# sandyresearch/chipmunk

Measured on AMD Instinct MI355X. Metric: DiT denoise steps/sec at fixed sparsity, higher is better.
Workload: dtype bf16

## Files before the change

### chipmunk_amd/_native.py

```python
from __future__ import annotations

import ctypes
import os

_HERE = os.path.dirname(os.path.abspath(__file__))
LIB_PATH = os.environ.get("CHIPMUNK_HIP_LIB") or os.path.join(_HERE, "lib", "libchipmunk_hip.so")

SYMBOLS = [
    "chipmunk_last_error", "chipmunk_abi_version", "chipmunk_set_option", "chipmunk_set_random_seed",
    "chipmunk_csp_attn", "chipmunk_csp_attn_out", "chipmunk_csp_128_attn", "chipmunk_dense_attn", "chipmunk_dense_colsum_attn",
    "chipmunk_csp_mlp_mm1", "chipmunk_csp_mlp_mm1_scatter", "chipmunk_csp_mlp_mm1_fp8", "chipmunk_csp_mlp_mm2_and_scatter_add", "chipmunk_csp_scatter_add", "chipmunk_csp_mlp_mm2",
    "chipmunk_csp_mlp_mm1_ragged", "chipmunk_csp_mlp_mm1_scatter_ragged", "chipmunk_csp_mlp_mm1_fp8_ragged", "chipmunk_csp_mlp_mm2_ragged",
    "chipmunk_csp_mlp_mm2_and_scatter_add_ragged", "chipmunk_csp_scatter_add_ragged", "chipmunk_block_mean_ragged", "chipmunk_transpose16_pitched",
    "chipmunk_csp_mlp_mm1_batched", "chipmunk_csp_mlp_mm1_scatter_batched", "chipmunk_csp_mlp_mm1_fp8_batched", "chipmunk_csp_mlp_mm2_batched",
    "chipmunk_csp_mlp_mm2_and_scatter_add_batched", "chipmunk_csp_scatter_add_batched",
    "chipmunk_csp_mlp_mm1_glu", "chipmunk_csp_mlp_mm1_glu_batched", "chipmunk_csp_mlp_mm1_glu_fp8", "chipmunk_csp_mlp_mm1_glu_fp8_batched",
    "chipmunk_topk_indices", "chipmunk_topk_delta_indices", "chipmunk_topk_mask", "chipmunk_mask_to_indices", "chipmunk_mask_to_sorted_indices", "chipmunk_packed_mask_to_indices", "chipmunk_mask_row_counts", "chipmunk_mask_to_ragged_indices", "chipmunk_copy_indices",
    "chipmunk_bitpack", "chipmunk_bitunpack", "chipmunk_transpose16", "chipmunk_block_mean", "chipmunk_quantize_fp8", "chipmunk_gather_rows", "chipmunk_qkv_split_norm", "chipmunk_split_heads_rownorm", "chipmunk_dense_colsum_topk_mask", "chipmunk_dense_attn_strided", "chipmunk_csp_attn_out_ragged", "chipmunk_compact_indices", "chipmunk_residual_ln_modulate", "chipmunk_dense_colsum_attn_strided", "chipmunk_dense_colsum_topk_mask_strided", "chipmunk_release_scratch", "chipmunk_big_scratch_fallbacks",
    "chipmunk_host_alloc", "chipmunk_host_free", "chipmunk_copy_d2h_async", "chipmunk_copy_h2d_async", "chipmunk_host_bytes",
]

_lib = None


def lib() -> ctypes.CDLL:
    global _lib
    if _lib is None:
        if not os.path.exists(LIB_PATH):
            raise ImportError(
                f"{LIB_PATH} is missing: build it with `python -m chipmunk_amd.build` (hipcc --offload-arch=gfx950). "
                "chipmunk_amd has no CPU fallback.")
        _lib = ctypes.CDLL(LIB_PATH)
        _lib.chipmunk_last_error.restype = ctypes.c_char_p
        _lib.chipmunk_abi_version.restype = ctypes.c_int
        for item in filter(None, os.environ.get("CHIPMUNK_AMD_OPTIONS", "").split(",")):
            name, _, val = item.partition("=")
            if _lib.chipmunk_set_option(name.strip().encode(), int(val)) != 0:
                raise ValueError(f"CHIPMUNK_AMD_OPTIONS: {_lib.chipmunk_last_error().decode()}")
    return _lib


def last_error() -> str:
    return lib().chipmunk_last_error().decode()


def check(rc: int, what: str) -> None:
    if rc != 0:
        raise RuntimeError(f"{what}: {last_error()}")


def set_option(name: str, value: int) -> None:
    check(lib().chipmunk_set_option(name.encode(), int(value)), "chipmunk_set_option")


def manual_seed(seed: int) -> None:
    check(lib().chipmunk_set_random_seed(ctypes.c_uint64(int(seed) & 0xFFFFFFFFFFFFFFFF)), "chipmunk_set_random_seed")


class HostBuffer:

    def __init__(self, numel: int, dtype) -> None:
        import torch
        self.dtype = dtype
        self._numel = int(numel)
        self._itemsize = torch.empty(0, dtype=dtype).element_size()
        self.nbytes = self._numel * self._itemsize
        p = ctypes.c_void_p()
        check(lib().chipmunk_host_alloc(ctypes.c_size_t(max(self.nbytes, 1)), ctypes.byref(p)), "chipmunk_host_alloc")
        self.ptr = p.value

    def numel(self) -> int:
        return self._numel

    def element_size(self) -> int:
        return self._itemsize

    def is_pinned(self) -> bool:
        return True

    def free(self) -> None:
        if getattr(self, "ptr", None):
            lib().chipmunk_host_free(ctypes.c_void_p(self.ptr))
            self.ptr = None

    def __del__(self):
        try:
            self.free()
        except Exception:
            pass


def copy_d2h_async(host_ptr: int, dev_ptr: int, nbytes: int, stream: int) -> None:
    check(lib().chipmunk_copy_d2h_async(ctypes.c_void_p(host_ptr), ctypes.c_void_p(dev_ptr), ctypes.c_size_t(nbytes), ctypes.c_void_p(stream)),
          "chipmunk_copy_d2h_async")


def copy_h2d_async(dev_ptr: int, host_ptr: int, nbytes: int, stream: int) -> None:
    check(lib().chipmunk_copy_h2d_async(ctypes.c_void_p(dev_ptr), ctypes.c_void_p(host_ptr), ctypes.c_size_t(nbytes), ctypes.c_void_p(stream)),
          "chipmunk_copy_h2d_async")


def host_bytes() -> int:
    f = lib().chipmunk_host_bytes
    f.restype = ctypes.c_size_t
    return int(f())
```

### chipmunk_amd/csrc/attn.hip

```cpp
#include "common.h"
#include "attn_params.h"
#include <type_traits>

namespace {

constexpr int QG = 192;
constexpr int QW = 48;
constexpr int KVT = 32;
constexpr int NST = 4;
constexpr int KRING = 8;
constexpr int HD = 128;
constexpr int TILE_BYTES = KVT * HD * 2;
constexpr float SCALE_LOG2E = 0.08838834764f * 1.44269504089f;
constexpr int NSTV = NST + 1;
constexpr int KEY_RING_OFF = (NST + NSTV) * TILE_BYTES;
constexpr int CS_OFF = KEY_RING_OFF + KRING * 256;
constexpr int ATTN_LDS_BYTES = CS_OFF + 2 * 2 * 4 * KVT * 4;

__device__ __forceinline__ f32x4 mfma16(bf16x8 a, bf16x8 b, f32x4 c) {
    return __builtin_amdgcn_mfma_f32_16x16x32_bf16(a, b, c, 0, 0, 0);
}

#ifdef ATTN_PROF
__device__ unsigned long long g_attn_prof[8 * 8];
// ... 1062 lines not shown
    p.q = (const uint16_t *)q, p.k = (const uint16_t *)k, p.v = (const uint16_t *)v, p.o = (uint16_t *)o_out;
    p.o_in = (const uint16_t *)o_in;
    for (int i = 0; i < 3; ++i) p.qs[i] = q_strides[i], p.ks[i] = k_strides[i], p.vs[i] = v_strides[i], p.os[i] = o_strides[i];
    p.indices = indices, p.counts = counts;
    p.B = B, p.H = H, p.Nq = Nq, p.Nk = Nk, p.G = (Nq + QG - 1) / QG, p.idx_stride = idx_stride;
    p.o_scale = (float)o_scale;
    return launch_attn<true, true, false>(p, (hipStream_t)stream);
}

extern "C" int chipmunk_csp_attn_out_ragged(const void *q, const void *k, const void *v, const void *o_in, void *o_out,
                                            const int64_t q_strides[3], const int64_t k_strides[3], const int64_t v_strides[3],
                                            const int64_t o_strides[3], const int32_t *indices, const int64_t *idx_offsets,
                                            const int32_t *counts, int B, int H, int Nq, int Nk, int o_scale, void *stream) {
    if (int e = check_common(q, k, v, o_out, B, H, Nq, Nk)) return e;
    CM_CHECK(o_in != nullptr && ((uintptr_t)o_in & 15) == 0, "csp_attn_out_ragged: o_in missing or not 16-byte aligned");
    CM_CHECK(o_scale == 1 || o_scale == -1, "o_scale must be 1 or -1");
    CM_CHECK(indices && counts && idx_offsets, "csp_attn_out_ragged: indices / offsets / counts missing");
    CM_CHECK(((uintptr_t)indices & 15) == 0, "csp_attn_out_ragged: indices must be 16-byte aligned");
    if (int e = check_strides(q_strides, "q")) return e;
    if (int e = check_strides(k_strides, "k")) return e;
    if (int e = check_strides(v_strides, "v")) return e;
    if (int e = check_strides(o_strides, "o")) return e;
    AttnParams p = {};
    p.q = (const uint16_t *)q, p.k = (const uint16_t *)k, p.v = (const uint16_t *)v, p.o = (uint16_t *)o_out;
    p.o_in = (const uint16_t *)o_in;
    for (int i = 0; i < 3; ++i) p.qs[i] = q_strides[i], p.ks[i] = k_strides[i], p.vs[i] = v_strides[i], p.os[i] = o_strides[i];
    p.indices = indices, p.counts = counts, p.idx_off = idx_offsets;
    p.B = B, p.H = H, p.Nq = Nq, p.Nk = Nk, p.G = (Nq + QG - 1) / QG, p.idx_stride = 0;
    p.o_scale = (float)o_scale;
    return launch_attn<true, true, false>(p, (hipStream_t)stream);
}

extern "C" int chipmunk_csp_128_attn(const void *q, const void *k, const void *v, void *o, const int32_t *indices,
                                     const int32_t *counts, int B, int H, int Nq, int Nk, int idx_stride,
                                     void *stream) {
    if (int e = check_common(q, k, v, o, B, H, Nq, Nk)) return e;
    CM_CHECK(indices && counts, "csp_128_attn: indices / counts missing");
    AttnParams p = {};
    p.q = (const uint16_t *)q, p.k = (const uint16_t *)k, p.v = (const uint16_t *)v, p.o = (uint16_t *)o;
    contiguous_strides(p.qs, H, Nq), contiguous_strides(p.os, H, Nq);
    contiguous_strides(p.ks, H, Nk), contiguous_strides(p.vs, H, Nk);
    p.indices = indices, p.counts = counts;
    p.B = B, p.H = H, p.Nq = Nq, p.Nk = Nk, p.G = (Nq + QG - 1) / QG, p.idx_stride = idx_stride;
    p.o_scale = 1.f;
    return launch_attn<true, false, false>(p, (hipStream_t)stream);
}

static int output_strides(int64_t os[3], const int64_t *o_strides, int H, int Nq) {
    if (!o_strides) {
        contiguous_strides(os, H, Nq);
        return CHIPMUNK_OK;
    }
    for (int i = 0; i < 3; ++i) os[i] = o_strides[i];
    return check_strides(o_strides, "o");
}

extern "C" int chipmunk_dense_attn_strided(const void *q, const void *k, const void *v, const int64_t q_strides[3],
                                           const int64_t k_strides[3], const int64_t v_strides[3], void *o,
                                           const int64_t *o_strides, float *l, int B, int H, int Nq, int Nk, void *stream) {
    if (int e = check_common(q, k, v, o, B, H, Nq, Nk)) return e;
    CM_CHECK(l != nullptr, "dense_attn: l output missing");
    if (int e = check_strides(q_strides, "q")) return e;
    if (int e = check_strides(k_strides, "k")) return e;
    if (int e = check_strides(v_strides, "v")) return e;
    AttnParams p = {};
    p.q = (const uint16_t *)q, p.k = (const uint16_t *)k, p.v = (const uint16_t *)v, p.o = (uint16_t *)o;
    for (int i = 0; i < 3; ++i) p.qs[i] = q_strides[i], p.ks[i] = k_strides[i], p.vs[i] = v_strides[i];
    if (int e = output_strides(p.os, o_strides, H, Nq)) return e;
    p.l_out = l;
    p.B = B, p.H = H, p.Nq = Nq, p.Nk = Nk, p.G = (Nq + QG - 1) / QG;
    p.o_scale = 1.f;
    if (use_dense64(B, H, Nq, Nk)) {
        CM_CHECK((int64_t)Nk * p.ks[2] * 2 < (1ll << 32) && (int64_t)Nk * p.vs[2] * 2 < (1ll << 32),
                 "attention: one head's K or V spans more than 4 GiB (32-bit DMA offsets)");
        return chipmunk_dense64_launch(q, k, v, o, l, p.qs, p.ks, p.vs, p.os, B, H, Nq, Nk, (hipStream_t)stream);
    }
    return launch_attn<false, false, true>(p, (hipStream_t)stream);
}

extern "C" int chipmunk_dense_attn(const void *q, const void *k, const void *v, const int64_t q_strides[3],
                                   const int64_t k_strides[3], const int64_t v_strides[3], void *o, float *l, int B,
                                   int H, int Nq, int Nk, void *stream) {
    return chipmunk_dense_attn_strided(q, k, v, q_strides, k_strides, v_strides, o, nullptr, l, B, H, Nq, Nk, stream);
}

extern "C" int chipmunk_dense_colsum_attn_strided(const void *q, const void *k, const void *v, const int64_t q_strides[3],
                                                  const int64_t k_strides[3], const int64_t v_strides[3], const float *pin,
                                                  void *o, const int64_t *o_strides, void *cs, float *l, int B, int H, int Nq,
                                                  int Nk, int cs_stride, void *stream) {
    if (int e = check_common(q, k, v, o, B, H, Nq, Nk)) return e;
    CM_CHECK(l && cs && pin, "dense_colsum_attn: p / cs / l missing");
    CM_CHECK(cs_stride >= Nk, "dense_colsum_attn: cs row stride %d < Nk %d", cs_stride, Nk);
    if (int e = check_strides(q_strides, "q")) return e;
    if (int e = check_strides(k_strides, "k")) return e;
    if (int e = check_strides(v_strides, "v")) return e;
    AttnParams p = {};
    p.q = (const uint16_t *)q, p.k = (const uint16_t *)k, p.v = (const uint16_t *)v, p.o = (uint16_t *)o;
    for (int i = 0; i < 3; ++i) p.qs[i] = q_strides[i], p.ks[i] = k_strides[i], p.vs[i] = v_strides[i];
    if (int e = output_strides(p.os, o_strides, H, Nq)) return e;
    p.l_out = l, p.p_in = pin, p.cs = (uint16_t *)cs, p.cs_stride = cs_stride;
    p.B = B, p.H = H, p.Nq = Nq, p.Nk = Nk, p.G = (Nq + QG - 1) / QG;
    p.o_scale = 1.f;
    hipStream_t st = (hipStream_t)stream;
    int rc;
    if (chipmunk_get_option("attn_fused_colsum") == 5) {
        if (use_colsum64(B, H, Nq, Nk)) return chipmunk_colsum64_launch(p, st);
        return launch_attn<false, false, false, true>(p, st);
    }
    if (use_dense64(B, H, Nq, Nk)) {
        CM_CHECK((int64_t)Nk * p.ks[2] * 2 < (1ll << 32) && (int64_t)Nk * p.vs[2] * 2 < (1ll << 32),
                 "attention: one head's K or V spans more than 4 GiB (32-bit DMA offsets)");
        if (chipmunk_get_option("attn_fused_colsum") != 2) {
            int hc = H;
            uint16_t *part = nullptr;
            const int hc_min = chipmunk_get_option("attn_fused_colsum") == 4 ? 1 : 0;
            if (hc_min) hc = 1;
            for (; hc >= 1; hc /= 2) {
                part = (uint16_t *)chipmunk_big_scratch(st, chipmunk_colsum_part_bytes(hc == H ? B : 1, hc, Nq, Nk));
                if (part) break;
            }
            if (part && hc == H) return chipmunk_dense64_colsum_launch(p, part, st);
            if (part) {
                for (int b = 0; b < B; ++b)
                    for (int h0 = 0; h0 < H; h0 += hc) {
                        AttnParams c = p;
                        const int hn = H - h0 < hc ? H - h0 : hc;
                        const int64_t bh0 = (int64_t)b * H + h0;
                        c.q += b * p.qs[0] + h0 * p.qs[1], c.k += b * p.ks[0] + h0 * p.ks[1], c.v += b * p.vs[0] + h0 * p.vs[1];
                        c.o += b * p.os[0] + h0 * p.os[1];
                        c.l_out += bh0 * Nq, c.p_in += bh0 * Nq, c.cs += bh0 * p.G * (int64_t)cs_stride;
                        c.B = 1, c.H = hn;
                        if (int e = chipmunk_dense64_colsum_launch(c, part, st)) return e;
                    }
                return CHIPMUNK_OK;
            }
        }
        rc = chipmunk_dense64_launch(q, k, v, o, l, p.qs, p.ks, p.vs, p.os, B, H, Nq, Nk, st);
    } else {
        rc = launch_attn<false, false, true>(p, st);
    }
    if (rc != CHIPMUNK_OK) return rc;
    if (use_colsum64(B, H, Nq, Nk)) return chipmunk_colsum64_launch(p, st);
    return launch_attn<false, false, false, true>(p, st);
}

extern "C" int chipmunk_dense_colsum_attn(const void *q, const void *k, const void *v, const int64_t q_strides[3],
                                          const int64_t k_strides[3], const int64_t v_strides[3], const float *pin,
                                          void *o, void *cs, float *l, int B, int H, int Nq, int Nk, int cs_stride,
                                          void *stream) {
    return chipmunk_dense_colsum_attn_strided(q, k, v, q_strides, k_strides, v_strides, pin, o, nullptr, cs, l, B, H, Nq, Nk,
                                              cs_stride, stream);
}

extern "C" int chipmunk_dense_colsum_topk_mask_strided(const void *q, const void *k, const void *v, const int64_t q_strides[3],
                                               const int64_t k_strides[3], const int64_t v_strides[3], const float *pin, void *o,
                                               const int64_t *o_strides, float *l, int B, int H, int Nq, int Nk, const void *static_mask,
                                               int64_t static_stride, int static_rows, const void *group_flags, void *mask,
                                               int topk, double random_amount, void *stream) {
    if (int e = check_common(q, k, v, o, B, H, Nq, Nk)) return e;
    CM_CHECK(l && pin && mask, "dense_colsum_topk_mask: p / l / mask missing");
    if (int e = check_strides(q_strides, "q")) return e;
    if (int e = check_strides(k_strides, "k")) return e;
    if (int e = check_strides(v_strides, "v")) return e;
    hipStream_t st = (hipStream_t)stream;
    if (!use_dense64(B, H, Nq, Nk) || chipmunk_get_option("attn_fused_colsum") == 2 || (Nk & 3) || Nk > CHIPMUNK_TOPK_MASK_MAX_N)
        return CHIPMUNK_ERR_UNSUPPORTED;
    AttnParams p = {};
    p.q = (const uint16_t *)q, p.k = (const uint16_t *)k, p.v = (const uint16_t *)v, p.o = (uint16_t *)o;
    for (int i = 0; i < 3; ++i) p.qs[i] = q_strides[i], p.ks[i] = k_strides[i], p.vs[i] = v_strides[i];
    CM_CHECK((int64_t)Nk * p.ks[2] * 2 < (1ll << 32) && (int64_t)Nk * p.vs[2] * 2 < (1ll << 32),
             "attention: one head's K or V spans more than 4 GiB (32-bit DMA offsets)");
    if (int e = output_strides(p.os, o_strides, H, Nq)) return e;
    p.l_out = l, p.p_in = pin, p.cs = nullptr, p.cs_stride = 0;
    p.B = B, p.H = H, p.Nq = Nq, p.Nk = Nk, p.G = (Nq + QG - 1) / QG;
    p.o_scale = 1.f;
    uint16_t *part = (uint16_t *)chipmunk_big_scratch(st, chipmunk_colsum_part_bytes(B, H, Nq, Nk));
    if (!part) return CHIPMUNK_ERR_UNSUPPORTED;
    if (int e = chipmunk_dense64_colsum_launch(p, part, st)) return e;
    const int nrb = ((Nq + 255) / 256) * 2;
    return chipmunk_topk_mask_parts(part, chipmunk_colsum_part_stride(Nk), nrb, p.G, Nq, static_mask, static_stride, static_rows, group_flags, mask, B * H * p.G, Nk,
                                    topk, random_amount, st);
}

extern "C" int chipmunk_dense_colsum_topk_mask(const void *q, const void *k, const void *v, const int64_t q_strides[3],
                                               const int64_t k_strides[3], const int64_t v_strides[3], const float *pin, void *o,
                                               float *l, int B, int H, int Nq, int Nk, const void *static_mask,
                                               int64_t static_stride, int static_rows, const void *group_flags, void *mask,
                                               int topk, double random_amount, void *stream) {
    return chipmunk_dense_colsum_topk_mask_strided(q, k, v, q_strides, k_strides, v_strides, pin, o, nullptr, l, B, H, Nq, Nk,
                                                   static_mask, static_stride, static_rows, group_flags, mask, topk, random_amount,
                                                   stream);
}
```

### chipmunk_amd/csrc/attn_params.h

```cpp
#pragma once
#include <stdint.h>
#include <hip/hip_runtime.h>

struct AttnParams {
    const uint16_t *q, *k, *v;
    uint16_t *o;
    const uint16_t *o_in;
    int64_t qs[3], ks[3], vs[3], os[3];
    const int32_t *indices, *counts;
    const int64_t *idx_off;
    float *l_out;
    const float *p_in;
    uint16_t *cs;
    int cs_stride;
    int B, H, Nq, Nk, G, idx_stride;
    float o_scale;
    int split_full, nsplit;
    float *ws;
    int32_t *tickets;
    const int32_t *plan;
    int xcd_chunks;
    const float *kmax;
    uint16_t *cs_part;
    int cs_pstride;
    int probe;
};


int chipmunk_csp64_launch(const AttnParams &p, int inplace, int grid, hipStream_t stream);
int chipmunk_dense64_colsum_launch(const AttnParams &p, uint16_t *part, hipStream_t stream);
int chipmunk_topk_mask_parts(const uint16_t *part, int part_stride, int nrb, int groups_per_bh, int Nq, const void *static_mask, int64_t static_stride,
                             int static_rows, const void *group_flags, void *mask, int rows, int n, int k, double random_amount,
                             hipStream_t stream);
size_t chipmunk_colsum_part_bytes(int B, int H, int Nq, int Nk);
int chipmunk_colsum_part_stride(int Nk);
int chipmunk_colsum64_launch(const AttnParams &p, hipStream_t stream);
int chipmunk_csp96_launch(const AttnParams &p, int inplace, int grid, hipStream_t stream);
const float *chipmunk_knorm_max(const uint16_t *k, const int64_t ks[3], int B, int H, int Nk, hipStream_t stream);

__host__ __device__ inline int colsum_part_rows(int j, int nwg, int &r0, int &r1) {
    const int a = (3 * j) >> 2, w0 = 3 * j - 4 * a;
    r0 = 2 * a + (w0 ? 1 : 0);
    r1 = 2 * (a + 1);
    return (w0 >= 2 && a + 1 < nwg) ? 2 : 1;
}

struct IndexRow {
    const int32_t *ptr;
    int width;
};
__device__ __forceinline__ IndexRow index_row(const AttnParams &p, int64_t item) {
    if (p.idx_off) {
        const int64_t o = p.idx_off[item];
        return {p.indices + o, (int)(p.idx_off[item + 1] - o)};
    }
    return {p.indices + item * p.idx_stride, p.idx_stride};
}
```

### chipmunk_amd/csrc/indexed_io.hip

```cpp
#include "common.h"
#include "attn_params.h"

namespace {

__device__ __forceinline__ uint32_t wave_incl_scan(uint32_t x) {
    x += (uint32_t)__builtin_amdgcn_update_dpp(0, (int)x, 0x111, 0xf, 0xf, true);
    x += (uint32_t)__builtin_amdgcn_update_dpp(0, (int)x, 0x112, 0xf, 0xf, true);
    x += (uint32_t)__builtin_amdgcn_update_dpp(0, (int)x, 0x114, 0xf, 0xf, true);
    x += (uint32_t)__builtin_amdgcn_update_dpp(0, (int)x, 0x118, 0xf, 0xf, true);
    x += (uint32_t)__builtin_amdgcn_update_dpp(0, (int)x, 0x142, 0xa, 0xf, false);
    x += (uint32_t)__builtin_amdgcn_update_dpp(0, (int)x, 0x143, 0xc, 0xf, false);
    return x;
}
struct M2IParams {
    const uint8_t *mask;
    int32_t *indices;
    int32_t *counts;
    int n, pad_n, multiple_of;
    const int64_t *offsets;
};

template <bool PACKED, bool SORTED = false, bool RAGGED = false>
__global__ __launch_bounds__(256) void mask_to_indices_kernel(const M2IParams p) {
    extern __shared__ __attribute__((aligned(16))) unsigned char smem[];
// ... 70 lines not shown
    }
    __syncthreads();

    if constexpr (SORTED) {
        uint32_t *blktot = (uint32_t *)T;
        for (int blk = w; blk < NB; blk += 4) {
            const uint32_t c = wave_incl_scan(__popc(bits[blk * 64 + lane]));
            if (lane == 63) blktot[blk] = c;
        }
        __syncthreads();
        if (w == 0) {
            uint32_t run = 0;
            for (int b0 = 0; b0 < NB; b0 += 64) {
                const uint32_t v = b0 + lane < NB ? blktot[b0 + lane] : 0u;
                const uint32_t incl = wave_incl_scan(v);
                if (b0 + lane < NB) blktot[b0 + lane] = run + incl - v;
                run += (uint32_t)__builtin_amdgcn_readlane((int)incl, 63);
            }
            if (lane == 0) blktot[NB] = run;
        }
        __syncthreads();
        const int total = (int)blktot[NB];
        for (int blk = w; blk < NB; blk += 4) {
            uint32_t v = bits[blk * 64 + lane];
            const uint32_t c = __popc(v);
            const uint32_t incl = wave_incl_scan(c);
            int pos = (int)(blktot[blk] + incl - c);
            const int col0 = (blk * 64 + lane) * 32;
            while (v) {
                const int bit = __builtin_ctz(v);
                v &= v - 1;
                put(pos++, col0 + bit);
            }
        }
        if constexpr (RAGGED) zero_rest(total);
        if (tid == 0) {
            const int padded = ((total + p.multiple_of - 1) / p.multiple_of) * p.multiple_of;
            int pp = total;
            for (int i = 0; i < NI && pp < padded; ++i) {
                uint32_t z = ~bits[i];
                const int rem = n - i * 32;
                if (rem < 32) z &= (1u << rem) - 1u;
                while (z && pp < padded) {
                    const int bit = __builtin_ctz(z);
                    z &= z - 1;
                    put(pp++, i * 32 + bit);
                }
            }
            if constexpr (!RAGGED) p.counts[row] = padded;
        }
        return;
    }
    for (int blk = w; blk < NB; blk += 4) {
        const uint32_t word = bits[blk * 64 + lane];
        unsigned long long mine = 0;
#pragma unroll
        for (int t = 0; t < 32; ++t) {
            const unsigned long long bal = __ballot((word >> t) & 1u);
            if (lane == t) mine = bal;
        }
        if (lane < 32) T[lane * NB + blk] = mine;
    }
    __syncthreads();

    if (tid < 32) {
        uint32_t run = 0;
        for (int blk = 0; blk < NB; ++blk) {
            pre[tid * NB + blk] = run;
            run += __popcll(T[tid * NB + blk]);
        }
        cls[tid + 1] = run;
    }
    __syncthreads();
    if (tid == 0) {
        uint32_t run = 0;
        for (int t = 0; t < 32; ++t) {
            const uint32_t c = cls[t + 1];
            cls[t] = run;
            run += c;
            if (t == 31) cls[32] = run;
        }
    }
    __syncthreads();
    const int total = (int)cls[32];

    for (int cell = tid; cell < 32 * NB; cell += 256) {
        const int t = cell / NB, blk = cell - t * NB;
        unsigned long long v = T[cell];
        int pos = (int)(cls[t] + pre[cell]);
        while (v) {
            const int bit = __builtin_ctzll(v);
            v &= v - 1;
            put(pos++, ((blk * 64 + bit) << 5) + t);
        }
    }
    if constexpr (RAGGED) zero_rest(total);

    if (tid == 0) {
        const int padded = ((total + p.multiple_of - 1) / p.multiple_of) * p.multiple_of;
        int pos = total;
        for (int i = 0; i < NI && pos < padded; ++i) {
            uint32_t z = ~bits[i];
            const int rem = n - i * 32;
            if (rem < 32) z &= (1u << rem) - 1u;
            while (z && pos < padded) {
                const int bit = __builtin_ctz(z);
                z &= z - 1;
                put(pos++, i * 32 + bit);
            }
        }
        if constexpr (!RAGGED) p.counts[row] = padded;
    }
}

struct RowCountParams {
    const uint8_t *mask;
    int32_t *counts;
    int64_t *lengths;
    int64_t rows;
    int n, pad_n, multiple_of;
};

template <bool PACKED>
__global__ __launch_bounds__(256) void mask_row_counts_kernel(const RowCountParams p) {
    const int lane = threadIdx.x & 63;
    const int64_t row = (int64_t)blockIdx.x * 4 + (threadIdx.x >> 6);
    if (row >= p.rows) return;
    const int nbytes = PACKED ? p.n >> 3 : p.n;
    const uint8_t *src = p.mask + (PACKED ? (row * p.n) >> 3 : row * p.n);
    auto set_in_byte = [](uint32_t b) { return PACKED ? (uint32_t)__popc(b) : (uint32_t)(b != 0); };
    auto set_in_word = [](uint32_t x) {
        if constexpr (!PACKED) x = (x | (x >> 1) | (x >> 2) | (x >> 3) | (x >> 4) | (x >> 5) | (x >> 6) | (x >> 7)) & 0x01010101u;
        return (uint32_t)__popc(x);
    };
    const int head = min(nbytes, (int)((16 - ((uintptr_t)src & 15)) & 15));
    uint32_t cnt = lane < head ? set_in_byte(src[lane]) : 0u;
    const int nvec = (nbytes - head) >> 4;
    const u32x4 *vec = (const u32x4 *)(src + head);
#pragma unroll 4
    for (int i = lane; i < nvec; i += 64) {
        const u32x4 x = vec[i];
        cnt += set_in_word(x[0]) + set_in_word(x[1]) + set_in_word(x[2]) + set_in_word(x[3]);
    }
    const int tail = head + (nvec << 4) + lane;
    if (tail < nbytes) cnt += set_in_byte(src[tail]);
    const int64_t kept = (uint32_t)__builtin_amdgcn_readlane((int)wave_incl_scan(cnt), 63);
    if (lane == 0) {
        const int64_t padded = ((kept + p.multiple_of - 1) / p.multiple_of) * p.multiple_of;
        p.counts[row] = (int32_t)padded;
        p.lengths[row] = (min(padded, (int64_t)p.pad_n) + 31) / 32 * 32;
    }
}

struct TopkParams {
    const void *act;
    void *cache;
    int32_t *indices;
    int32_t *counts;
    int rows, cols, multiple_of;
    float quantile, random_amount;
    uint32_t salt;
};

template <typename T>
__device__ __forceinline__ float load_as_float(const T *p, int i);
template <>
__device__ __forceinline__ float load_as_float<uint16_t>(const uint16_t *p, int i) { return bf16_bits_to_f32(p[i]); }
template <>
__device__ __forceinline__ float load_as_float<_Float16>(const _Float16 *p, int i) { return (float)p[i]; }
template <>
__device__ __forceinline__ float load_as_float<float>(const float *p, int i) { return p[i]; }

template <typename T>
__device__ __forceinline__ float round_to(float x);
template <>
__device__ __forceinline__ float round_to<uint16_t>(float x) { return round_bf16(x); }
template <>
__device__ __forceinline__ float round_to<_Float16>(float x) { return (float)(_Float16)x; }
template <>
__device__ __forceinline__ float round_to<float>(float x) { return x; }

__device__ __forceinline__ float hash_uniform(uint32_t row, uint32_t col, uint32_t salt) {
    uint32_t x = (row * 0x9E3779B9u ^ (col + 0x7F4A7C15u) * 0x85EBCA6Bu) + salt * 0xC2B2AE35u;
    x ^= x >> 16, x *= 0x7feb352du, x ^= x >> 15, x *= 0x846ca68bu, x ^= x >> 16;
    return (float)(x >> 8) * (1.0f / 16777216.0f);
}

__device__ __forceinline__ int compact_slot(bool keep, int lane, int w, uint32_t *wave_tot, int &base) {
    const unsigned long long bal = __ballot(keep);
    const int before = __popcll(bal & ((1ull << lane) - 1ull));
    if (lane == 0) wave_tot[w] = __popcll(bal);
    __syncthreads();
    int off = base, tot = 0;
#pragma unroll
    for (int i = 0; i < 16; ++i) {
        const int c = wave_tot[i];
        off += i < w ? c : 0;
        tot += c;
    }
    __syncthreads();
    base += tot;
    return keep ? off + before : -1;
}

template <typename T, bool DELTA>
__global__ __launch_bounds__(1024) void topk_indices_kernel(const TopkParams p) {
    __shared__ uint32_t wave_tot[16];
    __shared__ float thr_s;
    const int tid = threadIdx.x, lane = tid & 63, w = tid >> 6;
    const int row = blockIdx.x;
    const T *x = (const T *)p.act + (int64_t)row * p.cols;
    T *xc = DELTA ? (T *)p.cache + (int64_t)row * p.cols : nullptr;
    int32_t *out = p.indices + (int64_t)row * p.cols;
    const int cols = p.cols;
    auto value = [&](int c) {
        const float b = load_as_float<T>(x, c);
        if constexpr (DELTA) return fabsf(round_to<T>(b - load_as_float<T>(xc, c)));
        else return b;
    };

    const uint32_t salt = p.salt ^ (__float_as_uint(value(0)) * 0x27D4EB2Fu);
    if (p.quantile == 0.f) {
        if constexpr (DELTA)
            for (int c = tid; c < cols; c += 1024) xc[c] = x[c];
        for (int c = tid; c < cols; c += 1024) out[c] = c;
        if (tid == 0) p.counts[row] = cols;
        return;
    }
    if (p.quantile == 1.f) {
        for (int c = tid; c < cols; c += 1024) out[c] = -1;
        if (tid == 0) p.counts[row] = 0;
        return;
    }
    __shared__ float sample[1024];
    float v_first[16];
#pragma unroll
    for (int j = 0; j < 16; ++j) {
        const int c = j * 1024 + tid;
        v_first[j] = c < cols ? value(c) : 0.f;
    }
    sample[tid] = v_first[0];
    __syncthreads();
    if (w == 0) {
        uint32_t key[16];
#pragma unroll
        for (int j = 0; j < 16; ++j) {
            const uint32_t u = __float_as_uint(sample[lane + 64 * j]);
            key[j] = (u & 0x80000000u) ? ~u : (u | 0x80000000u);
        }
        const int k = (int)(1024 * p.quantile);
        uint32_t res = 0;
        constexpr int LOWZ = !DELTA ? 0 : std::is_same<T, uint16_t>::value ? 16 : std::is_same<T, _Float16>::value ? 13 : 0;
        constexpr int LAST = LOWZ ? LOWZ - 1 : 0;
        for (int bit = 31; bit >= LAST; --bit) {
            const uint32_t cand = res | (LOWZ && bit == LAST ? (1u << LOWZ) - 1u : (1u << bit));
            int cnt = 0;
#pragma unroll
            for (int j = 0; j < 16; ++j) cnt += key[j] < cand ? 1 : 0;
            const int tot = (int)sum_across_rows(row16_sum((float)cnt));
            if (tot <= k) res = cand;
        }
        const uint32_t u = (res & 0x80000000u) ? (res & 0x7fffffffu) : ~res;
        if (lane == 0) thr_s = __uint_as_float(u);
    }
    __syncthreads();
    const float thr = thr_s;

    __shared__ uint32_t tot[16 * 16 + 1];
    int base = 0;
    int my_last_invalid = -1;
    for (int pass0 = 0; pass0 < cols; pass0 += 16 * 1024) {
        float v[16];
#pragma unroll
        for (int j = 0; j < 16; ++j) {
            const int c = pass0 + j * 1024 + tid;
            v[j] = pass0 == 0 ? v_first[j] : (c < cols ? value(c) : 0.f);
        }
        uint32_t keepbits = 0;
        int before[16];
#pragma unroll
        for (int j = 0; j < 16; ++j) {
            const int c = pass0 + j * 1024 + tid;
            bool keep = false;
            if (c < cols) {
                keep = v[j] >= thr;
                if (!keep && p.random_amount > 0.f) keep = hash_uniform(row, c, salt) < p.random_amount;
                if (!keep) my_last_invalid = c;
            }
            const unsigned long long bal = __ballot(keep);
            before[j] = __popcll(bal & ((1ull << lane) - 1ull));
            if (lane == 0) tot[j * 16 + w] = __popcll(bal);
            keepbits |= keep ? (1u << j) : 0u;
        }
        __syncthreads();
        if (tid < 64) {
            uint32_t a0 = tot[tid * 4], a1 = tot[tid * 4 + 1], a2 = tot[tid * 4 + 2], a3 = tot[tid * 4 + 3];
            uint32_t sum = a0 + a1 + a2 + a3, incl = sum;
#pragma unroll
            for (int d = 1; d < 64; d <<= 1) {
                const uint32_t o = __shfl_up(incl, d);
                if (lane >= d) incl += o;
            }
            const uint32_t excl = incl - sum;
            tot[tid * 4] = excl, tot[tid * 4 + 1] = excl + a0, tot[tid * 4 + 2] = excl + a0 + a1;
            tot[tid * 4 + 3] = excl + a0 + a1 + a2;
            if (tid == 63) tot[256] = incl;
// ... 9 lines not shown
        base += tot[256];
        __syncthreads();
    }
    const int kept = base;
    const int mod = kept % p.multiple_of;
    const int pad = mod == 0 ? 0 : p.multiple_of - mod;
    if (tid == 0) p.counts[row] = kept + pad;
    if (pad > 0) {
        int pbase = 0;
        const int slot = compact_slot(my_last_invalid != -1, lane, w, wave_tot, pbase);
        if (slot >= 0 && slot < pad) {
            out[kept + slot] = my_last_invalid;
            if constexpr (DELTA) xc[my_last_invalid] = x[my_last_invalid];
        }
    }
}

template <typename T>
__global__ __launch_bounds__(256) void copy_indices_kernel(const T *src, T *dst, const int32_t *inds,
                                                           const int32_t *counts, int M, int R, int F) {
    const int64_t grow = blockIdx.x;
    const int64_t b = grow / ((int64_t)M * R);
    const int base_m = (int)((grow % ((int64_t)M * R)) / R);
    const int cnt = counts[b * M + base_m];
    const int32_t *ii = inds + (b * M + base_m) * (int64_t)F;
    for (int c = threadIdx.x; c < cnt; c += 256) {
        const int col = ii[c];
        dst[grow * F + col] = src[grow * F + col];
    }
}

__global__ __launch_bounds__(256) void bitpack_kernel(const uint8_t *mask, uint8_t *packed, int64_t n) {
    const int64_t nb = (n + 7) >> 3;
    for (int64_t i = (int64_t)blockIdx.x * 256 + threadIdx.x; i < nb; i += (int64_t)gridDim.x * 256) {
        uint8_t byte = 0;
        if (i * 8 + 8 <= n && ((((uintptr_t)mask) & 7) == 0)) {
            unsigned long long v = *(const unsigned long long *)(mask + i * 8);
#pragma unroll
            for (int j = 0; j < 8; ++j) byte |= (uint8_t)((((v >> (8 * j)) & 0xffull) != 0) << j);
        } else {
            for (int j = 0; j < 8 && i * 8 + j < n; ++j) byte |= (uint8_t)((mask[i * 8 + j] != 0) << j);
        }
        packed[i] = byte;
    }
}
__global__ __launch_bounds__(256) void bitunpack_kernel(const uint8_t *packed, uint8_t *mask, int64_t n) {
    const int64_t nb = (n + 7) >> 3;
    for (int64_t i = (int64_t)blockIdx.x * 256 + threadIdx.x; i < nb; i += (int64_t)gridDim.x * 256) {
        const uint8_t byte = packed[i];
        if (i * 8 + 8 <= n && ((((uintptr_t)mask) & 7) == 0)) {
            unsigned long long v = 0;
#pragma unroll
            for (int j = 0; j < 8; ++j) v |= (unsigned long long)((byte >> j) & 1u) << (8 * j);
            *(unsigned long long *)(mask + i * 8) = v;
        } else {
            for (int j = 0; j < 8 && i * 8 + j < n; ++j) mask[i * 8 + j] = (byte >> j) & 1u;
        }
    }
}

__global__ __launch_bounds__(256) void transpose16_kernel(const uint16_t *src, uint16_t *dst, int R, int C, int ld) {
    __shared__ __attribute__((aligned(16))) uint16_t tile[64][72];
    const int64_t boff = (int64_t)blockIdx.z * R * C;
    const int r0 = blockIdx.y * 64, c0 = blockIdx.x * 64;
    const int tid = threadIdx.x;
#pragma unroll
    for (int i = 0; i < 2; ++i) {
        const int item = i * 256 + tid, r = item >> 3, ch = item & 7;
        u32x4 v = {0u, 0u, 0u, 0u};
        if (r0 + r < R && c0 + ch * 8 + 8 <= C) v = *(const u32x4 *)(src + boff + (int64_t)(r0 + r) * C + c0 + ch * 8);
        else if (r0 + r < R)
            for (int e = 0; e < 8; ++e)
                if (c0 + ch * 8 + e < C) {
                    const uint32_t x = src[boff + (int64_t)(r0 + r) * C + c0 + ch * 8 + e];
                    v[e >> 1] |= x << (16 * (e & 1));
                }
#pragma unroll
        for (int e = 0; e < 4; ++e) {
            tile[ch * 8 + 2 * e][r] = (uint16_t)(v[e] & 0xffffu);
            tile[ch * 8 + 2 * e + 1][r] = (uint16_t)(v[e] >> 16);
        }
    }
    __syncthreads();
#pragma unroll
    for (int i = 0; i < 2; ++i) {
        const int item = i * 256 + tid, c = item >> 3, ch = item & 7;
        if (c0 + c >= C) continue;
        uint16_t *d = dst + (int64_t)blockIdx.z * C * ld + (int64_t)(c0 + c) * ld + r0 + ch * 8;
        if (r0 + ch * 8 + 8 <= ld && ((ld & 7) == 0)) *(u32x4 *)d = *(const u32x4 *)&tile[c][ch * 8];
        else
            for (int e = 0; e < 8; ++e)
                if (r0 + ch * 8 + e < ld) d[e] = tile[c][ch * 8 + e];
    }
}

__global__ __launch_bounds__(256) void compact_indices_kernel(const int32_t *indices, int64_t idx_stride, const int32_t *counts,
                                                             const int64_t *offsets, int32_t *flat) {
    const int64_t r = blockIdx.x;
    const int32_t *src = indices + r * idx_stride;
    const int64_t o = offsets[r];
    int32_t *dst = flat + o;
    const int width = (int)(offsets[r + 1] - o);
    int c = counts[r];
    c = c < 0 ? 0 : (c < width ? c : width);
    c = c < idx_stride ? c : (int)idx_stride;
    if ((((uintptr_t)src | (uintptr_t)dst) & 15) == 0) {
        const int c4 = c >> 2;
        for (int i = threadIdx.x; i < c4; i += 256) ((u32x4 *)dst)[i] = ((const u32x4 *)src)[i];
        for (int i = (c4 << 2) + threadIdx.x; i < c; i += 256) dst[i] = src[i];
    } else {
        for (int i = threadIdx.x; i < c; i += 256) dst[i] = src[i];
    }
    for (int i = c + threadIdx.x; i < width; i += 256) dst[i] = 0;
}

size_t m2i_lds_bytes(int n, bool sorted) {
    const int NI = (n + 31) >> 5, NB = (NI + 63) >> 6;
    if (sorted) return (size_t)NB * 64 * 4 + (size_t)(NB + 1) * 4 + 16;
    return (size_t)NB * 64 * 4 + (size_t)32 * NB * 8 + (size_t)32 * NB * 4 + 33 * 4 + 16;
}

template <bool PACKED, bool SORTED = false, bool RAGGED = false>
int launch_m2i(const void *mask, int32_t *indices, int32_t *counts, int64_t rows, int n, int pad_n, int multiple_of,
               void *stream, const int64_t *offsets = nullptr) {
    CM_CHECK(mask && indices && (RAGGED ? (const void *)offsets : (const void *)counts), "mask_to_indices: null pointer");
    CM_CHECK(rows >= 0 && n > 0 && pad_n >= n && multiple_of > 0, "mask_to_indices: bad sizes rows=%lld n=%d pad_n=%d multiple_of=%d",
             (long long)rows, n, pad_n, multiple_of);
    CM_CHECK(rows < (1ll << 31), "mask_to_indices: too many rows");
    if (PACKED) CM_CHECK(n % 8 == 0, "packed_mask_to_indices: n must be a multiple of 8 (got %d)", n);
    const size_t lds = m2i_lds_bytes(n, SORTED);
    CM_CHECK(lds <= 160 * 1024, "mask_to_indices: row length %d needs %zu B of LDS (> 160 KiB)", n, lds);
    if (rows == 0) return CHIPMUNK_OK;
    auto kern = mask_to_indices_kernel<PACKED, SORTED, RAGGED>;
    if (lds > 64 * 1024) (void)hipFuncSetAttribute((const void *)kern, hipFuncAttributeMaxDynamicSharedMemorySize, (int)lds);
    M2IParams p = {(const uint8_t *)mask, indices, counts, n, pad_n, multiple_of, offsets};
    hipLaunchKernelGGL(kern, dim3((unsigned)rows), dim3(256), lds, (hipStream_t)stream, p);
    CM_LAUNCH_CHECK();
    return CHIPMUNK_OK;
}


struct TopkMaskParams {
    const uint16_t *cs;
    const uint8_t *stat;
    const uint8_t *groups;
    uint8_t *mask;
    int64_t cs_stride, stat_stride;
    int rows, n, k, stat_rows;
    float random_amount;
    uint32_t salt;
    const uint16_t *parts;
    int64_t pstride;
    int nrb, ngroups, nq;
};

__device__ __forceinline__ uint32_t bf16_key(uint32_t u) {
    return (u & 0x8000u) ? (~u & 0xffffu) : (u | 0x8000u);
}

template <int KPT, bool ALIGNED, bool PARTS = false>
__global__ __launch_bounds__(1024) void topk_mask_kernel(const TopkMaskParams p) {
    constexpr int NV = KPT / 4;
    __shared__ int wave_cnt[16];
    const int tid = threadIdx.x, lane = tid & 63, w = tid >> 6;
    const int row = blockIdx.x;
    const int n = p.n;
    const uint16_t *x = nullptr;
    int prow = 1;
    int64_t row1 = 0;
    if constexpr (PARTS) {
        const int bh = row / p.ngroups, g = row - bh * p.ngroups;
        int r0, r1;
        prow = colsum_part_rows(g, p.nrb / 2, r0, r1);
        x = p.parts + ((int64_t)bh * p.nrb + r0) * p.pstride;
        row1 = (int64_t)(r1 - r0) * p.pstride;
    } else {
        x = p.cs + (int64_t)row * p.cs_stride;
    }
    const uint32_t lane_off8 = 8u * (uint32_t)tid;
    const uint32_t lane_off4 = 4u * (uint32_t)tid;
    uint32_t key[NV][2];
    constexpr int LB = NV % 10 == 0 ? 10 : (NV % 8 == 0 ? 8 : (NV % 6 == 0 ? 6 : 4));
    static_assert(NV % LB == 0, "NV must split into whole load batches");
#pragma unroll
    for (int j0 = 0; j0 < NV; j0 += LB) {
        uint32_t raw[LB][2];
#pragma unroll
        for (int jj = 0; jj < LB; ++jj) {
            const int c = 4 * tid + 4096 * (j0 + jj);
            uint32_t v0 = 0xffffffffu, v1 = 0xffffffffu;
            if constexpr (ALIGNED) {
                if (c < n) {
                    const u32x2 v = *(const u32x2 *)((const unsigned char *)(x + 4096 * (j0 + jj)) + lane_off8);
                    v0 = v[0], v1 = v[1];
                    if constexpr (PARTS) {
                        if (prow == 2) {
                            float a0 = __uint_as_float(v0 << 16), a1 = __uint_as_float(v0 & 0xffff0000u);
                            float a2 = __uint_as_float(v1 << 16), a3 = __uint_as_float(v1 & 0xffff0000u);
                            const u32x2 y = *(const u32x2 *)((const unsigned char *)(x + row1 + 4096 * (j0 + jj)) + lane_off8);
                            a0 += __uint_as_float(y[0] << 16), a1 += __uint_as_float(y[0] & 0xffff0000u);
                            a2 += __uint_as_float(y[1] << 16), a3 += __uint_as_float(y[1] & 0xffff0000u);
                            v0 = pack_bf16x2(a0, a1), v1 = pack_bf16x2(a2, a3);
                        }
                    }
                }
            } else if (c < n) {
                v0 = v1 = 0;
#pragma unroll
                for (int e = 0; e < 4; ++e) {
                    const uint32_t u = c + e < n ? x[c + e] : 0xffffu;
                    if (e < 2) v0 |= u << (16 * e);
                    else v1 |= u << (16 * (e - 2));
                }
            }
            raw[jj][0] = v0, raw[jj][1] = v1;
        }
#pragma unroll
        for (int jj = 0; jj < LB; ++jj) {
            key[j0 + jj][0] = bf16_key(raw[jj][0] & 0xffffu) | (bf16_key(raw[jj][0] >> 16) << 16);
            key[j0 + jj][1] = bf16_key(raw[jj][1] & 0xffffu) | (bf16_key(raw[jj][1] >> 16) << 16);
        }
        __builtin_amdgcn_sched_barrier(0);
    }
    auto block_count = [&](int mine) {
#pragma unroll
        for (int d = 32; d > 0; d >>= 1) mine += __shfl_xor(mine, d);
        if (lane == 0) wave_cnt[w] = mine;
        __syncthreads();
        int t = 0;
#pragma unroll
        for (int i = 0; i < 16; ++i) t += wave_cnt[i];
        __syncthreads();
        return t;
    };
    const bool active = p.groups == nullptr || p.groups[row] != 0;
    const int k = p.k < n ? p.k : n;
    uint32_t thr = 0x10000u;
    int ties_to_take = 0;
    if (active && k > 0) {
        uint32_t res = 0;
        for (int bit = 15; bit >= 0; --bit) {
            const uint32_t cand = res | (1u << bit);
            const uint32_t cm1 = (cand - 1u) | ((cand - 1u) << 16);
            const uint32_t one2 = 0x00010001u;
            uint32_t cnt2 = 0;
#pragma unroll
            for (int j = 0; j < NV; ++j)
#pragma unroll
                for (int h = 0; h < 2; ++h) {
                    uint32_t d;
                    asm volatile("v_pk_sub_u16 %0, %1, %2 clamp\n\tv_pk_min_u16 %0, %0, %3" : "=&v"(d) : "v"(key[j][h]), "v"(cm1), "v"(one2));
                    asm volatile("v_pk_add_u16 %0, %0, %1" : "+v"(cnt2) : "v"(d));
                }
            const int mine = (int)(cnt2 & 0xffffu) + (int)(cnt2 >> 16);
            if (block_count(mine) >= k) res = cand;
        }
        thr = res;
        int gt = 0;
#pragma unroll
        for (int j = 0; j < NV; ++j)
#pragma unroll
            for (int h = 0; h < 2; ++h) {
                uint32_t kw = key[j][h];
                asm volatile("" : "+v"(kw));
                gt += ((kw & 0xffffu) > thr ? 1 : 0) + ((kw >> 16) > thr ? 1 : 0);
            }
        ties_to_take = k - block_count(gt);
    }
    int my_ties = 0;
    if (ties_to_take > 0) {
#pragma unroll
        for (int j = 0; j < NV; ++j)
#pragma unroll
            for (int h = 0; h < 2; ++h) {
                uint32_t kw = key[j][h];
                asm volatile("" : "+v"(kw));
                my_ties += ((kw & 0xffffu) == thr ? 1 : 0) + ((kw >> 16) == thr ? 1 : 0);
            }
    }
    int tie_budget = 0;
    {
        int incl = my_ties;
#pragma unroll
        for (int d = 1; d < 64; d <<= 1) {
            const int o = __shfl_up(incl, d);
            if (lane >= d) incl += o;
        }
        if (lane == 63) wave_cnt[w] = incl;
        __syncthreads();
        int before = incl - my_ties;
#pragma unroll
        for (int i = 0; i < 16; ++i) before += i < w ? wave_cnt[i] : 0;
        __syncthreads();
        tie_budget = ties_to_take - before;
    }
    uint8_t *out = p.mask + (int64_t)row * n;
    const uint8_t *st = p.stat ? p.stat + (int64_t)(row % p.stat_rows) * p.stat_stride : nullptr;
    const bool rnd = active && p.random_amount > 0.f;
    auto combined4 = [&](int c0, uint32_t &v0, uint32_t &v1) {
        const u32x2 v = *(const u32x2 *)(x + c0);
        v0 = v[0], v1 = v[1];
        if constexpr (PARTS) {
            float a0 = __uint_as_float(v0 << 16), a1 = __uint_as_float(v0 & 0xffff0000u);
            float a2 = __uint_as_float(v1 << 16), a3 = __uint_as_float(v1 & 0xffff0000u);
            if (prow == 2) {
                const u32x2 y = *(const u32x2 *)(x + row1 + c0);
                a0 += __uint_as_float(y[0] << 16), a1 += __uint_as_float(y[0] & 0xffff0000u);
                a2 += __uint_as_float(y[1] << 16), a3 += __uint_as_float(y[1] & 0xffff0000u);
            }
            v0 = pack_bf16x2(a0, a1), v1 = pack_bf16x2(a2, a3);
        }
    };
    uint32_t first = x[0];
    if constexpr (PARTS) {
        uint32_t f0, f1;
        combined4(0, f0, f1);
        first = f0 & 0xffffu;
    }
    const uint32_t salt = p.salt ^ (first * 0x27D4EB2Fu);
    const int nsteps = (n + 4095) / 4096;
    auto emit = [&](auto keyed, int c, uint32_t v0, uint32_t v1, uint32_t sb) {
        uint32_t bytes = 0;
        if constexpr (decltype(keyed)::value) asm volatile("" : "+v"(v0), "+v"(v1));
#pragma unroll
        for (int e = 0; e < 4; ++e) {
            const uint32_t half = ((e < 2 ? v0 : v1) >> (16 * (e & 1))) & 0xffffu;
            const uint32_t kv = decltype(keyed)::value ? half : bf16_key(half);
            bool keep = kv > thr;
            const bool tie = kv == thr && tie_budget > 0 && c + e < n;
            tie_budget -= tie ? 1 : 0;
            keep = keep || tie;
            if (rnd && !keep) keep = hash_uniform(row, c + e, salt) < p.random_amount;
            keep = keep || ((sb >> (8 * e)) & 0xffu) != 0;
            bytes |= (keep ? 1u : 0u) << (8 * e);
        }
        if constexpr (ALIGNED) {
            *(uint32_t *)(out + c) = bytes;
        } else {
#pragma unroll
            for (int e = 0; e < 4; ++e)
                if (c + e < n) out[c + e] = (uint8_t)(bytes >> (8 * e));
        }
    };
    if constexpr (ALIGNED) {
        constexpr int OB = 5;
#pragma unroll
        for (int j0 = 0; j0 < NV; j0 += OB) {
            uint32_t sbv[OB];
#pragma unroll
            for (int jj = 0; jj < OB; ++jj) {
                const int c = 4 * tid + 4096 * (j0 + jj);
                sbv[jj] = (j0 + jj < NV && st && c < n) ? *(const uint32_t *)(st + c) : 0u;
            }
            __builtin_amdgcn_sched_barrier(0);
#pragma unroll
            for (int jj = 0; jj < OB; ++jj) {
                if constexpr (true) {
                    const int c = 4 * tid + 4096 * (j0 + jj);
                    if (j0 + jj < NV && c < n) emit(std::integral_constant<int, 1>{}, c, key[(j0 + jj) < NV ? (j0 + jj) : 0][0], key[(j0 + jj) < NV ? (j0 + jj) : 0][1], sbv[jj]);
                    asm volatile("" ::: "memory");
                }
            }
            __builtin_amdgcn_sched_barrier(0);
        }
    } else {
        for (int j = 0; j < nsteps; ++j) {
            const int c = 4 * tid + 4096 * j;
            if (c >= n) break;
            uint32_t v0 = 0, v1 = 0, sb = 0;
#pragma unroll
            for (int e = 0; e < 4; ++e) {
                const uint32_t u = c + e < n ? x[c + e] : 0xffffu;
                if (e < 2) v0 |= u << (16 * e);
                else v1 |= u << (16 * (e - 2));
                if (st && c + e < n) sb |= (uint32_t)st[c + e] << (8 * e);
            }
            emit(std::integral_constant<int, 0>{}, c, v0, v1, sb);
        }
    }
}

__device__ __forceinline__ uint32_t bf16_key2(uint32_t u) {
    uint32_t s;
    const uint32_t fifteen2 = 0x000f000fu;
    asm("v_pk_ashrrev_i16 %0, %1, %2" : "=v"(s) : "v"(fifteen2), "v"(u));
    return u ^ (s | 0x80008000u);
}

template <bool ALIGNED, bool PARTS>
__global__ __launch_bounds__(1024) void topk_mask_stream_kernel(const TopkMaskParams p) {
    __shared__ int wave_cnt[16];
    const int tid = threadIdx.x, lane = tid & 63, w = tid >> 6;
    const int row = blockIdx.x;
    const int n = p.n;
    const uint16_t *x = nullptr;
    int prow = 1;
    int64_t row1 = 0;
    if constexpr (PARTS) {
        const int bh = row / p.ngroups, g = row - bh * p.ngroups;
        int r0, r1;
        prow = colsum_part_rows(g, p.nrb / 2, r0, r1);
        x = p.parts + ((int64_t)bh * p.nrb + r0) * p.pstride;
        row1 = (int64_t)(r1 - r0) * p.pstride;
    } else {
        x = p.cs + (int64_t)row * p.cs_stride;
    }
    const uint32_t lane_off8 = 8u * (uint32_t)tid;
    const int nsteps = (n + 4095) / 4096;
    const bool active = p.groups == nullptr || p.groups[row] != 0;
    const int k = p.k < n ? p.k : n;
    const bool select = active && k > 0;
    const bool rnd = active && p.random_amount > 0.f;

    auto combined4 = [&](int c0, uint32_t &v0, uint32_t &v1) {
        const u32x2 v = *(const u32x2 *)(x + c0);
        v0 = v[0], v1 = v[1];
        if constexpr (PARTS) {
            if (prow == 2) {
                float a0 = __uint_as_float(v0 << 16), a1 = __uint_as_float(v0 & 0xffff0000u);
                float a2 = __uint_as_float(v1 << 16), a3 = __uint_as_float(v1 & 0xffff0000u);
                const u32x2 y = *(const u32x2 *)(x + row1 + c0);
                a0 += __uint_as_float(y[0] << 16), a1 += __uint_as_float(y[0] & 0xffff0000u);
                a2 += __uint_as_float(y[1] << 16), a3 += __uint_as_float(y[1] & 0xffff0000u);
                v0 = pack_bf16x2(a0, a1), v1 = pack_bf16x2(a2, a3);
            }
        }
    };
    uint32_t first = 0;
    if (rnd) {
        first = x[0];
        if constexpr (PARTS) {
            uint32_t f0, f1;
            combined4(0, f0, f1);
            first = f0 & 0xffffu;
        }
    }
    const uint32_t salt = p.salt ^ (first * 0x27D4EB2Fu);
    if constexpr (PARTS) {
        __syncthreads();
        if (select) {
            uint16_t *xk = const_cast<uint16_t *>(x);
            for (int j = 0; j < nsteps; ++j) {
                const int c = 4 * tid + 4096 * j;
                if (c < n) {
                    uint32_t v0, v1;
                    combined4(c, v0, v1);
                    u32x2 kk = {bf16_key2(v0), bf16_key2(v1)};
                    *(u32x2 *)(xk + c) = kk;
                }
            }
        }
        __syncthreads();
    }
    auto load_raw = [&](int j, uint32_t &v0, uint32_t &v1) {
        const int c = 4 * tid + 4096 * j;
        if constexpr (ALIGNED) {
            v0 = v1 = PARTS ? 0u : 0xffffffffu;
            if (c < n) {
                const u32x2 v = *(const u32x2 *)((const unsigned char *)(x + 4096 * j) + lane_off8);
                v0 = v[0], v1 = v[1];
            }
        } else {
            v0 = v1 = 0xffffffffu;
            if (c < n) {
                v0 = v1 = 0;
#pragma unroll
                for (int e = 0; e < 4; ++e) {
                    const uint32_t u = c + e < n ? x[c + e] : 0xffffu;
                    if (e < 2) v0 |= u << (16 * e);
                    else v1 |= u << (16 * (e - 2));
                }
            }
        }
    };
    auto to_keys = [&](uint32_t &v0, uint32_t &v1) {
        if constexpr (!PARTS) v0 = bf16_key2(v0), v1 = bf16_key2(v1);
    };
    auto block_count = [&](int mine) {
#pragma unroll
        for (int d = 32; d > 0; d >>= 1) mine += __shfl_xor(mine, d);
        if (lane == 0) wave_cnt[w] = mine;
        __syncthreads();
        int t = 0;
#pragma unroll
        for (int i = 0; i < 16; ++i) t += wave_cnt[i];
        __syncthreads();
        return t;
    };
    constexpr int U = ALIGNED ? 8 : 2;
    uint32_t thr = 0x10000u;
    int ties_to_take = 0, my_ties = 0;
    if (select) {
        uint32_t res = 0;
        for (int bit = 15; bit >= 0; --bit) {
            const uint32_t cand = res | (1u << bit);
            const uint32_t cm1 = (cand - 1u) | ((cand - 1u) << 16);
            const uint32_t one2 = 0x00010001u;
// ... 5 lines not shown
#pragma unroll
                for (int jj = 0; jj < U; ++jj) {
                    to_keys(kw[jj][0], kw[jj][1]);
#pragma unroll
                    for (int h = 0; h < 2; ++h) {
                        uint32_t d;
                        asm volatile("v_pk_sub_u16 %0, %1, %2 clamp\n\tv_pk_min_u16 %0, %0, %3" : "=&v"(d) : "v"(kw[jj][h]), "v"(cm1), "v"(one2));
                        asm volatile("v_pk_add_u16 %0, %0, %1" : "+v"(cnt2) : "v"(d));
                    }
                }
            }
            const int mine = (int)(cnt2 & 0xffffu) + (int)(cnt2 >> 16);
            if (block_count(mine) >= k) res = cand;
        }
        thr = res;
        int gt = 0;
        for (int j0 = 0; j0 < nsteps; j0 += U) {
            uint32_t kw[U][2];
#pragma unroll
            for (int jj = 0; jj < U; ++jj) load_raw(j0 + jj, kw[jj][0], kw[jj][1]);
#pragma unroll
            for (int jj = 0; jj < U; ++jj) {
                to_keys(kw[jj][0], kw[jj][1]);
#pragma unroll
                for (int h = 0; h < 2; ++h) {
                    const uint32_t lo = kw[jj][h] & 0xffffu, hi = kw[jj][h] >> 16;
                    gt += (lo > thr ? 1 : 0) + (hi > thr ? 1 : 0);
                    my_ties += (lo == thr ? 1 : 0) + (hi == thr ? 1 : 0);
                }
            }
        }
        ties_to_take = k - block_count(gt);
    }
    int tie_budget = 0;
    {
        int incl = my_ties;
#pragma unroll
        for (int d = 1; d < 64; d <<= 1) {
            const int o = __shfl_up(incl, d);
            if (lane >= d) incl += o;
        }
        if (lane == 63) wave_cnt[w] = incl;
        __syncthreads();
        int before = incl - my_ties;
#pragma unroll
        for (int i = 0; i < 16; ++i) before += i < w ? wave_cnt[i] : 0;
        __syncthreads();
        tie_budget = ties_to_take - before;
    }
    uint8_t *out = p.mask + (int64_t)row * n;
    const uint8_t *st = p.stat ? p.stat + (int64_t)(row % p.stat_rows) * p.stat_stride : nullptr;
    for (int j0 = 0; j0 < nsteps; j0 += U) {
        uint32_t kw[U][2], sbv[U];
#pragma unroll
        for (int jj = 0; jj < U; ++jj) {
            const int c = 4 * tid + 4096 * (j0 + jj);
            kw[jj][0] = kw[jj][1] = 0;
            if (select) load_raw(j0 + jj, kw[jj][0], kw[jj][1]);
            sbv[jj] = 0;
            if constexpr (ALIGNED) {
                if (st && c < n) sbv[jj] = *(const uint32_t *)(st + c);
            } else if (st) {
#pragma unroll
                for (int e = 0; e < 4; ++e)
                    if (c + e < n) sbv[jj] |= (uint32_t)st[c + e] << (8 * e);
            }
        }
#pragma unroll
        for (int jj = 0; jj < U; ++jj) {
            const int c = 4 * tid + 4096 * (j0 + jj);
            if (c >= n) continue;
            if (select) to_keys(kw[jj][0], kw[jj][1]);
            uint32_t bytes = 0;
#pragma unroll
            for (int e = 0; e < 4; ++e) {
                const uint32_t kv = (kw[jj][e >> 1] >> (16 * (e & 1))) & 0xffffu;
                bool keep = kv > thr;
                const bool tie = kv == thr && tie_budget > 0 && c + e < n;
                tie_budget -= tie ? 1 : 0;
                keep = keep || tie;
                if (rnd && !keep) keep = hash_uniform(row, c + e, salt) < p.random_amount;
                keep = keep || ((sbv[jj] >> (8 * e)) & 0xffu) != 0;
                bytes |= (keep ? 1u : 0u) << (8 * e);
            }
            if constexpr (ALIGNED) {
                *(uint32_t *)(out + c) = bytes;
            } else {
#pragma unroll
                for (int e = 0; e < 4; ++e)
                    if (c + e < n) out[c + e] = (uint8_t)(bytes >> (8 * e));
            }
        }
    }
}

}

extern "C" int chipmunk_mask_to_indices(const void *mask, int32_t *indices, int32_t *counts, int64_t rows, int n,
                                        int pad_n, int multiple_of, void *stream) {
    return launch_m2i<false>(mask, indices, counts, rows, n, pad_n, multiple_of, stream);
}

extern "C" int chipmunk_packed_mask_to_indices(const void *packed, int32_t *indices, int32_t *counts, int64_t rows,
                                               int n, int pad_n, int multiple_of, void *stream) {
    return launch_m2i<true>(packed, indices, counts, rows, n, pad_n, multiple_of, stream);
}

static int launch_topk(const void *activation, void *cache, int dtype, int32_t *indices, int32_t *counts, int rows,
                       int cols, double sparsity_amount, int multiple_of, double random_amount, void *stream) {
    CM_CHECK(activation && indices && counts, "topk_indices: null pointer");
    CM_CHECK(rows >= 0 && cols >= 1024, "topk_indices: rows >= 0 and cols >= 1024 required (the quantile is taken over the first 1024 columns); got rows=%d cols=%d", rows, cols);
    CM_CHECK(multiple_of > 0, "topk_indices: multiple_of must be positive");
    CM_CHECK(sparsity_amount >= 0.0 && sparsity_amount <= 1.0, "topk_indices: sparsity_amount must be in [0,1]");
    if (rows == 0) return CHIPMUNK_OK;
    TopkParams p = {activation, cache, indices, counts, rows, cols, multiple_of, (float)sparsity_amount, (float)random_amount,
                    random_amount > 0.0 ? chipmunk_next_random_salt() : 0u};
    hipStream_t s = (hipStream_t)stream;
#define LAUNCH_TOPK(T)                                                                                           \
    do {                                                                                                         \
        if (cache) hipLaunchKernelGGL((topk_indices_kernel<T, true>), dim3(rows), dim3(1024), 0, s, p);          \
        else hipLaunchKernelGGL((topk_indices_kernel<T, false>), dim3(rows), dim3(1024), 0, s, p);               \
    } while (0)
    switch (dtype) {
        case CHIPMUNK_DTYPE_BF16: LAUNCH_TOPK(uint16_t); break;
        case CHIPMUNK_DTYPE_FP16: LAUNCH_TOPK(_Float16); break;
        case CHIPMUNK_DTYPE_FP32: LAUNCH_TOPK(float); break;
        default: CM_CHECK(false, "topk_indices: unsupported dtype code %d", dtype);
    }
#undef LAUNCH_TOPK
    CM_LAUNCH_CHECK();
    return CHIPMUNK_OK;
}

extern "C" int chipmunk_mask_to_sorted_indices(const void *mask, int packed, int32_t *indices, int32_t *counts,
                                               int64_t rows, int n, int pad_n, int multiple_of, void *stream) {
    return packed ? launch_m2i<true, true>(mask, indices, counts, rows, n, pad_n, multiple_of, stream)
                  : launch_m2i<false, true>(mask, indices, counts, rows, n, pad_n, multiple_of, stream);
}

extern "C" int chipmunk_mask_row_counts(const void *mask, int packed, int32_t *counts, int64_t *lengths, int64_t rows, int n,
                                        int pad_n, int multiple_of, void *stream) {
    CM_CHECK(mask && counts && lengths, "mask_row_counts: null pointer");
    CM_CHECK(rows >= 0 && n > 0 && pad_n >= n && multiple_of > 0, "mask_row_counts: bad sizes rows=%lld n=%d pad_n=%d multiple_of=%d",
             (long long)rows, n, pad_n, multiple_of);
    CM_CHECK(rows < (1ll << 31), "mask_row_counts: too many rows");
    CM_CHECK(!packed || n % 8 == 0, "mask_row_counts: n must be a multiple of 8 for a packed mask (got %d)", n);
    const size_t lds = m2i_lds_bytes(n, true);
    CM_CHECK(lds <= 160 * 1024, "mask_to_indices: row length %d needs %zu B of LDS (> 160 KiB)", n, lds);
    if (rows == 0) return CHIPMUNK_OK;
    RowCountParams p = {(const uint8_t *)mask, counts, lengths, rows, n, pad_n, multiple_of};
    const dim3 grid((unsigned)((rows + 3) / 4));
    if (packed) hipLaunchKernelGGL(mask_row_counts_kernel<true>, grid, dim3(256), 0, (hipStream_t)stream, p);
    else hipLaunchKernelGGL(mask_row_counts_kernel<false>, grid, dim3(256), 0, (hipStream_t)stream, p);
    CM_LAUNCH_CHECK();
    return CHIPMUNK_OK;
}

extern "C" int chipmunk_mask_to_ragged_indices(const void *mask, int packed, int sorted, const int64_t *offsets, int32_t *flat,
                                               int64_t rows, int n, int multiple_of, void *stream) {
    if (packed) return sorted ? launch_m2i<true, true, true>(mask, flat, nullptr, rows, n, n, multiple_of, stream, offsets)
                              : launch_m2i<true, false, true>(mask, flat, nullptr, rows, n, n, multiple_of, stream, offsets);
    return sorted ? launch_m2i<false, true, true>(mask, flat, nullptr, rows, n, n, multiple_of, stream, offsets)
                  : launch_m2i<false, false, true>(mask, flat, nullptr, rows, n, n, multiple_of, stream, offsets);
}

extern "C" int chipmunk_topk_indices(const void *activation, int dtype, int32_t *indices, int32_t *counts, int rows,
                                     int cols, double sparsity_amount, int multiple_of, double random_amount,
                                     void *stream) {
    return launch_topk(activation, nullptr, dtype, indices, counts, rows, cols, sparsity_amount, multiple_of,
                       random_amount, stream);
}

extern "C" int chipmunk_topk_delta_indices(const void *activation, void *cache, int dtype, int32_t *indices,
                                           int32_t *counts, int rows, int cols, double sparsity_amount,
                                           int multiple_of, double random_amount, void *stream) {
    CM_CHECK(cache != nullptr, "topk_delta_indices: cache missing");
    return launch_topk(activation, cache, dtype, indices, counts, rows, cols, sparsity_amount, multiple_of,
                       random_amount, stream);
}

extern "C" int chipmunk_copy_indices(const void *src, void *dst, const int32_t *inds, const int32_t *counts, int B,
                                     int M, int R, int F, int elem_size, void *stream) {
    CM_CHECK(src && dst && inds && counts, "copy_indices: null pointer");
    CM_CHECK(B >= 0 && M > 0 && R > 0 && F > 0, "copy_indices: bad sizes");
    CM_CHECK(elem_size == 2 || elem_size == 4, "copy_indices: element size must be 2 or 4 bytes (got %d)", elem_size);
    const int64_t rows = (int64_t)B * M * R;
    if (rows == 0) return CHIPMUNK_OK;
    CM_CHECK(rows < (1ll << 31), "copy_indices: too many rows");
    hipStream_t s = (hipStream_t)stream;
    if (elem_size == 2)
        hipLaunchKernelGGL(copy_indices_kernel<uint16_t>, dim3((unsigned)rows), dim3(256), 0, s, (const uint16_t *)src,
                           (uint16_t *)dst, inds, counts, M, R, F);
    else
        hipLaunchKernelGGL(copy_indices_kernel<uint32_t>, dim3((unsigned)rows), dim3(256), 0, s, (const uint32_t *)src,
                           (uint32_t *)dst, inds, counts, M, R, F);
    CM_LAUNCH_CHECK();
    return CHIPMUNK_OK;
}

extern "C" int chipmunk_bitpack(const void *mask, void *packed, int64_t n, void *stream) {
    CM_CHECK(mask && packed && n >= 0, "bitpack: bad arguments");
    if (n == 0) return CHIPMUNK_OK;
    const int64_t nb = (n + 7) >> 3;
    const unsigned grid = (unsigned)((nb + 255) / 256 < 8192 ? (nb + 255) / 256 : 8192);
    hipLaunchKernelGGL(bitpack_kernel, dim3(grid), dim3(256), 0, (hipStream_t)stream, (const uint8_t *)mask,
                       (uint8_t *)packed, n);
    CM_LAUNCH_CHECK();
    return CHIPMUNK_OK;
}

extern "C" int chipmunk_bitunpack(const void *packed, void *mask, int64_t n, void *stream) {
    CM_CHECK(mask && packed && n >= 0, "bitunpack: bad arguments");
    if (n == 0) return CHIPMUNK_OK;
    const int64_t nb = (n + 7) >> 3;
    const unsigned grid = (unsigned)((nb + 255) / 256 < 8192 ? (nb + 255) / 256 : 8192);
    hipLaunchKernelGGL(bitunpack_kernel, dim3(grid), dim3(256), 0, (hipStream_t)stream, (const uint8_t *)packed,
                       (uint8_t *)mask, n);
    CM_LAUNCH_CHECK();
    return CHIPMUNK_OK;
}

extern "C" int chipmunk_transpose16(const void *src, void *dst, int B, int R, int C, void *stream) {
    CM_CHECK(src && dst && B > 0 && R > 0 && C > 0, "transpose16: bad arguments");
    CM_CHECK((C & 7) == 0 || true, "unreachable");
    hipLaunchKernelGGL(transpose16_kernel, dim3((C + 63) / 64, (R + 63) / 64, B), dim3(256), 0, (hipStream_t)stream,
                       (const uint16_t *)src, (uint16_t *)dst, R, C, R);
    CM_LAUNCH_CHECK();
    return CHIPMUNK_OK;
}

extern "C" int chipmunk_transpose16_pitched(const void *src, void *dst, int B, int R, int C, int ld, void *stream) {
    CM_CHECK(src && dst && B > 0 && R > 0 && C > 0, "transpose16: bad arguments");
    CM_CHECK(ld >= R, "transpose16: the output pitch ld (%d) must be at least R (%d)", ld, R);
    hipLaunchKernelGGL(transpose16_kernel, dim3((C + 63) / 64, (ld + 63) / 64, B), dim3(256), 0, (hipStream_t)stream,
                       (const uint16_t *)src, (uint16_t *)dst, R, C, ld);
    CM_LAUNCH_CHECK();
    return CHIPMUNK_OK;
}

template <typename V>
__global__ __launch_bounds__(256) void gather_rows_kernel(const V *src, V *dst, const int32_t *map, int64_t n_out,
                                                          int64_t n_src, int64_t cpr, int64_t total) {
    for (int64_t idx = (int64_t)blockIdx.x * 256 + threadIdx.x; idx < total; idx += (int64_t)gridDim.x * 256) {
        const int64_t row = idx / cpr, c = idx - row * cpr;
        const int64_t o = row / n_out, r = row - o * n_out;
        dst[idx] = src[(o * n_src + map[r]) * cpr + c];
    }
}

extern "C" int chipmunk_gather_rows(const void *src, void *dst, const int32_t *map, int64_t outer, int64_t n_src,
                                    int64_t n_out, int64_t row_bytes, void *stream) {
    CM_CHECK(src && dst && map, "gather_rows: null pointer");
    CM_CHECK(outer >= 0 && n_src > 0 && n_out >= 0 && row_bytes > 0, "gather_rows: bad sizes");
    if (outer == 0 || n_out == 0) return CHIPMUNK_OK;
    hipStream_t s = (hipStream_t)stream;
    const uintptr_t align = (uintptr_t)src | (uintptr_t)dst | (uintptr_t)row_bytes;
#define LAUNCH_GATHER(V)                                                                                              \
    do {                                                                                                              \
        const int64_t cpr = row_bytes / (int64_t)sizeof(V), total = outer * n_out * cpr;                               \
        const int64_t blocks = (total + 255) / 256;                                                                    \
        hipLaunchKernelGGL((gather_rows_kernel<V>), dim3((unsigned)(blocks > 65536 * 16 ? 65536 * 16 : blocks)),       \
                           dim3(256), 0, s, (const V *)src, (V *)dst, map, n_out, n_src, cpr, total);                  \
    } while (0)
    if ((align & 15) == 0) LAUNCH_GATHER(u32x4);
    else if ((align & 3) == 0) LAUNCH_GATHER(uint32_t);
    else if ((align & 1) == 0) LAUNCH_GATHER(uint16_t);
    else LAUNCH_GATHER(uint8_t);
#undef LAUNCH_GATHER
    CM_LAUNCH_CHECK();
    return CHIPMUNK_OK;
}

int chipmunk_topk_mask_parts(const uint16_t *part, int part_stride, int nrb, int groups_per_bh, int Nq, const void *static_mask, int64_t static_stride,
                             int static_rows, const void *group_flags, void *mask, int rows, int n, int k, double random_amount,
                             hipStream_t s) {
    CM_CHECK(part && mask && rows >= 0 && n > 0 && (n & 3) == 0 && n <= CHIPMUNK_TOPK_MASK_MAX_N && k >= 0 && part_stride >= n && (part_stride & 3) == 0, "topk_mask_parts: bad arguments");
    CM_CHECK(!static_mask || (static_rows > 0 && static_stride >= n && (static_stride & 3) == 0 && ((uintptr_t)static_mask & 3) == 0),
             "topk_mask_parts: bad static mask geometry");
    CM_CHECK(((uintptr_t)mask & 3) == 0 && ((uintptr_t)part & 7) == 0, "topk_mask_parts: unaligned buffers");
    if (rows == 0) return CHIPMUNK_OK;
    TopkMaskParams p = {nullptr, (const uint8_t *)static_mask, (const uint8_t *)group_flags, (uint8_t *)mask, 0, static_stride,
                        rows, n, k, static_mask ? static_rows : 1, (float)random_amount,
                        random_amount > 0.0 ? chipmunk_next_random_salt() : 0u};
    p.parts = part, p.pstride = part_stride, p.nrb = nrb, p.ngroups = groups_per_bh, p.nq = Nq;
    if (n > 1024 * 120 || chipmunk_get_option("topk_mask_stream") == 1) hipLaunchKernelGGL((topk_mask_stream_kernel<true, true>), dim3(rows), dim3(1024), 0, s, p);
    else if (n <= 1024 * 16) hipLaunchKernelGGL((topk_mask_kernel<16, true, true>), dim3(rows), dim3(1024), 0, s, p);
    else if (n <= 1024 * 48) hipLaunchKernelGGL((topk_mask_kernel<48, true, true>), dim3(rows), dim3(1024), 0, s, p);
    else hipLaunchKernelGGL((topk_mask_kernel<120, true, true>), dim3(rows), dim3(1024), 0, s, p);
    CM_LAUNCH_CHECK();
    return CHIPMUNK_OK;
}

__global__ __launch_bounds__(256) void qkv_split_norm_kernel(const uint16_t *qkv, int64_t row_stride, const uint16_t *qw,
                                                             const uint16_t *kw, uint16_t *q, uint16_t *k, uint16_t *v, int64_t n,
                                                             int H, float eps, int64_t segments, const float *fcos, const float *fsin,
                                                             int64_t rope_rows) {
    const int l15 = threadIdx.x & 15;
    u32x4 wq = {0x3f803f80u, 0x3f803f80u, 0x3f803f80u, 0x3f803f80u}, wk = wq;
    if (qw) wq = *(const u32x4 *)(qw + l15 * 8);
    if (kw) wk = *(const u32x4 *)(kw + l15 * 8);
    for (int64_t seg = ((int64_t)blockIdx.x * 256 + threadIdx.x) >> 4; seg < segments; seg += ((int64_t)gridDim.x * 256) >> 4) {
        const int64_t tok = seg / (3 * H);
        const int rem = (int)(seg - tok * 3 * H), which = rem / H, h = rem - which * H;
        u32x4 x = *(const u32x4 *)(qkv + tok * row_stride + (int64_t)rem * 128 + l15 * 8);
        uint16_t *dst = (which == 0 ? q : which == 1 ? k : v) + ((int64_t)h * n + tok) * 128 + l15 * 8;
        if (which < 2) {
            float f[8], ss = 0.f;
#pragma unroll
            for (int e = 0; e < 4; ++e) {
                f[2 * e] = __uint_as_float(x[e] << 16), f[2 * e + 1] = __uint_as_float(x[e] & 0xffff0000u);
                ss = __builtin_fmaf(f[2 * e], f[2 * e], ss);
                ss = __builtin_fmaf(f[2 * e + 1], f[2 * e + 1], ss);
            }
            ss = row16_sum(ss);
            const float r = 1.0f / __builtin_sqrtf(ss * (1.0f / 128.0f) + eps);
            const u32x4 w = which == 0 ? wq : wk;
#pragma unroll
            for (int e = 0; e < 4; ++e) {
                float a = f[2 * e] * r, b = f[2 * e + 1] * r;
                round_bf16_pair(a, b);
                x[e] = pack_bf16x2(a * __uint_as_float(w[e] << 16), b * __uint_as_float(w[e] & 0xffff0000u));
            }
            if (fcos && tok < rope_rows) {
                const f32x4 c0 = *(const f32x4 *)(fcos + tok * 128 + l15 * 8), c1 = *(const f32x4 *)(fcos + tok * 128 + l15 * 8 + 4);
                const f32x4 s0 = *(const f32x4 *)(fsin + tok * 128 + l15 * 8), s1 = *(const f32x4 *)(fsin + tok * 128 + l15 * 8 + 4);
#pragma unroll
                for (int e = 0; e < 4; ++e) {
                    const float re = __uint_as_float(x[e] << 16), im = __uint_as_float(x[e] & 0xffff0000u);
                    const float cr = e < 2 ? c0[2 * e] : c1[2 * e - 4], ci = e < 2 ? c0[2 * e + 1] : c1[2 * e - 3];
                    const float sr = e < 2 ? s0[2 * e] : s1[2 * e - 4], si = e < 2 ? s0[2 * e + 1] : s1[2 * e - 3];
                    x[e] = pack_bf16x2(re * cr + (-im) * sr, im * ci + re * si);
                }
            }
        }
        *(u32x4 *)dst = x;
    }
}

extern "C" int chipmunk_qkv_split_norm(const void *qkv, int64_t row_stride, const void *q_weight, const void *k_weight, void *q,
                                       void *k, void *v, int64_t n, int heads, float eps, const float *freqs_cos,
                                       const float *freqs_sin, int64_t rope_rows, void *stream) {
    CM_CHECK(qkv && q && k && v, "qkv_split_norm: null pointer");
    CM_CHECK(n >= 0 && heads > 0 && row_stride >= (int64_t)3 * heads * 128, "qkv_split_norm: bad sizes");
    CM_CHECK((((uintptr_t)qkv | (uintptr_t)q | (uintptr_t)k | (uintptr_t)v | (uintptr_t)q_weight | (uintptr_t)k_weight) & 15) == 0 &&
                 (row_stride & 7) == 0 && (((uintptr_t)freqs_cos | (uintptr_t)freqs_sin) & 15) == 0,
             "qkv_split_norm: pointers and the row stride must be 16-byte aligned");
    CM_CHECK((freqs_cos == nullptr) == (freqs_sin == nullptr) && rope_rows >= 0 && rope_rows <= n, "qkv_split_norm: bad rotary arguments");
    if (n == 0) return CHIPMUNK_OK;
    const int64_t segments = n * 3 * heads, blocks = (segments + 15) / 16;
    hipLaunchKernelGGL(qkv_split_norm_kernel, dim3((unsigned)(blocks > 256 * 64 ? 256 * 64 : blocks)), dim3(256), 0, (hipStream_t)stream,
                       (const uint16_t *)qkv, row_stride, (const uint16_t *)q_weight, (const uint16_t *)k_weight, (uint16_t *)q,
                       (uint16_t *)k, (uint16_t *)v, n, heads, eps, segments, freqs_cos, freqs_sin, freqs_cos ? rope_rows : 0);
    CM_LAUNCH_CHECK();
    return CHIPMUNK_OK;
}

extern "C" int chipmunk_topk_mask(const void *cs, int64_t cs_stride, const void *static_mask, int64_t static_stride,
                                  int static_rows, const void *group_flags, void *mask, int rows, int n, int k,
                                  double random_amount, void *stream) {
    CM_CHECK(cs && mask, "topk_mask: null pointer");
    CM_CHECK(rows >= 0 && n > 0 && k >= 0, "topk_mask: bad sizes (rows=%d n=%d k=%d)", rows, n, k);
    CM_CHECK(cs_stride >= n, "topk_mask: cs row stride %lld < n %d", (long long)cs_stride, n);
    CM_CHECK(n <= CHIPMUNK_TOPK_MASK_MAX_N, "topk_mask: rows of more than %d columns are not supported (got %d)", CHIPMUNK_TOPK_MASK_MAX_N, n);
    CM_CHECK(!static_mask || (static_rows > 0 && static_stride >= n), "topk_mask: bad static mask geometry");
    CM_CHECK(random_amount >= 0.0 && random_amount <= 1.0, "topk_mask: random_amount must be in [0,1]");
    if (rows == 0) return CHIPMUNK_OK;
    TopkMaskParams p = {(const uint16_t *)cs, (const uint8_t *)static_mask, (const uint8_t *)group_flags, (uint8_t *)mask,
                        cs_stride, static_stride, rows, n, k, static_mask ? static_rows : 1, (float)random_amount,
                        random_amount > 0.0 ? chipmunk_next_random_salt() : 0u};
    hipStream_t s = (hipStream_t)stream;
    const bool aligned = n % 4 == 0 && (((uintptr_t)cs) & 7) == 0 && (cs_stride * 2) % 8 == 0 && (((uintptr_t)mask) & 3) == 0 &&
                         (!static_mask || ((((uintptr_t)static_mask) & 3) == 0 && static_stride % 4 == 0));
#define LAUNCH_TM(KPT)                                                                                       \
    do {                                                                                                     \
        if (aligned) hipLaunchKernelGGL((topk_mask_kernel<KPT, true>), dim3(rows), dim3(1024), 0, s, p);     \
        else hipLaunchKernelGGL((topk_mask_kernel<KPT, false>), dim3(rows), dim3(1024), 0, s, p);            \
    } while (0)
    if (n > 1024 * 120 || chipmunk_get_option("topk_mask_stream") == 1) {
        if (aligned) hipLaunchKernelGGL((topk_mask_stream_kernel<true, false>), dim3(rows), dim3(1024), 0, s, p);
        else hipLaunchKernelGGL((topk_mask_stream_kernel<false, false>), dim3(rows), dim3(1024), 0, s, p);
    } else if (n <= 1024 * 16) LAUNCH_TM(16);
    else if (n <= 1024 * 48) LAUNCH_TM(48);
    else LAUNCH_TM(120);
#undef LAUNCH_TM
    CM_LAUNCH_CHECK();
    return CHIPMUNK_OK;
}

extern "C" int chipmunk_compact_indices(const int32_t *indices, int64_t idx_stride, const int32_t *counts, const int64_t *offsets,
                                        int32_t *flat, int64_t rows, void *stream) {
    CM_CHECK(indices && counts && offsets && flat, "compact_indices: null pointer");
    CM_CHECK(rows >= 0 && rows < (1ll << 31) && idx_stride > 0, "compact_indices: bad sizes rows=%lld idx_stride=%lld", (long long)rows,
             (long long)idx_stride);
    if (rows == 0) return CHIPMUNK_OK;
    hipLaunchKernelGGL(compact_indices_kernel, dim3((unsigned)rows), dim3(256), 0, (hipStream_t)stream, indices, idx_stride, counts,
                       offsets, flat);
    CM_LAUNCH_CHECK();
    return CHIPMUNK_OK;
}
```

### chipmunk_amd/csrc/torch_registry.cpp

```cpp
#include <ATen/ATen.h>
#include <ATen/hip/impl/HIPStreamMasqueradingAsCUDA.h>
#include <Python.h>
#include <c10/core/DeviceGuard.h>
#include <torch/library.h>

#include <vector>

#include "../../include/chipmunk_hip.h"

extern "C" {
PyObject *PyInit_cuda(void) {
    static struct PyModuleDef module_def = {PyModuleDef_HEAD_INIT, "cuda", NULL, -1, NULL};
    return PyModule_Create(&module_def);
}
}

namespace chipmunk {
namespace {

void *cur_stream(const at::Tensor &t) {
    return (void *)c10::hip::getCurrentHIPStreamMasqueradingAsCUDA(t.device().index()).stream();
}
void check(int rc, const char *op) { TORCH_CHECK(rc == 0, "chipmunk::", op, ": ", chipmunk_last_error()); }

// ... 589 lines not shown
    TORCH_CHECK(counts.numel() == activation.size(0) * activation.size(1), "counts must be [batch, rows]");
    int dtype;
    switch (activation.scalar_type()) {
        case at::kBFloat16: dtype = CHIPMUNK_DTYPE_BF16; break;
        case at::kHalf: dtype = CHIPMUNK_DTYPE_FP16; break;
        case at::kFloat: dtype = CHIPMUNK_DTYPE_FP32; break;
        default: TORCH_CHECK(false, "Unsupported dtype for topk_indices");
    }
    c10::DeviceGuard guard(activation.device());
    check(chipmunk_topk_indices(activation.data_ptr(), dtype, indices.data_ptr<int>(), counts.data_ptr<int>(),
                                (int)(activation.size(0) * activation.size(1)), (int)activation.size(2),
                                sparsity_amount, (int)multiple_of, random_amount, cur_stream(activation)),
          "topk_indices");
}

void topk_delta_indices(at::Tensor activation, at::Tensor cache, at::Tensor indices, at::Tensor counts,
                        double sparsity_amount, int64_t multiple_of, double random_amount) {
    CHECK_DEV(activation); CHECK_DEV(cache); CHECK_DEV(indices); CHECK_DEV(counts);
    CHECK_CONTIG(activation); CHECK_CONTIG(cache); CHECK_CONTIG(indices); CHECK_CONTIG(counts);
    TORCH_CHECK(activation.dim() == 3 && cache.sizes() == activation.sizes(), "activation and cache must be [batch, rows, cols]");
    TORCH_CHECK(cache.scalar_type() == activation.scalar_type(), "activation and cache must have the same dtype");
    CHECK_I32(indices); CHECK_I32(counts);
    TORCH_CHECK(indices.sizes() == activation.sizes(), "indices must have the shape of activation");
    TORCH_CHECK(counts.numel() == activation.size(0) * activation.size(1), "counts must be [batch, rows]");
    int dtype;
    switch (activation.scalar_type()) {
        case at::kBFloat16: dtype = CHIPMUNK_DTYPE_BF16; break;
        case at::kHalf: dtype = CHIPMUNK_DTYPE_FP16; break;
        case at::kFloat: dtype = CHIPMUNK_DTYPE_FP32; break;
        default: TORCH_CHECK(false, "Unsupported dtype for topk_delta_indices");
    }
    c10::DeviceGuard guard(activation.device());
    check(chipmunk_topk_delta_indices(activation.data_ptr(), cache.data_ptr(), dtype, indices.data_ptr<int>(),
                                      counts.data_ptr<int>(), (int)(activation.size(0) * activation.size(1)),
                                      (int)activation.size(2), sparsity_amount, (int)multiple_of, random_amount,
                                      cur_stream(activation)),
          "topk_delta_indices");
}

std::vector<at::Tensor> mask_to_indices(at::Tensor mask, int64_t multiple_of, int64_t pad_to_multiple_of) {
    TORCH_CHECK(mask.dim() == 4, "mask must be 4-dimensional [b, h, m, n]");
    TORCH_CHECK(mask.scalar_type() == at::kBool, "mask must be bool type");
    CHECK_DEV(mask);
    TORCH_CHECK(multiple_of > 0 && pad_to_multiple_of > 0, "multiple_of and pad_to_multiple_of must be positive");
    mask = mask.contiguous();
    const int64_t b = mask.size(0), h = mask.size(1), m = mask.size(2), n = mask.size(3);
    const int64_t pad_n = ((n + pad_to_multiple_of - 1) / pad_to_multiple_of) * pad_to_multiple_of;
    c10::DeviceGuard guard(mask.device());
    at::Tensor indices = at::empty({b, h, m, pad_n}, mask.options().dtype(at::kInt));
    at::Tensor counts = at::empty({b, h, m}, mask.options().dtype(at::kInt));
    check(chipmunk_mask_to_indices(mask.data_ptr(), indices.data_ptr<int>(), counts.data_ptr<int>(), b * h * m, (int)n,
                                   (int)pad_n, (int)multiple_of, cur_stream(mask)),
          "mask_to_indices");
    return {indices, counts};
}

std::vector<at::Tensor> packed_mask_to_indices(at::Tensor packed, at::IntArrayRef shape, int64_t multiple_of,
                                               int64_t pad_to_multiple_of) {
    TORCH_CHECK(packed.scalar_type() == at::kByte && packed.is_contiguous(), "packed must be a contiguous uint8 tensor");
    CHECK_DEV(packed);
    TORCH_CHECK(shape.size() == 4, "shape must be [b, h, m, n]");
    const int64_t b = shape[0], h = shape[1], m = shape[2], n = shape[3];
    TORCH_CHECK(n % 8 == 0, "n must be a multiple of 8");
    TORCH_CHECK(packed.numel() * 8 >= b * h * m * n, "packed is too short for the given shape");
    const int64_t pad_n = ((n + pad_to_multiple_of - 1) / pad_to_multiple_of) * pad_to_multiple_of;
    c10::DeviceGuard guard(packed.device());
    at::Tensor indices = at::empty({b, h, m, pad_n}, packed.options().dtype(at::kInt));
    at::Tensor counts = at::empty({b, h, m}, packed.options().dtype(at::kInt));
    check(chipmunk_packed_mask_to_indices(packed.data_ptr(), indices.data_ptr<int>(), counts.data_ptr<int>(),
                                          b * h * m, (int)n, (int)pad_n, (int)multiple_of, cur_stream(packed)),
          "packed_mask_to_indices");
    return {indices, counts};
}

at::Tensor transpose_last2(at::Tensor x) {
    CHECK_DEV(x);
    TORCH_CHECK(x.dim() >= 2 && x.element_size() == 2, "transpose_last2: need a >=2-D tensor of a 16-bit dtype");
    x = x.contiguous();
    const int64_t R = x.size(-2), C = x.size(-1), B = x.numel() / (R * C);
    auto sizes = x.sizes().vec();
    std::swap(sizes[sizes.size() - 1], sizes[sizes.size() - 2]);
    c10::DeviceGuard guard(x.device());
    at::Tensor out = at::empty(sizes, x.options());
    check(chipmunk_transpose16(x.data_ptr(), out.data_ptr(), (int)B, (int)R, (int)C, cur_stream(x)), "transpose_last2");
    return out;
}

at::Tensor transpose_last2_pitched(at::Tensor x, int64_t ld) {
    CHECK_DEV(x);
    TORCH_CHECK(x.dim() >= 2 && x.element_size() == 2, "transpose_last2_pitched: need a >=2-D tensor of a 16-bit dtype");
    x = x.contiguous();
    const int64_t R = x.size(-2), C = x.size(-1), B = x.numel() / (R * C);
    TORCH_CHECK(ld >= R, "transpose_last2_pitched: ld must be at least the row count");
    auto sizes = x.sizes().vec();
    sizes[sizes.size() - 2] = C;
    sizes[sizes.size() - 1] = ld;
    c10::DeviceGuard guard(x.device());
    at::Tensor out = at::empty(sizes, x.options());
    check(chipmunk_transpose16_pitched(x.data_ptr(), out.data_ptr(), (int)B, (int)R, (int)C, (int)ld, cur_stream(x)), "transpose_last2_pitched");
    return out;
}

at::Tensor block_mean(at::Tensor x, int64_t mbm) {
    CHECK_DEV(x);
    TORCH_CHECK(x.dim() == 3 && x.scalar_type() == at::kBFloat16, "block_mean: need a [b, n, c] bfloat16 tensor");
    TORCH_CHECK(mbm > 0 && x.size(1) > 0, "block_mean: mbm and n must be positive");
    x = x.contiguous();
    c10::DeviceGuard guard(x.device());
    const int64_t n = x.size(1), blocks = (n + mbm - 1) / mbm;
    at::Tensor out = at::empty({x.size(0), blocks, x.size(2)}, x.options());
    if (n % mbm == 0) {
        check(chipmunk_block_mean(x.data_ptr(), out.data_ptr(), x.size(0) * n, (int)x.size(2), (int)mbm, cur_stream(x)), "block_mean");
    } else {
        for (int64_t b = 0; b < x.size(0); ++b)
            check(chipmunk_block_mean_ragged(x[b].data_ptr(), out[b].data_ptr(), n, (int)x.size(2), (int)mbm, cur_stream(x)), "block_mean");
    }
    return out;
}

at::Tensor quantize_fp8(at::Tensor x, at::Tensor scale, double max_value) {
    CHECK_DEV(x); CHECK_DEV(scale);
    TORCH_CHECK(x.scalar_type() == at::kBFloat16, "quantize_fp8: x must be bfloat16");
    TORCH_CHECK(scale.scalar_type() == at::kFloat && scale.numel() == 1, "quantize_fp8: scale must be a one-element float32 tensor");
    TORCH_CHECK(x.numel() % 8 == 0, "quantize_fp8: the element count must be a multiple of 8");
    x = x.contiguous();
    c10::DeviceGuard guard(x.device());
    at::Tensor out = at::empty(x.sizes(), x.options().dtype(at::kFloat8_e4m3fn));
    check(chipmunk_quantize_fp8(x.data_ptr(), scale.data_ptr<float>(), out.data_ptr(), x.numel(), (float)max_value, cur_stream(x)), "quantize_fp8");
    return out;
}

std::vector<at::Tensor> mask_to_sorted_indices(at::Tensor mask, at::IntArrayRef shape, int64_t multiple_of,
                                               int64_t pad_to_multiple_of) {
    CHECK_DEV(mask);
    const bool packed = mask.scalar_type() == at::kByte;
    TORCH_CHECK(packed || mask.scalar_type() == at::kBool, "mask must be bool, or uint8 bit-packed with a shape");
    mask = mask.contiguous();
    std::vector<int64_t> shp = packed ? shape.vec() : mask.sizes().vec();
    TORCH_CHECK(shp.size() == 4, "shape must be [b, h, m, n]");
    const int64_t b = shp[0], h = shp[1], m = shp[2], n = shp[3];
    if (packed) TORCH_CHECK(n % 8 == 0 && mask.numel() * 8 >= b * h * m * n, "bad packed mask");
    const int64_t pad_n = ((n + pad_to_multiple_of - 1) / pad_to_multiple_of) * pad_to_multiple_of;
    c10::DeviceGuard guard(mask.device());
    at::Tensor indices = at::empty({b, h, m, pad_n}, mask.options().dtype(at::kInt));
    at::Tensor counts = at::empty({b, h, m}, mask.options().dtype(at::kInt));
    check(chipmunk_mask_to_sorted_indices(mask.data_ptr(), packed ? 1 : 0, indices.data_ptr<int>(),
                                          counts.data_ptr<int>(), b * h * m, (int)n, (int)pad_n, (int)multiple_of,
                                          cur_stream(mask)),
          "mask_to_sorted_indices");
    return {indices, counts};
}

std::vector<at::Tensor> mask_to_ragged_indices(at::Tensor mask, at::IntArrayRef shape, int64_t multiple_of, int64_t pad_to_multiple_of,
                                               bool sorted) {
    CHECK_DEV(mask);
    const bool packed = mask.scalar_type() == at::kByte;
    TORCH_CHECK(packed || mask.scalar_type() == at::kBool, "mask must be bool, or uint8 bit-packed with a shape");
    TORCH_CHECK(multiple_of > 0 && pad_to_multiple_of > 0, "multiple_of and pad_to_multiple_of must be positive");
    mask = mask.contiguous();
    std::vector<int64_t> shp = packed ? shape.vec() : mask.sizes().vec();
    TORCH_CHECK(shp.size() == 4, "shape must be [b, h, m, n]");
    const int64_t b = shp[0], h = shp[1], m = shp[2], n = shp[3], rows = b * h * m;
    if (packed) TORCH_CHECK(n % 8 == 0 && mask.numel() * 8 >= rows * n, "bad packed mask");
    const int64_t pad_n = ((n + pad_to_multiple_of - 1) / pad_to_multiple_of) * pad_to_multiple_of;
    TORCH_CHECK(n > 0 && pad_n <= INT_MAX, "rows must have between 1 and 2^31 - 1 columns");
    c10::DeviceGuard guard(mask.device());
    at::Tensor counts = at::empty({b, h, m}, mask.options().dtype(at::kInt));
    at::Tensor len = at::empty({rows}, mask.options().dtype(at::kLong));
    check(chipmunk_mask_row_counts(mask.data_ptr(), packed ? 1 : 0, counts.data_ptr<int>(), len.data_ptr<int64_t>(), rows, (int)n,
                                   (int)pad_n, (int)multiple_of, cur_stream(mask)),
          "mask_to_ragged_indices");
    at::Tensor offsets = at::zeros({rows + 1}, len.options());
    if (rows) offsets.narrow(0, 1, rows).copy_(len.cumsum(0));
    const int64_t total = rows ? offsets[rows].item<int64_t>() : 0;
    at::Tensor flat = at::empty({total + 64}, counts.options());
    flat.narrow(0, total, 64).zero_();
    check(chipmunk_mask_to_ragged_indices(mask.data_ptr(), packed ? 1 : 0, sorted ? 1 : 0, offsets.data_ptr<int64_t>(), flat.data_ptr<int>(),
                                          rows, (int)n, (int)multiple_of, cur_stream(mask)),
          "mask_to_ragged_indices");
    return {flat, offsets, counts};
}

std::vector<at::Tensor> dense_colsum_attn_layout(at::Tensor q, at::Tensor k, at::Tensor v, at::Tensor p, bool token_major_o);
at::Tensor topk_mask(at::Tensor cs, int64_t k, double random_amount, const c10::optional<at::Tensor> &groups,
                     const c10::optional<at::Tensor> &static_mask);
std::vector<at::Tensor> dense_colsum_topk_mask(at::Tensor q, at::Tensor k, at::Tensor v, at::Tensor p, int64_t k_top, double random_amount,
                                               const c10::optional<at::Tensor> &groups, const c10::optional<at::Tensor> &static_mask,
                                               bool token_major_o) {
    CHECK_DEV(q); CHECK_DEV(k); CHECK_DEV(v); CHECK_DEV(p);
    CHECK_BF16(q); CHECK_BF16(k); CHECK_BF16(v);
    const bool shapes_ok = q.dim() == 4 && k.dim() == 4 && v.dim() == 4 && q.size(3) == 128 && q.stride(3) == 1 && k.stride(3) == 1 &&
                           v.stride(3) == 1 && p.scalar_type() == at::kFloat && p.is_contiguous();
    if (shapes_ok) {
        const int64_t B = q.size(0), H = q.size(1), Nq = q.size(2), Nk = k.size(2), G = (Nq + 191) / 192;
        const void *st = nullptr, *gf = nullptr;
        int64_t st_stride = 0, st_rows = 1;
        at::Tensor stc, gfc;
        bool ok = p.numel() == B * H * Nq;
        if (ok && static_mask.has_value() && static_mask->defined()) {
            stc = *static_mask;
            ok = stc.is_cuda() && stc.scalar_type() == at::kBool && stc.dim() == 4 && stc.size(3) == Nk && stc.size(2) == G && stc.size(1) == H &&
                 (stc.size(0) == 1 || stc.size(0) == B) && stc.stride(3) == 1 && stc.stride(1) == G * stc.stride(2) &&
                 (stc.size(0) == 1 || stc.stride(0) == H * stc.stride(1));
            if (ok) st = stc.data_ptr(), st_stride = stc.stride(2), st_rows = stc.size(0) * H * G;
        }
        if (ok && groups.has_value() && groups->defined()) {
            gfc = *groups;
            ok = gfc.is_cuda() && gfc.scalar_type() == at::kBool && gfc.dim() == 4 && gfc.size(3) == 1 && gfc.size(2) == G && gfc.size(1) == H &&
                 (gfc.size(0) == 1 || gfc.size(0) == B);
            if (ok) {
                gfc = gfc.expand({B, H, G, 1}).contiguous();
                gf = gfc.data_ptr();
            }
        }
        if (ok) {
            c10::DeviceGuard guard(q.device());
            at::Tensor o = alloc_o(q, q, token_major_o);
            const int64_t os[3] = {o.stride(0), o.stride(1), o.stride(2)};
            at::Tensor l = at::empty({B, H, Nq, 1}, q.options().dtype(at::kFloat));
            at::Tensor mask = at::empty({B, H, G, Nk}, q.options().dtype(at::kBool));
            const int64_t qs[3] = {q.stride(0), q.stride(1), q.stride(2)}, ks[3] = {k.stride(0), k.stride(1), k.stride(2)},
                          vs[3] = {v.stride(0), v.stride(1), v.stride(2)};
            const int rc = chipmunk_dense_colsum_topk_mask_strided(q.data_ptr(), k.data_ptr(), v.data_ptr(), qs, ks, vs, p.data_ptr<float>(), o.data_ptr(),
                                                           os, l.data_ptr<float>(), (int)B, (int)H, (int)Nq, (int)Nk, st, st_stride, (int)st_rows, gf,
                                                           mask.data_ptr(), (int)k_top, random_amount, cur_stream(q));
            if (rc == CHIPMUNK_OK) return {o, mask, l};
            if (rc != CHIPMUNK_ERR_UNSUPPORTED) check(rc, "dense_colsum_topk_mask");
        }
    }
    auto ocl = dense_colsum_attn_layout(q, k, v, p, token_major_o);
    at::Tensor cs = ocl[1];
    const int64_t Nk = k.size(2), G = (q.size(2) + 191) / 192;
    if (cs.size(-1) != Nk || cs.size(-2) != G) cs = cs.slice(-2, 0, G).slice(-1, 0, Nk);
    return {ocl[0], topk_mask(cs, k_top, random_amount, groups, static_mask), ocl[2]};
}

at::Tensor topk_mask(at::Tensor cs, int64_t k, double random_amount, const c10::optional<at::Tensor> &groups,
                     const c10::optional<at::Tensor> &static_mask) {
    CHECK_DEV(cs); CHECK_BF16(cs);
    TORCH_CHECK(cs.dim() == 4 && cs.stride(3) == 1, "cs must be [B, H, G, N] with a contiguous last dim");
    const int64_t B = cs.size(0), H = cs.size(1), G = cs.size(2), N = cs.size(3);
    if (!(cs.stride(1) == G * cs.stride(2) && (B == 1 || cs.stride(0) == H * cs.stride(1)))) cs = cs.contiguous();
    const int64_t rows = B * H * G;
    c10::DeviceGuard guard(cs.device());
    at::Tensor mask = at::empty({B, H, G, N}, cs.options().dtype(at::kBool));
    const void *st = nullptr, *gf = nullptr;
    int64_t st_stride = 0, st_rows = 1;
    at::Tensor stc, gfc;
    if (static_mask.has_value() && static_mask->defined()) {
        stc = *static_mask;
        CHECK_DEV(stc);
        TORCH_CHECK(stc.scalar_type() == at::kBool && stc.dim() == 4 && stc.size(3) == N && stc.size(2) == G &&
                    stc.size(1) == H && (stc.size(0) == 1 || stc.size(0) == B), "static_mask must be bool [1|B, H, G, N]");
        if (!(stc.stride(3) == 1 && stc.stride(1) == G * stc.stride(2) && (stc.size(0) == 1 || stc.stride(0) == H * stc.stride(1))))
            stc = stc.contiguous();
        st = stc.data_ptr(), st_stride = stc.stride(2), st_rows = stc.size(0) * H * G;
    }
    if (groups.has_value() && groups->defined()) {
        gfc = *groups;
        CHECK_DEV(gfc);
        TORCH_CHECK(gfc.scalar_type() == at::kBool && gfc.dim() == 4 && gfc.size(3) == 1 && gfc.size(2) == G &&
                    gfc.size(1) == H && (gfc.size(0) == 1 || gfc.size(0) == B), "groups must be bool [1|B, H, G, 1]");
        gfc = gfc.expand({B, H, G, 1}).contiguous();
        gf = gfc.data_ptr();
    }
    check(chipmunk_topk_mask(cs.data_ptr(), cs.stride(2), st, st_stride, (int)st_rows, gf, mask.data_ptr(), (int)rows, (int)N,
                             (int)k, random_amount, cur_stream(cs)),
          "topk_mask");
    return mask;
}

at::Tensor bitpack(at::Tensor mask) {
    TORCH_CHECK(mask.scalar_type() == at::kBool, "mask must be bool type");
    CHECK_DEV(mask);
    mask = mask.contiguous();
    c10::DeviceGuard guard(mask.device());
    at::Tensor packed = at::empty({(mask.numel() + 7) / 8}, mask.options().dtype(at::kByte));
    check(chipmunk_bitpack(mask.data_ptr(), packed.data_ptr(), mask.numel(), cur_stream(mask)), "bitpack");
    return packed;
}
at::Tensor bitunpack(at::Tensor packed, at::IntArrayRef shape) {
    TORCH_CHECK(packed.scalar_type() == at::kByte && packed.is_contiguous(), "packed must be a contiguous uint8 tensor");
    CHECK_DEV(packed);
    int64_t n = 1;
    for (auto d : shape) n *= d;
    TORCH_CHECK(packed.numel() * 8 >= n, "packed is too short for the given shape");
    c10::DeviceGuard guard(packed.device());
    at::Tensor mask = at::empty(shape, packed.options().dtype(at::kBool));
    check(chipmunk_bitunpack(packed.data_ptr(), mask.data_ptr(), n, cur_stream(packed)), "bitunpack");
    return mask;
}

std::vector<at::Tensor> qkv_split_norm(at::Tensor qkv, const c10::optional<at::Tensor> &q_weight, const c10::optional<at::Tensor> &k_weight,
                                       int64_t heads, double eps, const c10::optional<at::Tensor> &freqs_cos,
                                       const c10::optional<at::Tensor> &freqs_sin) {
    CHECK_DEV(qkv); CHECK_BF16(qkv);
    TORCH_CHECK(qkv.dim() == 2 && qkv.stride(1) == 1 && qkv.size(1) >= 3 * heads * 128, "qkv_split_norm: qkv must be [n, >= 3*heads*128] with a contiguous last dim");
    const void *qw = nullptr, *kw = nullptr;
    at::Tensor qwc, kwc;
    if (q_weight.has_value() && q_weight->defined()) { qwc = q_weight->contiguous(); CHECK_DEV(qwc); CHECK_BF16(qwc); TORCH_CHECK(qwc.numel() == 128); qw = qwc.data_ptr(); }
    if (k_weight.has_value() && k_weight->defined()) { kwc = k_weight->contiguous(); CHECK_DEV(kwc); CHECK_BF16(kwc); TORCH_CHECK(kwc.numel() == 128); kw = kwc.data_ptr(); }
    const int64_t n = qkv.size(0);
    const float *fc = nullptr, *fs = nullptr;
    int64_t rope_rows = 0;
    at::Tensor fcc, fsc;
    if (freqs_cos.has_value() && freqs_cos->defined()) {
        TORCH_CHECK(freqs_sin.has_value() && freqs_sin->defined(), "qkv_split_norm: freqs_cos without freqs_sin");
        fcc = freqs_cos->contiguous(), fsc = freqs_sin->contiguous();
        CHECK_DEV(fcc); CHECK_DEV(fsc);
        TORCH_CHECK(fcc.scalar_type() == at::kFloat && fsc.scalar_type() == at::kFloat && fcc.dim() == 2 && fcc.size(1) == 128 &&
                    fsc.sizes() == fcc.sizes() && fcc.size(0) <= n, "qkv_split_norm: freqs must be float32 [rows <= n, 128]");
        fc = fcc.data_ptr<float>(), fs = fsc.data_ptr<float>(), rope_rows = fcc.size(0);
    }
    c10::DeviceGuard guard(qkv.device());
    at::Tensor out = at::empty({3, 1, heads, n, 128}, qkv.options());
    check(chipmunk_qkv_split_norm(qkv.data_ptr(), qkv.stride(0), qw, kw, out[0].data_ptr(), out[1].data_ptr(), out[2].data_ptr(), n,
                                  (int)heads, (float)eps, fc, fs, rope_rows, cur_stream(qkv)),
          "qkv_split_norm");
    return {out[0], out[1], out[2]};
}

std::vector<at::Tensor> split_heads_rownorm(at::Tensor x, int64_t heads, int64_t parts, const c10::optional<at::Tensor> &w0,
                                            const c10::optional<at::Tensor> &w1, const c10::optional<at::Tensor> &w2, int64_t norm_mask,
                                            int64_t rope_mask, double eps, const c10::optional<at::Tensor> &freqs_cos,
                                            const c10::optional<at::Tensor> &freqs_sin) {
    CHECK_DEV(x); CHECK_BF16(x);
    TORCH_CHECK(parts >= 1 && parts <= 3 && heads >= 1 && heads <= 64, "split_heads_rownorm: parts must be in 1 .. 3 and heads in 1 .. 64");
    TORCH_CHECK((x.dim() == 2 || x.dim() == 3) && x.stride(-1) == 1 && x.size(-1) >= parts * heads * 128,
                "split_heads_rownorm: x must be [B, n, >= parts*heads*128] or [n, >= parts*heads*128] with a contiguous last dim");
    TORCH_CHECK(norm_mask >= 0 && rope_mask >= 0 && (norm_mask >> parts) == 0 && (rope_mask >> parts) == 0, "split_heads_rownorm: a mask names a part past parts");
    const int64_t B = x.dim() == 3 ? x.size(0) : 1, n = x.size(-2), C = heads * 128;
    TORCH_CHECK(B >= 1, "split_heads_rownorm: empty batch");
    const c10::optional<at::Tensor> *ws[3] = {&w0, &w1, &w2};
    at::Tensor wc[3];
    const void *wp[3] = {nullptr, nullptr, nullptr};
    int wd[3] = {0, 0, 0};
    for (int p = 0; p < 3; ++p) {
        if (!(ws[p]->has_value() && (*ws[p])->defined())) continue;
        TORCH_CHECK(p < parts && (norm_mask >> p & 1), "split_heads_rownorm: weight ", p, " belongs to a part that is not normalised");
        wc[p] = (*ws[p])->contiguous();
        CHECK_DEV(wc[p]);
        TORCH_CHECK((wc[p].scalar_type() == at::kBFloat16 || wc[p].scalar_type() == at::kFloat) && wc[p].numel() == C,
                    "split_heads_rownorm: a weight must be bfloat16 or float32 with heads*128 entries");
        wp[p] = wc[p].data_ptr(), wd[p] = wc[p].scalar_type() == at::kFloat ? 2 : 1;
    }
    const float *fc = nullptr, *fs = nullptr;
    int64_t rope_rows = 0;
    at::Tensor fcc, fsc;
    const bool has_cos = freqs_cos.has_value() && freqs_cos->defined(), has_sin = freqs_sin.has_value() && freqs_sin->defined();
    TORCH_CHECK(has_cos == has_sin, "split_heads_rownorm: freqs_cos and freqs_sin come together");
    TORCH_CHECK(rope_mask == 0 || has_cos, "split_heads_rownorm: a rotated part needs freqs_cos / freqs_sin");
    if (has_cos) {
        fcc = freqs_cos->contiguous(), fsc = freqs_sin->contiguous();
        CHECK_DEV(fcc); CHECK_DEV(fsc);
        TORCH_CHECK(fcc.scalar_type() == at::kFloat && fsc.scalar_type() == at::kFloat && fcc.dim() == 2 && fcc.size(1) == 128 &&
                    fsc.sizes() == fcc.sizes() && fcc.size(0) <= n, "split_heads_rownorm: freqs must be float32 [rows <= n, 128]");
        fc = fcc.data_ptr<float>(), fs = fsc.data_ptr<float>(), rope_rows = fcc.size(0);
    }
    c10::DeviceGuard guard(x.device());
    at::Tensor out = at::empty({parts, B, heads, n, 128}, x.options());
    void *op[3] = {nullptr, nullptr, nullptr};
    std::vector<at::Tensor> res;
    for (int p = 0; p < parts; ++p) res.push_back(out[p]), op[p] = res.back().data_ptr();
    if (n == 0) return res;
    check(chipmunk_split_heads_rownorm(x.data_ptr(), x.dim() == 3 ? x.stride(0) : 0, x.stride(-2), (int)parts, wp[0], wd[0], wp[1], wd[1], wp[2],
                                       wd[2], op[0], op[1], op[2], (unsigned)norm_mask, (unsigned)rope_mask, B, n, (int)heads, (float)eps, fc,
                                       fs, rope_rows, cur_stream(x)),
          "split_heads_rownorm");
    return res;
}

at::Tensor gather_rows(at::Tensor src, at::Tensor map) {
    CHECK_DEV(src);
    CHECK_DEV(map);
    TORCH_CHECK(src.dim() >= 2, "gather_rows: src must be [..., n, d]");
    TORCH_CHECK(map.scalar_type() == at::kInt && map.dim() == 1 && map.is_contiguous(), "gather_rows: map must be a contiguous int32 vector");
    src = src.contiguous();
    const int64_t n_src = src.size(-2), d = src.size(-1), n_out = map.numel();
    const int64_t outer = n_src * d == 0 ? 0 : src.numel() / (n_src * d);
    auto sizes = src.sizes().vec();
    sizes[sizes.size() - 2] = n_out;
    c10::DeviceGuard guard(src.device());
    at::Tensor dst = at::empty(sizes, src.options());
    if (dst.numel() == 0) return dst;
    check(chipmunk_gather_rows(src.data_ptr(), dst.data_ptr(), map.data_ptr<int>(), outer, n_src, n_out,
                               d * (int64_t)src.element_size(), cur_stream(src)),
          "gather_rows");
    return dst;
}

}

TORCH_LIBRARY(chipmunk, m) {
    m.def("csp_mlp_mm1(Tensor a, Tensor b_colmajor, Tensor(c!) c, Tensor bias, Tensor pa_cache_colmajor, Tensor indices, Tensor indices_counts) -> ()");
    m.def("csp_mlp_mm2_and_scatter_add(Tensor packed, Tensor(unpacked_colmajor!) unpacked_colmajor, Tensor sp_inds, Tensor sp_counts, Tensor mma_a, Tensor mma_b, Tensor mma_c, int num_sms_scatter_add, int matmul_kernel) -> ()");

    m.def("csp_attn(Tensor q, Tensor k, Tensor v, Tensor o, Tensor indices, Tensor indices_counts, int o_scale) -> ()");
    m.def("csp_128_attn(Tensor q, Tensor k, Tensor v, Tensor indices, Tensor indices_counts) -> Tensor");
    m.def("dense_attn(Tensor q, Tensor k, Tensor v) -> Tensor[]");
    m.def("dense_colsum_attn(Tensor q, Tensor k, Tensor v, Tensor p) -> Tensor[]");

    m.def("copy_indices(Tensor bmfc1, Tensor(bm_mid_cache!) bm_mid_cache, Tensor sp_inds, Tensor sp_counts) -> ()");
    m.def("topk_indices(Tensor activation, Tensor(indices!) indices, Tensor counts, float sparsity_amount, int multiple_of, float random_amount) -> ()");
    m.def("csp_scatter_add(Tensor packed, Tensor(unpacked_colmajor!) unpacked_colmajor, Tensor sp_inds, Tensor sp_counts, int num_sms) -> ()");
    m.def("mask_to_indices(Tensor mask, int multiple_of, int pad_to_multiple_of) -> Tensor[]");

    m.def("csp_attn_out(Tensor q, Tensor k, Tensor v, Tensor o_in, Tensor indices, Tensor indices_counts, int o_scale) -> Tensor");
    m.def("csp_mlp_mm1_scatter(Tensor a, Tensor b_colmajor, Tensor(c!) c, Tensor bias, Tensor(pa_cache_colmajor!) pa_cache_colmajor, Tensor indices, Tensor indices_counts) -> ()");
    m.def("csp_mlp_mm2(Tensor mma_a, Tensor mma_b, Tensor indices, Tensor counts, Tensor(mma_c!) mma_c) -> ()");
    m.def("csp_mlp_mm1_fp8(Tensor a, Tensor b, Tensor(c!) c, Tensor bias, Tensor(pa_cache_colmajor!) pa_cache_colmajor, Tensor indices, Tensor indices_counts, Tensor scale_a, Tensor scale_b, bool update_cache) -> ()");
    m.def("csp_mlp_mm1_fp8_scatter(Tensor a, Tensor b, Tensor(c!) c, Tensor bias, Tensor(pa_cache_colmajor!) pa_cache_colmajor, Tensor indices, Tensor indices_counts, Tensor scale_a, Tensor scale_b) -> ()");
    m.def("csp_mlp_mm1_glu(Tensor a, Tensor b_gate, Tensor b_up, Tensor(c!) c, Tensor? bias_gate, Tensor? bias_up, Tensor(pa_cache_colmajor!) pa_cache_colmajor, Tensor indices, Tensor indices_counts, str act, bool update_cache) -> ()");
    m.def("csp_mlp_mm1_glu_fp8(Tensor a, Tensor b_gate, Tensor b_up, Tensor(c!) c, Tensor? bias_gate, Tensor? bias_up, Tensor(pa_cache_colmajor!) pa_cache_colmajor, Tensor indices, Tensor indices_counts, Tensor scale_a, Tensor scale_b_gate, Tensor scale_b_up, str act, bool update_cache) -> ()");
    m.def("topk_delta_indices(Tensor activation, Tensor(cache!) cache, Tensor(indices!) indices, Tensor(counts!) counts, float sparsity_amount, int multiple_of, float random_amount) -> ()");
    m.def("packed_mask_to_indices(Tensor packed, int[] shape, int multiple_of, int pad_to_multiple_of) -> Tensor[]");
    m.def("mask_to_sorted_indices(Tensor mask, int[] shape, int multiple_of, int pad_to_multiple_of) -> Tensor[]");
    m.def("topk_mask(Tensor cs, int k, float random_amount, Tensor? groups, Tensor? static_mask) -> Tensor");
    m.def("dense_colsum_topk_mask(Tensor q, Tensor k, Tensor v, Tensor p, int k_top, float random_amount, Tensor? groups, Tensor? static_mask, bool token_major_o=False) -> Tensor[]");
    m.def("dense_attn_layout(Tensor q, Tensor k, Tensor v, bool token_major_o) -> Tensor[]");
    m.def("dense_colsum_attn_layout(Tensor q, Tensor k, Tensor v, Tensor p, bool token_major_o) -> Tensor[]");
    m.def("compact_indices(Tensor indices, Tensor counts) -> Tensor[]");
    m.def("mask_to_ragged_indices(Tensor mask, int[] shape, int multiple_of, int pad_to_multiple_of, bool sorted) -> Tensor[]");
    m.def("csp_attn_out_ragged(Tensor q, Tensor k, Tensor v, Tensor o_in, Tensor indices, Tensor offsets, Tensor indices_counts, int o_scale) -> Tensor");
    m.def("residual_ln_modulate(Tensor x, Tensor? y, Tensor? gate, Tensor shift, Tensor scale, float eps) -> Tensor[]");
    m.def("transpose_last2(Tensor x) -> Tensor");
    m.def("transpose_last2_pitched(Tensor x, int ld) -> Tensor");
    m.def("block_mean(Tensor x, int mbm) -> Tensor");
    m.def("quantize_fp8(Tensor x, Tensor scale, float max_value) -> Tensor");
    m.def("bitpack(Tensor mask) -> Tensor");
    m.def("bitunpack(Tensor packed, int[] shape) -> Tensor");
    m.def("gather_rows(Tensor src, Tensor map) -> Tensor");
    m.def("qkv_split_norm(Tensor qkv, Tensor? q_weight, Tensor? k_weight, int heads, float eps, Tensor? freqs_cos=None, Tensor? freqs_sin=None) -> Tensor[]");
    m.def("split_heads_rownorm(Tensor x, int heads, int parts, Tensor? w0, Tensor? w1, Tensor? w2, int norm_mask, int rope_mask, float eps, Tensor? freqs_cos=None, Tensor? freqs_sin=None) -> Tensor[]");
}

TORCH_LIBRARY_IMPL(chipmunk, CUDA, m) {
    m.impl("qkv_split_norm", &qkv_split_norm);
    m.impl("split_heads_rownorm", &split_heads_rownorm);
    m.impl("csp_mlp_mm1_fp8_scatter", &csp_mlp_mm1_fp8_scatter);
    m.impl("dense_colsum_topk_mask", &dense_colsum_topk_mask);
    m.impl("csp_mlp_mm1", &csp_mlp_mm1);
    m.impl("csp_mlp_mm2_and_scatter_add", &csp_mlp_mm2_and_scatter_add);
    m.impl("copy_indices", &copy_indices);
    m.impl("topk_indices", &topk_indices);
    m.impl("csp_scatter_add", &csp_scatter_add);
    m.impl("mask_to_indices", &mask_to_indices);
    m.impl("csp_attn", &csp_attn);
    m.impl("csp_128_attn", &csp_128_attn);
    m.impl("dense_attn", &dense_attn);
    m.impl("dense_colsum_attn", &dense_colsum_attn);
    m.impl("compact_indices", &compact_indices);
    m.impl("residual_ln_modulate", &residual_ln_modulate);
    m.impl("csp_attn_out_ragged", &csp_attn_out_ragged);
    m.impl("dense_attn_layout", &dense_attn_layout);
    m.impl("dense_colsum_attn_layout", &dense_colsum_attn_layout);
    m.impl("csp_attn_out", &csp_attn_out);
    m.impl("csp_mlp_mm1_scatter", &csp_mlp_mm1_scatter);
    m.impl("csp_mlp_mm2", &csp_mlp_mm2);
    m.impl("csp_mlp_mm1_fp8", &csp_mlp_mm1_fp8);
    m.impl("csp_mlp_mm1_glu", &csp_mlp_mm1_glu);
    m.impl("csp_mlp_mm1_glu_fp8", &csp_mlp_mm1_glu_fp8);
    m.impl("topk_delta_indices", &topk_delta_indices);
    m.impl("packed_mask_to_indices", &packed_mask_to_indices);
    m.impl("mask_to_sorted_indices", &mask_to_sorted_indices);
    m.impl("mask_to_ragged_indices", &mask_to_ragged_indices);
    m.impl("topk_mask", &topk_mask);
    m.impl("transpose_last2", &transpose_last2);
    m.impl("transpose_last2_pitched", &transpose_last2_pitched);
    m.impl("block_mean", &block_mean);
    m.impl("quantize_fp8", &quantize_fp8);
    m.impl("bitpack", &bitpack);
    m.impl("bitunpack", &bitunpack);
    m.impl("gather_rows", &gather_rows);
}

}
```

### chipmunk_amd/modules/attn.py

```python
from __future__ import annotations

from typing import Optional, Tuple

import torch
import torch.nn.functional as F
from torch import Tensor, nn

from .. import ops
from ..ops.voxel import get_local_indices_with_text
from ..util.config import GLOBAL_CONFIG, amd_key
from ..util.layer_counter import LayerCounter
from ..util.storage import AttnStorage
from ..util.storage.offloaded_tensor import release_kept_offloaded, release_resident, reserve_kept_offloaded, reserve_resident

singleton_static_mask: Optional[Tensor] = None
singleton_video_query_groups: Optional[Tensor] = None


def _cdiv(a: int, b: int) -> int:
    return (a + b - 1) // b


def _dense_attn_raw(q: Tensor, k: Tensor, v: Tensor, token_major_o: bool):
    return torch.ops.chipmunk.dense_attn_layout(q, k, v, True) if token_major_o else torch.ops.chipmunk.dense_attn(q, k, v)


class SparseDiffAttn(nn.Module):
    def __init__(self, layer_num: int, layer_counter: LayerCounter, storage_slot: int = 0, query_group_offset: int = 0):
        super().__init__()
        self.layer_num = layer_num
        self.layer_counter = layer_counter
        self.query_group_offset = query_group_offset
        self.storage = AttnStorage(layer_num, init_names=["indices", "out_cache"], slot=storage_slot)
        self.mask_shape = [None] * GLOBAL_CONFIG["num_model_invocations_per_inference_step"]
        self._unpacked = [None] * GLOBAL_CONFIG["num_model_invocations_per_inference_step"]

    def initialize_static_mask(self, seq_shape: Tuple, txt_len: int, local_heads_num: int, device: torch.device):
        if len(seq_shape) == 2:
            raise NotImplementedError("Not yet implemented for 2D sequences")
        tt, th, tw = seq_shape
        cfg = GLOBAL_CONFIG["attn"]
        n_video = tt * th * tw
        topk = int(cfg["top_keys"] * n_video)
        lv = cfg["local_voxels"]
        mask, _, _ = get_local_indices_with_text(vid_shape=(tt, th, tw), txt_len=txt_len, voxel_shape=(4, 6, 8),
                                                 local_shape=(lv, lv, lv), rk=cfg["random_keys"], device=device)
        if cfg["local_1d_window"] > 0:
            window = int(cfg["local_1d_window"] * n_video)
            for qg in range(n_video // 192):
                centre = qg * 192 + 96
                mask[qg, max(0, centre - window // 2):min(n_video, centre + window // 2)] = True
        mask = mask[None, None, :, :].expand(1, local_heads_num, -1, -1).contiguous()
        sparse_groups = (mask.sum(dim=-1, keepdim=True) + topk) < (n_video + txt_len)
        global singleton_static_mask, singleton_video_query_groups
        singleton_static_mask = mask
        singleton_video_query_groups = sparse_groups

    def _static(self, heads: int, qg: int, n: int):
        g0 = self.query_group_offset
        assert heads <= singleton_static_mask.shape[1] or singleton_static_mask.shape[1] == 1, (
            f"this module serves {heads} heads but initialize_static_mask() built {singleton_static_mask.shape[1]} head planes "
            "(local_heads_num): build the static mask for the largest head chunk")
        h = min(heads, singleton_static_mask.shape[1])
        return (singleton_static_mask[:, :h, g0:g0 + qg, :n], singleton_video_query_groups[:, :h, g0:g0 + qg, :])

    def random_and_topk(self, cs: Tensor, topk: int) -> Tensor:
        cfg = GLOBAL_CONFIG["attn"]
        qg, n = cs.shape[-2], cs.shape[-1]
        static, groups = self._static(cs.shape[1], qg, n)
        if cs.is_cuda and amd_key("attn", "fused_topk_mask") and cs.dtype == torch.bfloat16 and n <= ops.TOPK_MASK_MAX_N:
            return ops.topk_mask(cs, topk, 0.01, groups, static)
        mask = torch.randint(0, 100, cs.shape, device=cs.device, dtype=torch.uint8) == 0
        mask.scatter_(-1, cs.topk(k=topk, dim=-1).indices, True)
        mask.logical_and_(groups)
        mask.logical_or_(static)
        return mask

    def release_kept_indices(self) -> None:
        for inv, old in enumerate(self._unpacked):
            if old is not None:
                self._release_kept(old)
                self._unpacked[inv] = None

    @staticmethod
    def _release_kept(kept) -> None:
        release_resident(kept[3])
        if kept[4]:
            release_kept_offloaded(kept[3])

    def __del__(self):
        try:
            self.release_kept_indices()
        except Exception:
            pass

    @torch.compiler.disable
    def _remember_indices(self, inds: Optional[Tensor], counts: Tensor, ragged=None) -> None:
        inv = self.layer_counter.cur_model_invocation_per_step
        old, self._unpacked[inv] = self._unpacked[inv], None
        if old is not None:
            self._release_kept(old)
        self.storage.indices.suppress_current(False)
        if not (counts.is_cuda and amd_key("attn", "keep_unpacked_indices") and amd_key("attn", "fused_residual")
                and (self.storage.indices.is_resident() or amd_key("attn", "keep_unpacked_indices_offloaded"))):
            return
        if not reserve_resident(0):
            return
        flat, offsets = ragged if ragged is not None else ops.compact_indices(inds, counts)
        nbytes = 4 * flat.numel() + 8 * offsets.numel() + 4 * counts.numel()
        off_mode = not self.storage.indices.is_resident()
        if off_mode and not reserve_kept_offloaded(nbytes):
            return
        if not reserve_resident(nbytes):
            if off_mode:
                release_kept_offloaded(nbytes)
            return
        self._unpacked[inv] = (flat, offsets, counts, nbytes, off_mode)
        self.storage.indices.suppress_current(off_mode and bool(GLOBAL_CONFIG["attn"]["recompute_mask"]))

    def _kept_indices(self):
        kept = self._unpacked[self.layer_counter.cur_model_invocation_per_step]
        if kept is not None and GLOBAL_CONFIG["attn"]["should_compress_indices"] and (
                self.storage.indices.is_resident() or amd_key("attn", "keep_unpacked_indices_offloaded")):
            return kept[:3]
        return None

    def _stored_mask(self):
        if self.storage.indices.is_suppressed():
            self.storage.indices.suppress_current(False)
            self.storage.indices.load_async()
            self.storage.indices.load_async_wait()
        return self.storage.get_indices(), self.mask_shape[self.layer_counter.cur_model_invocation_per_step]

    @staticmethod
    def _ragged_enabled(x: Tensor) -> bool:
        return bool(x.is_cuda and GLOBAL_CONFIG["attn"]["should_compress_indices"] and amd_key("attn", "fused_residual")
                    and amd_key("attn", "fused_packed_mask_to_indices") and amd_key("attn", "ragged_mask_to_indices"))

    @torch.compiler.disable
    def _ragged_indices(self, packed: Tensor, shape, multiple_of: int, bm: int, mask: Optional[Tensor] = None):
        if shape[-1] % 8 != 0:
            packed = mask if mask is not None else ops.bitunpack(packed, shape)
        return ops.mask_to_ragged_indices(packed, shape, multiple_of, bm, bool(amd_key("attn", "sorted_indices")))

    def _stored_indices(self, multiple_of: int, bm: int):
        cfg = GLOBAL_CONFIG["attn"]
        if cfg["should_compress_indices"]:
            packed, shape = self._stored_mask()
            if amd_key("attn", "fused_packed_mask_to_indices") and packed.is_cuda and shape[-1] % 8 == 0:
                if amd_key("attn", "sorted_indices"):
                    return ops.mask_to_sorted_indices(packed, shape, multiple_of, bm)
                return ops.packed_mask_to_indices(packed, shape, multiple_of, bm)
            return ops.mask_to_indices(ops.bitunpack(packed, shape), multiple_of, bm)
        return self.storage.get_indices(), self.storage.get_counts()

    def _fast_attention(self, q: Tensor, k: Tensor, v: Tensor, inference_step: int, do_full_step: bool) -> Tensor:
        cfg = GLOBAL_CONFIG["attn"]
        bm = cfg["mbm"]
        assert bm == 192, "The kernel was written for BM=192. You may need to change the kernel."
        do_padding = cfg["pad_qkv_before_kernel"]
        multiple_of = 128 if do_padding else cfg["counts_multiple_of"]

        tm = bool(q.is_cuda and amd_key("attn", "token_major_output"))
        use_ragged = self._ragged_enabled(q)
        if self.layer_num < cfg["first_n_dense_layers"]:
            o, _ = ops.dense_attn(q, k, v, tm)
            return o

        if do_full_step:
            if inference_step == 0:
                o, lse = ops.dense_attn(q, k, v, tm) if do_padding else _dense_attn_raw(q, k, v, tm)
                lse[..., k.shape[-2]:, :] = 0
                self.storage.set_lse_constants(lse)
                return o

            ragged = None
            if inference_step == 1 or cfg["recompute_mask"]:
                prev_lse = self.storage.get_lse_constants()
                tk = int(multiple_of * round((cfg["top_keys"] * k.shape[-2]) / multiple_of))
                mask = bs = None
                if (q.is_cuda and cfg["should_compress_indices"] and tk > 0 and amd_key("attn", "fused_colsum_topk")
                        and amd_key("attn", "fused_topk_mask") and k.shape[-2] <= ops.TOPK_MASK_MAX_N):
                    static, groups = self._static(q.shape[1], _cdiv(q.shape[-2], bm), k.shape[-2])
                    o, mask, lse = ops.dense_colsum_topk_mask(q, k, v, prev_lse, tk, 0.01, groups, static, tm)
                elif do_padding:
                    o, bs, lse = ops.dense_colsum_attn(q, k, v, prev_lse, tm)
                else:
                    o, bs, lse = (torch.ops.chipmunk.dense_colsum_attn_layout(q, k, v, prev_lse, True) if tm else
                                  torch.ops.chipmunk.dense_colsum_attn(q, k, v, prev_lse))
                lse[..., k.shape[-2]:, :] = 0
                self.storage.set_lse_constants(lse)
                if cfg["should_compress_indices"]:
                    if mask is not None:
                        pass
                    elif tk > 0:
                        mask = self.random_and_topk(bs, tk)
                    else:
                        mask = self._static(bs.shape[1], bs.shape[-2], bs.shape[-1])[0]
                    packed, mask_shape = ops.bitpack(mask)
                    self.mask_shape[self.layer_counter.cur_model_invocation_per_step] = mask_shape
                    self.storage.set_indices(packed)
                    if use_ragged:
                        ragged = self._ragged_indices(packed, mask_shape, multiple_of, bm, mask)
                        self._remember_indices(None, ragged[2], ragged[:2])
                    else:
                        if mask.is_cuda and amd_key("attn", "fused_packed_mask_to_indices") and amd_key("attn", "sorted_indices"):
                            inds, counts = ops.mask_to_sorted_indices(mask, mask.shape, multiple_of, bm)
                        else:
                            inds, counts = ops.mask_to_indices(mask, multiple_of, bm)
                        self._remember_indices(inds, counts)
                else:
                    kseq = k.shape[-2]
                    bs = bs[..., :_cdiv(kseq, bm), :kseq]
                    inds = torch.topk(bs, k=tk, dim=-1).indices
                    counts = torch.full((q.shape[0], q.shape[1], _cdiv(q.shape[-2], bm)), tk, device=q.device,
                                        dtype=torch.int32)
                    pad = torch.empty((*counts.shape, q.shape[-2] - tk), device=q.device, dtype=torch.int32)
                    inds = torch.cat([inds, pad], dim=-1).to(torch.int32)
                    self.storage.set_indices(inds)
                    self.storage.set_counts(counts)
            else:
                o, _ = ops.dense_attn(q, k, v, tm)

            if use_ragged:
                if ragged is None:
                    ragged = self._ragged_indices(*self._stored_mask(), multiple_of, bm)
            elif not (inference_step == 1 or cfg["recompute_mask"]):
                inds, counts = self._stored_indices(multiple_of, bm)

            if ragged is not None:
                o_cache = ops.csp_attn_out_ragged(q, k, v, o, ragged[0], ragged[1], ragged[2], -1)
            elif o.is_cuda and amd_key("attn", "fused_residual"):
                o_cache = ops.csp_attn_out(q, k, v, o, inds, counts, -1)
            elif do_padding:
                o_cache = o - ops.csp_attn(q, k, v, inds, counts)
            else:
                o_cache = o.clone()
                ops.csp_attn_inplace(q, k, v, o_cache, inds, counts, -1)
            self.storage.set_out_cache(o_cache)
            return o

        o = self.storage.get_out_cache()
        kept = self._kept_indices() if (o.is_cuda and amd_key("attn", "fused_residual")) else None
        if kept is not None:
            return ops.csp_attn_out_ragged(q, k, v, o, kept[0], kept[1], kept[2], 1)
        if use_ragged:
            flat, offsets, counts = self._ragged_indices(*self._stored_mask(), multiple_of, bm)
            return ops.csp_attn_out_ragged(q, k, v, o, flat, offsets, counts, 1)
        inds, counts = self._stored_indices(multiple_of, bm)
        if do_padding:
            if o.is_cuda and amd_key("attn", "fused_residual"):
                return ops.csp_attn_out(q, k, v, o, inds, counts, 1)
            return o + ops.csp_attn(q, k, v, inds, counts)
        persistent = self.storage.out_cache.is_resident()
        if o.is_cuda and amd_key("attn", "fused_residual") and persistent:
            return ops.csp_attn_out(q, k, v, o, inds, counts, 1)
        if persistent:
            o = o.clone()
        ops.csp_attn_inplace(q, k, v, o, inds, counts, 1)
        return o

    def forward(self, q: Tensor, k: Tensor, v: Tensor) -> Tensor:
        if not GLOBAL_CONFIG["attn"]["is_enabled"]:
            return F.scaled_dot_product_attention(q, k, v)
        do_full_step = self.layer_counter.should_do_full_attn_step()
        out = self._fast_attention(q, k, v, self.layer_counter.cur_inference_step, do_full_step)
        self.layer_counter.increment()
        return out

    def __call__(self, *args, **kwargs):
        return self.forward(*args, **kwargs)
```

### chipmunk_amd/ops/__init__.py

```python
from .mlp import run_e2e as mlp
from .mlp import run_e2e_glu as mlp_glu, run_e2e_glu, mm1_glu
from .mlp import run_e2e_glu_fp8 as mlp_glu_fp8, run_e2e_glu_fp8, mm1_glu_fp8
from .indexed_io import (copy_indices, topk_indices, mask_to_indices, scatter_add, packed_mask_to_indices,
                         mask_to_sorted_indices, mask_to_ragged_indices, topk_mask, manual_seed, TOPK_MASK_MAX_N)
from .attn import compact_indices, csp_attn, csp_attn_inplace, csp_attn_out, csp_attn_out_ragged, dense_attn, dense_colsum_attn, dense_colsum_topk_mask
from .patch import patchify, unpatchify, patchify_rope
from .bitpack import bitpack, bitunpack
from . import voxel
from .qkv import qkv_split_norm, residual_ln_modulate, split_heads_rownorm, wan_rope_table

__all__ = ["mlp", "copy_indices", "topk_indices", "mask_to_indices", "scatter_add", "csp_attn", "dense_attn",
           "dense_colsum_attn", "patchify", "unpatchify", "patchify_rope", "bitpack", "bitunpack",
           "packed_mask_to_indices", "mask_to_sorted_indices", "csp_attn_inplace", "csp_attn_out", "topk_mask", "TOPK_MASK_MAX_N", "voxel", "manual_seed", "qkv_split_norm", "dense_colsum_topk_mask", "compact_indices", "csp_attn_out_ragged", "residual_ln_modulate",
           "split_heads_rownorm", "wan_rope_table", "mask_to_ragged_indices", "mlp_glu", "run_e2e_glu", "mm1_glu",
           "mlp_glu_fp8", "run_e2e_glu_fp8", "mm1_glu_fp8"]

from . import _fake
```

### chipmunk_amd/ops/_fake.py

```python
import torch


def _o_like(q, token_major):
    B, H, N, D = q.shape
    return q.new_empty((B, N, H, D)).permute(0, 2, 1, 3) if token_major else q.new_empty((B, H, N, D))


def _register():
    lib = torch.library

    @lib.register_fake("chipmunk::csp_128_attn")
    def _(q, k, v, indices, indices_counts):
        return torch.empty_like(q)

    @lib.register_fake("chipmunk::csp_attn_out")
    def _(q, k, v, o_in, indices, indices_counts, o_scale):
        return torch.empty_like(o_in)

    @lib.register_fake("chipmunk::residual_ln_modulate")
    def _(x, y, gate, shift, scale, eps):
        return [torch.empty_like(x), torch.empty_like(x)] if y is not None else [torch.empty_like(x)]

    @lib.register_fake("chipmunk::csp_attn_out_ragged")
    def _(q, k, v, o_in, indices, offsets, indices_counts, o_scale):
        return torch.empty_like(o_in)

    @lib.register_fake("chipmunk::dense_attn")
    def _(q, k, v):
        return [_o_like(q, False), q.new_empty((q.shape[0], q.shape[1], q.shape[2], 1), dtype=torch.float32)]

    @lib.register_fake("chipmunk::dense_attn_layout")
    def _(q, k, v, token_major_o):
        return [_o_like(q, token_major_o), q.new_empty((q.shape[0], q.shape[1], q.shape[2], 1), dtype=torch.float32)]

    @lib.register_fake("chipmunk::dense_colsum_attn_layout")
    def _(q, k, v, p, token_major_o):
        groups = (q.shape[2] + 191) // 192
        return [_o_like(q, token_major_o),
                q.new_empty((q.shape[0], q.shape[1], groups, max(q.shape[2], k.shape[2]))),
                q.new_empty((q.shape[0], q.shape[1], q.shape[2], 1), dtype=torch.float32)]

    @lib.register_fake("chipmunk::dense_colsum_attn")
    def _(q, k, v, p):
        groups = (q.shape[2] + 191) // 192
        return [_o_like(q, False),
                q.new_empty((q.shape[0], q.shape[1], groups, max(q.shape[2], k.shape[2]))),
                q.new_empty((q.shape[0], q.shape[1], q.shape[2], 1), dtype=torch.float32)]

    @lib.register_fake("chipmunk::mask_to_indices")
    def _(mask, multiple_of, pad_to_multiple_of):
        b, h, m, n = mask.shape
        pad_n = (n + pad_to_multiple_of - 1) // pad_to_multiple_of * pad_to_multiple_of
        return [mask.new_empty((b, h, m, pad_n), dtype=torch.int32), mask.new_empty((b, h, m), dtype=torch.int32)]

    @lib.register_fake("chipmunk::packed_mask_to_indices")
    def _(packed, shape, multiple_of, pad_to_multiple_of):
        b, h, m, n = shape
        pad_n = (n + pad_to_multiple_of - 1) // pad_to_multiple_of * pad_to_multiple_of
        return [packed.new_empty((b, h, m, pad_n), dtype=torch.int32), packed.new_empty((b, h, m), dtype=torch.int32)]

    @lib.register_fake("chipmunk::topk_mask")
    def _(cs, k, random_amount, groups, static_mask):
        return cs.new_empty(cs.shape, dtype=torch.bool)

    @lib.register_fake("chipmunk::block_mean")
    def _(x, mbm):
        return x.new_empty((x.shape[0], (x.shape[1] + mbm - 1) // mbm, x.shape[2]))

    @lib.register_fake("chipmunk::transpose_last2")
    def _(x):
        return x.new_empty(x.shape[:-2] + (x.shape[-1], x.shape[-2]))

    @lib.register_fake("chipmunk::transpose_last2_pitched")
    def _(x, ld):
        return x.new_empty(x.shape[:-2] + (x.shape[-1], ld))

    @lib.register_fake("chipmunk::quantize_fp8")
    def _(x, scale, max_value):
        return x.new_empty(x.shape, dtype=torch.float8_e4m3fn)

    @lib.register_fake("chipmunk::bitpack")
    def _(mask):
        return mask.new_empty(((mask.numel() + 7) // 8,), dtype=torch.uint8)

    @lib.register_fake("chipmunk::bitunpack")
    def _(packed, shape):
        return packed.new_empty(tuple(shape), dtype=torch.bool)

    @lib.register_fake("chipmunk::gather_rows")
    def _(src, map):
        shape = list(src.shape)
        shape[-2] = map.shape[0]
        return src.new_empty(shape)

    @lib.register_fake("chipmunk::dense_colsum_topk_mask")
    def _(q, k, v, p, k_top, random_amount, groups, static_mask, token_major_o=False):
        B, H, Nq, D = q.shape
        G = (Nq + 191) // 192
        return [_o_like(q, token_major_o), q.new_empty((B, H, G, k.shape[2]), dtype=torch.bool),
                q.new_empty((B, H, Nq, 1), dtype=torch.float32)]

    @lib.register_fake("chipmunk::qkv_split_norm")
    def _(qkv, q_weight, k_weight, heads, eps, freqs_cos=None, freqs_sin=None):
        out = qkv.new_empty((3, 1, heads, qkv.shape[0], 128))
        return [out[0], out[1], out[2]]

    @lib.register_fake("chipmunk::split_heads_rownorm")
    def _(x, heads, parts, w0, w1, w2, norm_mask, rope_mask, eps, freqs_cos=None, freqs_sin=None):
        out = x.new_empty((parts, x.shape[0] if x.dim() == 3 else 1, heads, x.shape[-2], 128))
        return [out[p] for p in range(parts)]

    @lib.register_fake("chipmunk::csp_mlp_mm1_glu")
    def _(a, b_gate, b_up, c, bias_gate, bias_up, pa_cache_colmajor, indices, indices_counts, act, update_cache):
        torch._check(a.shape[-1] == b_gate.shape[1] and b_gate.shape == b_up.shape, lambda: "a, b_gate and b_up must share K; b_up the shape of b_gate")
        torch._check(c.shape == a.shape[:-1] + (b_gate.shape[0],), lambda: "c must be [M, F] ([B, M, F] with the batch size of a)")
        torch._check(act in ("gelu_tanh", "silu", "gelu"), lambda: f"csp_mlp_mm1_glu: unknown activation '{act}'")
        return None

    @lib.register_fake("chipmunk::csp_mlp_mm1_glu_fp8")
    def _(a, b_gate, b_up, c, bias_gate, bias_up, pa_cache_colmajor, indices, indices_counts, scale_a, scale_b_gate, scale_b_up, act,
          update_cache):
        f8 = torch.float8_e4m3fn
        torch._check(a.dtype == f8 and b_gate.dtype == f8 and b_up.dtype == f8, lambda: "a, b_gate and b_up must be float8_e4m3fn")
        torch._check(c.dtype == torch.bfloat16 and pa_cache_colmajor.dtype == torch.bfloat16, lambda: "c and pa_cache_colmajor must be bfloat16")
        torch._check(a.shape[-1] == b_gate.shape[1] and b_gate.shape == b_up.shape, lambda: "a, b_gate and b_up must share K; b_up the shape of b_gate")
        torch._check(c.shape == a.shape[:-1] + (b_gate.shape[0],), lambda: "c must be [M, F] ([B, M, F] with the batch size of a)")
        for s in (scale_a, scale_b_gate, scale_b_up):
            torch._check(s.dtype == torch.float32 and s.numel() == 1, lambda: "scale_a, scale_b_gate and scale_b_up must be one-element float32 tensors")
        torch._check(act in ("gelu_tanh", "silu", "gelu"), lambda: f"csp_mlp_mm1_glu_fp8: unknown activation '{act}'")
        return None


_register()
```

### chipmunk_amd/ops/attn.py

```python
from __future__ import annotations

from typing import Tuple

import torch
import torch.nn.functional as F

PM = 192


def _pad_len(n: int) -> int:
    return ((n + PM - 1) // PM) * PM


def _last_dim_contiguous(t: torch.Tensor) -> torch.Tensor:
    return t if t.stride(-1) == 1 else t.contiguous()


def dense_attn(q: torch.Tensor, k: torch.Tensor, v: torch.Tensor, token_major_o: bool = False) -> Tuple[torch.Tensor, torch.Tensor]:
    n = q.shape[-2]
    q, k, v = _last_dim_contiguous(q), _last_dim_contiguous(k), _last_dim_contiguous(v)
    o, l = torch.ops.chipmunk.dense_attn_layout(q, k, v, True) if token_major_o else torch.ops.chipmunk.dense_attn(q, k, v)
    padded = _pad_len(n)
    if padded != n:
        l = F.pad(l, (0, 0, 0, padded - n))
    return o, l


def dense_colsum_attn(q: torch.Tensor, k: torch.Tensor, v: torch.Tensor, p: torch.Tensor, token_major_o: bool = False
                      ) -> Tuple[torch.Tensor, torch.Tensor, torch.Tensor]:
    n = q.shape[-2]
    padded = _pad_len(n)
    assert p.shape[-2] in (n, padded), "p must be the l vector of the previous full step"
    p_rows = p[..., :n, :].contiguous()
    q, k, v = _last_dim_contiguous(q), _last_dim_contiguous(k), _last_dim_contiguous(v)
    if token_major_o:
        o, cs, l = torch.ops.chipmunk.dense_colsum_attn_layout(q, k, v, p_rows, True)
    else:
        o, cs, l = torch.ops.chipmunk.dense_colsum_attn(q, k, v, p_rows)
    if padded != n:
        l = F.pad(l, (0, 0, 0, padded - n))
    kseq = k.shape[-2]
    kgroups = (kseq + PM - 1) // PM
    if cs.shape[-2] != kgroups or cs.shape[-1] != kseq:
        cs = cs[..., :kgroups, :kseq]
    return o, cs, l


def dense_colsum_topk_mask(q: torch.Tensor, k: torch.Tensor, v: torch.Tensor, p: torch.Tensor, k_top: int, random_amount: float,
                           groups, static_mask, token_major_o: bool = False) -> Tuple[torch.Tensor, torch.Tensor, torch.Tensor]:
    n = q.shape[-2]
    padded = _pad_len(n)
    assert p.shape[-2] in (n, padded), "p must be the l vector of the previous full step"
    o, mask, l = torch.ops.chipmunk.dense_colsum_topk_mask(_last_dim_contiguous(q), _last_dim_contiguous(k), _last_dim_contiguous(v),
                                                           p[..., :n, :].contiguous(), k_top, random_amount, groups, static_mask,
                                                           token_major_o)
    if padded != n:
        l = F.pad(l, (0, 0, 0, padded - n))
    return o, mask, l


def csp_attn(q: torch.Tensor, k: torch.Tensor, v: torch.Tensor, indices: torch.Tensor,
             indices_counts: torch.Tensor) -> torch.Tensor:
    return torch.ops.chipmunk.csp_128_attn(q.contiguous(), k.contiguous(), v.contiguous(), indices.contiguous(),
                                           indices_counts.contiguous())


def csp_attn_inplace(q: torch.Tensor, k: torch.Tensor, v: torch.Tensor, o: torch.Tensor, indices: torch.Tensor,
                     indices_counts: torch.Tensor, o_scale: int) -> None:
    torch.ops.chipmunk.csp_attn(q, k, v, o, indices, indices_counts, o_scale)


def csp_attn_out(q: torch.Tensor, k: torch.Tensor, v: torch.Tensor, o_in: torch.Tensor, indices: torch.Tensor,
                 indices_counts: torch.Tensor, o_scale: int) -> torch.Tensor:
    return torch.ops.chipmunk.csp_attn_out(q, k, v, o_in, indices, indices_counts, o_scale)


def compact_indices(indices: torch.Tensor, indices_counts: torch.Tensor) -> Tuple[torch.Tensor, torch.Tensor]:
    return tuple(torch.ops.chipmunk.compact_indices(indices.contiguous(), indices_counts.contiguous()))


def csp_attn_out_ragged(q: torch.Tensor, k: torch.Tensor, v: torch.Tensor, o_in: torch.Tensor, indices: torch.Tensor,
                        offsets: torch.Tensor, indices_counts: torch.Tensor, o_scale: int) -> torch.Tensor:
    return torch.ops.chipmunk.csp_attn_out_ragged(q, k, v, o_in, indices, offsets, indices_counts, o_scale)


__all__ = ["csp_attn", "csp_attn_inplace", "csp_attn_out", "csp_attn_out_ragged", "compact_indices", "dense_attn", "dense_colsum_attn",
           "dense_colsum_topk_mask"]
```

### chipmunk_amd/ops/indexed_io.py

```python
from __future__ import annotations

from typing import List, Optional, Sequence

import torch

TOPK_MASK_MAX_N = 1024 * 512


def copy_indices(bm_fc1: torch.Tensor, bm_mid_cache: torch.Tensor, indices: torch.Tensor, counts: torch.Tensor) -> None:
    torch.ops.chipmunk.copy_indices(bm_fc1, bm_mid_cache, indices, counts)


def topk_indices(activations: torch.Tensor, indices_out: torch.Tensor, counts_out: torch.Tensor,
                 sparsity_amount: float, multiple_of: int, rk: float) -> None:
    torch.ops.chipmunk.topk_indices(activations, indices_out, counts_out, sparsity_amount, multiple_of, rk)


def scatter_add(packed: torch.Tensor, unpacked: torch.Tensor, indices: torch.Tensor, counts: torch.Tensor,
                num_sms: int) -> None:
    if packed.ndim == 3:
        torch.ops.chipmunk.csp_scatter_add(packed, unpacked, indices, counts, num_sms)
        return
    torch.ops.chipmunk.csp_scatter_add(packed.unsqueeze(0), unpacked.unsqueeze(0), indices.unsqueeze(0),
                                       counts.unsqueeze(0), num_sms)


def mask_to_indices(mask: torch.Tensor, multiple_of: int, pad_to_multiple_of: int) -> List[torch.Tensor]:
    return torch.ops.chipmunk.mask_to_indices(mask, multiple_of, pad_to_multiple_of)


def packed_mask_to_indices(packed: torch.Tensor, shape: Sequence[int], multiple_of: int,
                           pad_to_multiple_of: int) -> List[torch.Tensor]:
    return torch.ops.chipmunk.packed_mask_to_indices(packed, list(shape), multiple_of, pad_to_multiple_of)


def mask_to_sorted_indices(mask: torch.Tensor, shape: Sequence[int], multiple_of: int,
                           pad_to_multiple_of: int) -> List[torch.Tensor]:
    return torch.ops.chipmunk.mask_to_sorted_indices(mask, list(shape), multiple_of, pad_to_multiple_of)


def mask_to_ragged_indices(mask: torch.Tensor, shape: Sequence[int], multiple_of: int, pad_to_multiple_of: int,
                           sorted: bool = True) -> List[torch.Tensor]:
    if mask.is_cuda:
        return torch.ops.chipmunk.mask_to_ragged_indices(mask, list(shape), multiple_of, pad_to_multiple_of, sorted)
    if mask.dtype == torch.uint8:
        from .bitpack import bitunpack
        mask = bitunpack(mask, shape)
    b, h, m, n = mask.shape
    pad_n = (n + pad_to_multiple_of - 1) // pad_to_multiple_of * pad_to_multiple_of
    rows = mask.reshape(-1, n) != 0
    kept = rows.sum(dim=1)
    counts = (kept + multiple_of - 1) // multiple_of * multiple_of
    lengths = (counts.clamp(max=pad_n) + 31) // 32 * 32
    offsets = torch.zeros(rows.shape[0] + 1, dtype=torch.int64)
    offsets[1:] = lengths.cumsum(0)
    flat = torch.zeros(int(offsets[-1]) + 64, dtype=torch.int32)
    cols = torch.arange(n, dtype=torch.int32)
    for r in range(rows.shape[0]):
        true = cols[rows[r]]
        if not sorted:
            true = true[torch.argsort(true % 32, stable=True)]
        row = torch.cat([true, cols[~rows[r]][:int(counts[r] - kept[r])]])
        flat[int(offsets[r]):int(offsets[r]) + row.numel()] = row
    return [flat, offsets, counts.to(torch.int32).view(b, h, m)]


def topk_mask(cs: torch.Tensor, k: int, random_amount: float = 0.0, groups: Optional[torch.Tensor] = None,
              static_mask: Optional[torch.Tensor] = None) -> torch.Tensor:
    return torch.ops.chipmunk.topk_mask(cs, k, random_amount, groups, static_mask)


def manual_seed(seed: int) -> None:
    from .._native import manual_seed as _seed
    _seed(seed)
```

### chipmunk_amd/util/config.py

```python
from __future__ import annotations

import copy
from typing import Any, Dict

import yaml

BASE_CONFIG: Dict[str, Any] = {
    "num_model_invocations_per_inference_step": 1,
    "should_profile": False,
    "generation_index": 0,
    "steps": 50,
    "world_size": 1,
    "mlp": {
        "is_enabled": True,
        "is_fp8": False,
        "top_keys": "dd",
        "random_keys": 0.05,
        "full_step_every": 10,
        "block_mask_cache": 2,
        "first_n_dense_layers": 2,
        "counts_multiple_of": 256,
        "bm": 128,
        "mbm": 128,
    },
    "patchify": {
        "is_enabled": True,
        "chunk_size_1": 8,
        "chunk_size_2": 4,
    },
    "attn": {
        "is_enabled": True,
        "top_keys": 0.05,
        "random_keys": 0.01,
        "local_voxels": 0,
        "local_1d_window": 0,
        "first_n_dense_layers": 2,
        "full_step_every": 10,
        "full_step_schedule": None,
        "recompute_mask": True,
        "should_compress_indices": True,
        "counts_multiple_of": 128,
        "pad_qkv_before_kernel": True,
        "mbm": 192,
    },
    "offloading": {
        "global_disable_offloading": False,
        "mlp.out_cache": False,
        "mlp.indices": False,
        "mlp.counts": False,
        "mlp.sparse_act_T": False,
        "mlp.blockmean_mid_cache": False,
        "attn.out_cache": True,
        "attn.indices": True,
        "attn.counts": False,
        "attn.lse_constants": False,
        "text_encoders": True,
    },
    "step_caching": {
        "is_enabled": True,
        "skip_step_schedule": {7, 11, 13, 14, 15, 17, 18, 19, 21, 22, 23, 25, 26, 27, 29, 31, 33, 34, 35, 37, 38, 39,
                               41, 42, 43},
    },
}

AMD_EXTRA_KEYS: Dict[str, Any] = {
    "offloading.keep_resident_if_fits": False,
    "offloading.hbm_budget_gb": 200.0,
    "offloading.native_host_pool": True,
    "attn.fused_packed_mask_to_indices": True,
    "attn.sorted_indices": True,
    "mlp.fused_topk_delta": True,
    "mlp.fused_block_mean": True,
    "mlp.fused_fp8_quantize": True,
    "attn.fused_residual": True,
    "attn.fused_topk_mask": True,
    "attn.fused_colsum_topk": True,
    "mlp.fused_scatter": True,
    "attn.token_major_output": False,
    "attn.keep_unpacked_indices": True,
    "attn.keep_unpacked_indices_offloaded": True,
    "attn.kept_indices_offloaded_budget_gb": 8.0,
    "attn.ragged_mask_to_indices": True,
}
BASE_CONFIG["offloading"]["keep_resident_if_fits"] = AMD_EXTRA_KEYS["offloading.keep_resident_if_fits"]
BASE_CONFIG["offloading"]["hbm_budget_gb"] = AMD_EXTRA_KEYS["offloading.hbm_budget_gb"]
BASE_CONFIG["offloading"]["native_host_pool"] = AMD_EXTRA_KEYS["offloading.native_host_pool"]
BASE_CONFIG["attn"]["fused_packed_mask_to_indices"] = AMD_EXTRA_KEYS["attn.fused_packed_mask_to_indices"]
BASE_CONFIG["attn"]["sorted_indices"] = AMD_EXTRA_KEYS["attn.sorted_indices"]
BASE_CONFIG["mlp"]["fused_topk_delta"] = AMD_EXTRA_KEYS["mlp.fused_topk_delta"]
BASE_CONFIG["attn"]["fused_residual"] = AMD_EXTRA_KEYS["attn.fused_residual"]
BASE_CONFIG["attn"]["fused_topk_mask"] = AMD_EXTRA_KEYS["attn.fused_topk_mask"]
BASE_CONFIG["attn"]["fused_colsum_topk"] = AMD_EXTRA_KEYS["attn.fused_colsum_topk"]
BASE_CONFIG["mlp"]["fused_scatter"] = AMD_EXTRA_KEYS["mlp.fused_scatter"]
BASE_CONFIG["attn"]["token_major_output"] = AMD_EXTRA_KEYS["attn.token_major_output"]
BASE_CONFIG["attn"]["keep_unpacked_indices"] = AMD_EXTRA_KEYS["attn.keep_unpacked_indices"]
BASE_CONFIG["attn"]["keep_unpacked_indices_offloaded"] = AMD_EXTRA_KEYS["attn.keep_unpacked_indices_offloaded"]
BASE_CONFIG["attn"]["kept_indices_offloaded_budget_gb"] = AMD_EXTRA_KEYS["attn.kept_indices_offloaded_budget_gb"]
BASE_CONFIG["attn"]["ragged_mask_to_indices"] = AMD_EXTRA_KEYS["attn.ragged_mask_to_indices"]

GLOBAL_CONFIG: Dict[str, Any] = copy.deepcopy(BASE_CONFIG)


def amd_key(section: str, key: str) -> Any:
    return GLOBAL_CONFIG.get(section, {}).get(key, AMD_EXTRA_KEYS[f"{section}.{key}"])


def update_global_config(config: Dict[str, Any]) -> None:
    GLOBAL_CONFIG.update(config)


def _deep_update(dst: Dict[str, Any], src: Dict[str, Any]) -> None:
    for key, value in src.items():
        if isinstance(value, dict) and isinstance(dst.get(key), dict):
            _deep_update(dst[key], value)
        else:
            dst[key] = value


def load_from_file(config_file: str) -> None:
    with open(config_file, "r") as f:
        loaded = yaml.safe_load(f)
    if loaded:
        _deep_update(GLOBAL_CONFIG, loaded)
        print(f"CHIPMUNK: using config file {config_file}")


def reset_to_base() -> None:
    fresh = copy.deepcopy(BASE_CONFIG)
    GLOBAL_CONFIG.clear()
    GLOBAL_CONFIG.update(fresh)
```

### include/chipmunk_hip.h

```cpp
#ifndef CHIPMUNK_HIP_H
#define CHIPMUNK_HIP_H

#include <stdint.h>

#ifdef __cplusplus
extern "C" {
#endif

#define CHIPMUNK_OK 0
#define CHIPMUNK_ERR_INVALID 1
#define CHIPMUNK_ERR_LAUNCH 2
#define CHIPMUNK_ERR_UNSUPPORTED 3

#define CHIPMUNK_DTYPE_BF16 0
#define CHIPMUNK_DTYPE_FP16 1
#define CHIPMUNK_DTYPE_FP32 2

const char *chipmunk_last_error(void);
int chipmunk_abi_version(void);
int chipmunk_set_option(const char *name, int value);
int chipmunk_set_random_seed(uint64_t seed);

int chipmunk_csp_attn(const void *q, const void *k, const void *v, void *o, const int64_t q_strides[3],
                      const int64_t k_strides[3], const int64_t v_strides[3], const int64_t o_strides[3],
                      const int32_t *indices, const int32_t *counts, int B, int H, int Nq, int Nk, int idx_stride,
                      int o_scale, void *stream);

int chipmunk_csp_attn_out(const void *q, const void *k, const void *v, const void *o_in, void *o_out,
                          const int64_t q_strides[3], const int64_t k_strides[3], const int64_t v_strides[3],
                          const int64_t o_strides[3], const int32_t *indices, const int32_t *counts, int B, int H,
                          int Nq, int Nk, int idx_stride, int o_scale, void *stream);

int chipmunk_csp_attn_out_ragged(const void *q, const void *k, const void *v, const void *o_in, void *o_out,
                                 const int64_t q_strides[3], const int64_t k_strides[3], const int64_t v_strides[3],
                                 const int64_t o_strides[3], const int32_t *indices, const int64_t *idx_offsets,
                                 const int32_t *counts, int B, int H, int Nq, int Nk, int o_scale, void *stream);
int chipmunk_compact_indices(const int32_t *indices, int64_t idx_stride, const int32_t *counts, const int64_t *offsets,
                             int32_t *flat, int64_t rows, void *stream);

int chipmunk_csp_128_attn(const void *q, const void *k, const void *v, void *o, const int32_t *indices,
                          const int32_t *counts, int B, int H, int Nq, int Nk, int idx_stride, void *stream);

int chipmunk_dense_attn(const void *q, const void *k, const void *v, const int64_t q_strides[3],
                        const int64_t k_strides[3], const int64_t v_strides[3], void *o, float *l, int B, int H,
                        int Nq, int Nk, void *stream);

int chipmunk_dense_attn_strided(const void *q, const void *k, const void *v, const int64_t q_strides[3],
                                const int64_t k_strides[3], const int64_t v_strides[3], void *o, const int64_t *o_strides,
                                float *l, int B, int H, int Nq, int Nk, void *stream);
int chipmunk_dense_colsum_attn_strided(const void *q, const void *k, const void *v, const int64_t q_strides[3],
                                       const int64_t k_strides[3], const int64_t v_strides[3], const float *p, void *o,
                                       const int64_t *o_strides, void *cs, float *l, int B, int H, int Nq, int Nk,
                                       int cs_stride, void *stream);
int chipmunk_dense_colsum_topk_mask_strided(const void *q, const void *k, const void *v, const int64_t q_strides[3],
                                            const int64_t k_strides[3], const int64_t v_strides[3], const float *p, void *o,
                                            const int64_t *o_strides, float *l, int B, int H, int Nq, int Nk,
                                            const void *static_mask, int64_t static_stride, int static_rows,
                                            const void *group_flags, void *mask, int k_top, double random_amount, void *stream);

int chipmunk_dense_colsum_attn(const void *q, const void *k, const void *v, const int64_t q_strides[3],
                               const int64_t k_strides[3], const int64_t v_strides[3], const float *p, void *o,
                               void *cs, float *l, int B, int H, int Nq, int Nk, int cs_stride, void *stream);

int chipmunk_residual_ln_modulate(const void *x, const void *y, const void *gate, const void *shift, const void *scale,
                                  void *x_out, void *xm, int64_t rows, int cols, double eps, void *stream);

int chipmunk_csp_mlp_mm1(const void *a, const void *b, void *c, const void *bias, const void *pa_cache,
                         const int32_t *indices, const int32_t *counts, int M, int K, int F, void *stream);

int chipmunk_csp_mlp_mm1_scatter(const void *a, const void *b, void *c, const void *bias, void *pa_cache,
                                 const int32_t *indices, const int32_t *counts, int M, int K, int F, void *stream);

int chipmunk_csp_mlp_mm1_fp8(const void *a, const void *b, void *c, const void *bias, void *pa_cache,
                             const int32_t *indices, const int32_t *counts, const float *scale_a,
                             const float *scale_b, int M, int K, int F, int update_cache, void *stream);

int chipmunk_csp_mlp_mm2_and_scatter_add(const void *packed, void *unpacked_colmajor, const int32_t *indices,
                                         const int32_t *counts, const void *mma_a, const void *mma_b, void *mma_c,
                                         int M, int F, int N2, int num_sms_scatter_add, void *stream);

int chipmunk_csp_scatter_add(const void *packed, void *unpacked_colmajor, const int32_t *indices,
                             const int32_t *counts, int M, int F, int num_sms, void *stream);

int chipmunk_csp_mlp_mm2(const void *mma_a, const void *mma_b, void *mma_c, const int32_t *indices,
                         const int32_t *counts, int M, int F, int N2, void *stream);

int chipmunk_csp_mlp_mm1_ragged(const void *a, const void *b, void *c, const void *bias, const void *pa_cache,
                                const int32_t *indices, const int32_t *counts, int M, int K, int F, int ldc, void *stream);
int chipmunk_csp_mlp_mm1_scatter_ragged(const void *a, const void *b, void *c, const void *bias, void *pa_cache,
                                        const int32_t *indices, const int32_t *counts, int M, int K, int F, int ldc,
                                        void *stream);
int chipmunk_csp_mlp_mm1_fp8_ragged(const void *a, const void *b, void *c, const void *bias, void *pa_cache,
                                    const int32_t *indices, const int32_t *counts, const float *scale_a,
                                    const float *scale_b, int M, int K, int F, int ldc, int update_cache, void *stream);
int chipmunk_csp_mlp_mm2_ragged(const void *mma_a, const void *mma_b, void *mma_c, const int32_t *indices,
                                const int32_t *counts, int M, int F, int N2, void *stream);
int chipmunk_csp_mlp_mm2_and_scatter_add_ragged(const void *packed, void *unpacked_colmajor, const int32_t *indices,
                                                const int32_t *counts, const void *mma_a, const void *mma_b, void *mma_c,
                                                int M, int F, int N2, int ldc, void *stream);
int chipmunk_csp_scatter_add_ragged(const void *packed, void *unpacked_colmajor, const int32_t *indices,
                                    const int32_t *counts, int M, int F, int ldc, void *stream);

int chipmunk_csp_mlp_mm1_batched(const void *a, const void *b, void *c, const void *bias, const void *pa_cache,
                                 const int32_t *indices, const int32_t *counts, int M, int K, int F, int ldc, int B,
                                 int64_t cache_batch_stride, void *stream);
int chipmunk_csp_mlp_mm1_scatter_batched(const void *a, const void *b, void *c, const void *bias, void *pa_cache,
                                         const int32_t *indices, const int32_t *counts, int M, int K, int F, int ldc, int B,
                                         int64_t cache_batch_stride, void *stream);
int chipmunk_csp_mlp_mm1_fp8_batched(const void *a, const void *b, void *c, const void *bias, void *pa_cache,
                                     const int32_t *indices, const int32_t *counts, const float *scale_a, const float *scale_b,
                                     int M, int K, int F, int ldc, int update_cache, int B, int64_t cache_batch_stride,
                                     void *stream);
int chipmunk_csp_mlp_mm2_batched(const void *mma_a, const void *mma_b, void *mma_c, const int32_t *indices,
                                 const int32_t *counts, int M, int F, int N2, int B, void *stream);
int chipmunk_csp_mlp_mm2_and_scatter_add_batched(const void *packed, void *unpacked_colmajor, const int32_t *indices,
                                                 const int32_t *counts, const void *mma_a, const void *mma_b, void *mma_c,
                                                 int M, int F, int N2, int ldc, int B, int64_t cache_batch_stride,
                                                 void *stream);
int chipmunk_csp_scatter_add_batched(const void *packed, void *unpacked_colmajor, const int32_t *indices,
                                     const int32_t *counts, int M, int F, int ldc, int B, int64_t cache_batch_stride,
                                     void *stream);

#define CHIPMUNK_ACT_GELU_TANH 0
#define CHIPMUNK_ACT_SILU 1
#define CHIPMUNK_ACT_GELU_ERF 2
int chipmunk_csp_mlp_mm1_glu(const void *a, const void *b_gate, const void *b_up, void *c, const void *bias_gate,
                             const void *bias_up, void *pa_cache, const int32_t *indices, const int32_t *counts, int M, int K,
                             int F, int ldc, int act, int update_cache, void *stream);
int chipmunk_csp_mlp_mm1_glu_batched(const void *a, const void *b_gate, const void *b_up, void *c, const void *bias_gate,
                                     const void *bias_up, void *pa_cache, const int32_t *indices, const int32_t *counts, int M,
                                     int K, int F, int ldc, int act, int update_cache, int B, int64_t cache_batch_stride,
                                     void *stream);
int chipmunk_csp_mlp_mm1_glu_fp8(const void *a, const void *b_gate, const void *b_up, void *c, const void *bias_gate,
                                 const void *bias_up, void *pa_cache, const int32_t *indices, const int32_t *counts,
                                 const float *scale_a, const float *scale_b_gate, const float *scale_b_up, int M, int K, int F,
                                 int ldc, int act, int update_cache, void *stream);
int chipmunk_csp_mlp_mm1_glu_fp8_batched(const void *a, const void *b_gate, const void *b_up, void *c, const void *bias_gate,
                                         const void *bias_up, void *pa_cache, const int32_t *indices, const int32_t *counts,
                                         const float *scale_a, const float *scale_b_gate, const float *scale_b_up, int M, int K,
                                         int F, int ldc, int act, int update_cache, int B, int64_t cache_batch_stride,
                                         void *stream);

int chipmunk_topk_indices(const void *activation, int dtype, int32_t *indices, int32_t *counts, int rows, int cols,
                          double sparsity_amount, int multiple_of, double random_amount, void *stream);

int chipmunk_topk_delta_indices(const void *activation, void *cache, int dtype, int32_t *indices, int32_t *counts,
                                int rows, int cols, double sparsity_amount, int multiple_of, double random_amount,
                                void *stream);

int chipmunk_dense_colsum_topk_mask(const void *q, const void *k, const void *v, const int64_t q_strides[3],
                                    const int64_t k_strides[3], const int64_t v_strides[3], const float *p, void *o, float *l,
                                    int B, int H, int Nq, int Nk, const void *static_mask, int64_t static_stride, int static_rows,
                                    const void *group_flags, void *mask, int k_top, double random_amount, void *stream);

int chipmunk_topk_mask(const void *cs, int64_t cs_stride, const void *static_mask, int64_t static_stride,
                       int static_rows, const void *group_flags, void *mask, int rows, int n, int k,
                       double random_amount, void *stream);

int chipmunk_mask_to_indices(const void *mask, int32_t *indices, int32_t *counts, int64_t rows, int n, int pad_n,
                             int multiple_of, void *stream);

int chipmunk_packed_mask_to_indices(const void *packed, int32_t *indices, int32_t *counts, int64_t rows, int n,
                                    int pad_n, int multiple_of, void *stream);

int chipmunk_mask_to_sorted_indices(const void *mask, int packed, int32_t *indices, int32_t *counts, int64_t rows,
                                    int n, int pad_n, int multiple_of, void *stream);

int chipmunk_mask_row_counts(const void *mask, int packed, int32_t *counts, int64_t *lengths, int64_t rows, int n, int pad_n,
                             int multiple_of, void *stream);
int chipmunk_mask_to_ragged_indices(const void *mask, int packed, int sorted, const int64_t *offsets, int32_t *flat, int64_t rows,
                                    int n, int multiple_of, void *stream);

int chipmunk_copy_indices(const void *src, void *dst, const int32_t *inds, const int32_t *counts, int B, int M, int R,
                          int F, int elem_size, void *stream);

int chipmunk_transpose16(const void *src, void *dst, int B, int R, int C, void *stream);
int chipmunk_transpose16_pitched(const void *src, void *dst, int B, int R, int C, int ld, void *stream);

int chipmunk_block_mean(const void *x, void *out, int64_t rows, int C, int mbm, void *stream);
int chipmunk_block_mean_ragged(const void *x, void *out, int64_t rows, int C, int mbm, void *stream);

int chipmunk_quantize_fp8(const void *x, const float *scale, void *out, int64_t n, float max_value, void *stream);

int chipmunk_bitpack(const void *mask, void *packed, int64_t n, void *stream);
int chipmunk_bitunpack(const void *packed, void *mask, int64_t n, void *stream);

int chipmunk_gather_rows(const void *src, void *dst, const int32_t *map, int64_t outer, int64_t n_src, int64_t n_out,
                         int64_t row_bytes, void *stream);

int chipmunk_host_alloc(size_t bytes, void **host_ptr);
int chipmunk_host_free(void *host_ptr);
int chipmunk_copy_d2h_async(void *host_dst, const void *dev_src, size_t bytes, void *stream);
int chipmunk_copy_h2d_async(void *dev_dst, const void *host_src, size_t bytes, void *stream);
size_t chipmunk_host_bytes(void);

int chipmunk_release_scratch(void);
int chipmunk_big_scratch_fallbacks(void);

int chipmunk_qkv_split_norm(const void *qkv, int64_t row_stride, const void *q_weight, const void *k_weight, void *q, void *k,
                            void *v, int64_t n, int heads, float eps, const float *freqs_cos, const float *freqs_sin,
                            int64_t rope_rows, void *stream);

int chipmunk_split_heads_rownorm(const void *x, int64_t batch_stride, int64_t row_stride, int parts, const void *w0, int w0_dtype,
                                 const void *w1, int w1_dtype, const void *w2, int w2_dtype, void *out0, void *out1, void *out2,
                                 unsigned norm_mask, unsigned rope_mask, int64_t B, int64_t n, int heads, float eps,
                                 const float *freqs_cos, const float *freqs_sin, int64_t rope_rows, void *stream);

#ifdef __cplusplus
}
#endif
#endif
```

Baseline: 0.5542.

## Emit bit-packed top-k masks with per-row kept counts from colsum selection

Adds a BITS variant of the top-k mask kernel. It writes the selected columns as a bit-packed mask, assembled with DPP lane ORs, and records the per-row kept count directly. A small kernel then turns those counts into padded counts and ragged lengths, so the separate row-count pass over the mask can be skipped. The aim is to cut mask write bandwidth by 8x and remove a full mask read pass before index building, and it is enabled by default through attn.packed_selection. In exchange it adds kernel template variants and restricts this path to Nk divisible by 8.

```diff
diff --git a/chipmunk_amd/_native.py b/chipmunk_amd/_native.py
--- a/chipmunk_amd/_native.py
+++ b/chipmunk_amd/_native.py
@@ -17,6 +17,7 @@
     "chipmunk_csp_mlp_mm1_glu", "chipmunk_csp_mlp_mm1_glu_batched", "chipmunk_csp_mlp_mm1_glu_fp8", "chipmunk_csp_mlp_mm1_glu_fp8_batched",
     "chipmunk_topk_indices", "chipmunk_topk_delta_indices", "chipmunk_topk_mask", "chipmunk_mask_to_indices", "chipmunk_mask_to_sorted_indices", "chipmunk_packed_mask_to_indices", "chipmunk_mask_row_counts", "chipmunk_mask_to_ragged_indices", "chipmunk_copy_indices",
     "chipmunk_bitpack", "chipmunk_bitunpack", "chipmunk_transpose16", "chipmunk_block_mean", "chipmunk_quantize_fp8", "chipmunk_gather_rows", "chipmunk_qkv_split_norm", "chipmunk_split_heads_rownorm", "chipmunk_dense_colsum_topk_mask", "chipmunk_dense_attn_strided", "chipmunk_csp_attn_out_ragged", "chipmunk_compact_indices", "chipmunk_residual_ln_modulate", "chipmunk_dense_colsum_attn_strided", "chipmunk_dense_colsum_topk_mask_strided", "chipmunk_release_scratch", "chipmunk_big_scratch_fallbacks",
+    "chipmunk_topk_bits", "chipmunk_dense_colsum_topk_bits", "chipmunk_row_counts_from_kept",
     "chipmunk_host_alloc", "chipmunk_host_free", "chipmunk_copy_d2h_async", "chipmunk_copy_h2d_async", "chipmunk_host_bytes",
 ]
 
diff --git a/chipmunk_amd/csrc/attn.hip b/chipmunk_amd/csrc/attn.hip
--- a/chipmunk_amd/csrc/attn.hip
+++ b/chipmunk_amd/csrc/attn.hip
@@ -1238,13 +1238,14 @@
                                               cs_stride, stream);
 }
 
-extern "C" int chipmunk_dense_colsum_topk_mask_strided(const void *q, const void *k, const void *v, const int64_t q_strides[3],
-                                               const int64_t k_strides[3], const int64_t v_strides[3], const float *pin, void *o,
-                                               const int64_t *o_strides, float *l, int B, int H, int Nq, int Nk, const void *static_mask,
-                                               int64_t static_stride, int static_rows, const void *group_flags, void *mask,
-                                               int topk, double random_amount, void *stream) {
+static int dense_colsum_select(const void *q, const void *k, const void *v, const int64_t q_strides[3],
+                               const int64_t k_strides[3], const int64_t v_strides[3], const float *pin, void *o,
+                               const int64_t *o_strides, float *l, int B, int H, int Nq, int Nk, const void *static_mask,
+                               int64_t static_stride, int static_rows, const void *group_flags, void *mask, int32_t *kept,
+                               int topk, double random_amount, void *stream) {
     if (int e = check_common(q, k, v, o, B, H, Nq, Nk)) return e;
     CM_CHECK(l && pin && mask, "dense_colsum_topk_mask: p / l / mask missing");
+    if (kept && ((Nk & 7) || Nk > 1024 * 120)) return CHIPMUNK_ERR_UNSUPPORTED;
     if (int e = check_strides(q_strides, "q")) return e;
     if (int e = check_strides(k_strides, "k")) return e;
     if (int e = check_strides(v_strides, "v")) return e;
@@ -1264,8 +1265,30 @@
     if (!part) return CHIPMUNK_ERR_UNSUPPORTED;
     if (int e = chipmunk_dense64_colsum_launch(p, part, st)) return e;
     const int nrb = ((Nq + 255) / 256) * 2;
+    if (kept)
+        return chipmunk_topk_bits_parts(part, chipmunk_colsum_part_stride(Nk), nrb, p.G, Nq, static_mask, static_stride, static_rows, group_flags, mask,
+                                        kept, B * H * p.G, Nk, topk, random_amount, st);
     return chipmunk_topk_mask_parts(part, chipmunk_colsum_part_stride(Nk), nrb, p.G, Nq, static_mask, static_stride, static_rows, group_flags, mask, B * H * p.G, Nk,
                                     topk, random_amount, st);
+}
+
+extern "C" int chipmunk_dense_colsum_topk_mask_strided(const void *q, const void *k, const void *v, const int64_t q_strides[3],
+                                               const int64_t k_strides[3], const int64_t v_strides[3], const float *pin, void *o,
+                                               const int64_t *o_strides, float *l, int B, int H, int Nq, int Nk, const void *static_mask,
+                                               int64_t static_stride, int static_rows, const void *group_flags, void *mask,
+                                               int topk, double random_amount, void *stream) {
+    return dense_colsum_select(q, k, v, q_strides, k_strides, v_strides, pin, o, o_strides, l, B, H, Nq, Nk, static_mask, static_stride,
+                               static_rows, group_flags, mask, nullptr, topk, random_amount, stream);
+}
+
+extern "C" int chipmunk_dense_colsum_topk_bits(const void *q, const void *k, const void *v, const int64_t q_strides[3],
+                                               const int64_t k_strides[3], const int64_t v_strides[3], const float *pin, void *o,
+                                               const int64_t *o_strides, float *l, int B, int H, int Nq, int Nk, const void *static_bits,
+                                               int64_t static_stride, int static_rows, const void *group_flags, void *packed, int32_t *kept,
+                                               int topk, double random_amount, void *stream) {
+    CM_CHECK(kept, "dense_colsum_topk_bits: kept missing");
+    return dense_colsum_select(q, k, v, q_strides, k_strides, v_strides, pin, o, o_strides, l, B, H, Nq, Nk, static_bits, static_stride,
+                               static_rows, group_flags, packed, kept, topk, random_amount, stream);
 }
 
 extern "C" int chipmunk_dense_colsum_topk_mask(const void *q, const void *k, const void *v, const int64_t q_strides[3],
diff --git a/chipmunk_amd/csrc/attn_params.h b/chipmunk_amd/csrc/attn_params.h
--- a/chipmunk_amd/csrc/attn_params.h
+++ b/chipmunk_amd/csrc/attn_params.h
@@ -32,6 +32,9 @@
 int chipmunk_topk_mask_parts(const uint16_t *part, int part_stride, int nrb, int groups_per_bh, int Nq, const void *static_mask, int64_t static_stride,
                              int static_rows, const void *group_flags, void *mask, int rows, int n, int k, double random_amount,
                              hipStream_t stream);
+int chipmunk_topk_bits_parts(const uint16_t *part, int part_stride, int nrb, int groups_per_bh, int Nq, const void *static_bits,
+                             int64_t static_stride, int static_rows, const void *group_flags, void *packed, int32_t *kept, int rows, int n,
+                             int k, double random_amount, hipStream_t stream);
 size_t chipmunk_colsum_part_bytes(int B, int H, int Nq, int Nk);
 int chipmunk_colsum_part_stride(int Nk);
 int chipmunk_colsum64_launch(const AttnParams &p, hipStream_t stream);
diff --git a/chipmunk_amd/csrc/indexed_io.hip b/chipmunk_amd/csrc/indexed_io.hip
--- a/chipmunk_amd/csrc/indexed_io.hip
+++ b/chipmunk_amd/csrc/indexed_io.hip
@@ -246,6 +246,15 @@
     }
 }
 
+__global__ __launch_bounds__(256) void row_counts_from_kept_kernel(const int32_t *kept, int32_t *counts, int64_t *lengths, int64_t rows,
+                                                                   int pad_n, int multiple_of) {
+    const int64_t row = (int64_t)blockIdx.x * 256 + threadIdx.x;
+    if (row >= rows) return;
+    const int64_t padded = (((int64_t)kept[row] + multiple_of - 1) / multiple_of) * multiple_of;
+    counts[row] = (int32_t)padded;
+    lengths[row] = (min(padded, (int64_t)pad_n) + 31) / 32 * 32;
+}
+
 struct TopkParams {
     const void *act;
     void *cache;
@@ -561,13 +570,21 @@
     const uint16_t *parts;
     int64_t pstride;
     int nrb, ngroups, nq;
+    int32_t *kept;
 };
+
+__device__ __forceinline__ uint32_t or_over_8_lanes(uint32_t v) {
+    v |= (uint32_t)__builtin_amdgcn_update_dpp(0, (int)v, 0xB1, 0xf, 0xf, false);
+    v |= (uint32_t)__builtin_amdgcn_update_dpp(0, (int)v, 0x4E, 0xf, 0xf, false);
+    v |= (uint32_t)__builtin_amdgcn_update_dpp(0, (int)v, 0x141, 0xf, 0xf, false);
+    return v;
+}
 
 __device__ __forceinline__ uint32_t bf16_key(uint32_t u) {
     return (u & 0x8000u) ? (~u & 0xffffu) : (u | 0x8000u);
 }
 
-template <int KPT, bool ALIGNED, bool PARTS = false>
+template <int KPT, bool ALIGNED, bool PARTS = false, bool BITS = false>
 __global__ __launch_bounds__(1024) void topk_mask_kernel(const TopkMaskParams p) {
     constexpr int NV = KPT / 4;
     __shared__ int wave_cnt[16];
@@ -751,7 +768,68 @@
                 if (c + e < n) out[c + e] = (uint8_t)(bytes >> (8 * e));
         }
     };
-    if constexpr (ALIGNED) {
+    if constexpr (BITS) {
+        static_assert(ALIGNED, "the packed output is written by the aligned form only");
+        const int nb = n >> 3;
+        uint8_t *outb = p.mask + (int64_t)row * nb;
+        const uint8_t *stb = p.stat ? p.stat + (int64_t)(row % p.stat_rows) * p.stat_stride : nullptr;
+        const bool dwords = ((uintptr_t)outb & 3) == 0;
+        const uint32_t nib_shift = 4u * (uint32_t)(lane & 7);
+        int kept = 0;
+        constexpr int OB = 5;
+#pragma unroll
+        for (int j0 = 0; j0 < NV; j0 += OB) {
+            uint32_t sbv[OB];
+#pragma unroll
+            for (int jj = 0; jj < OB; ++jj) {
+                const int c = 4 * tid + 4096 * (j0 + jj);
+                sbv[jj] = (j0 + jj < NV && stb && c < n) ? (uint32_t)stb[c >> 3] : 0u;
+            }
+            __builtin_amdgcn_sched_barrier(0);
+#pragma unroll
+            for (int jj = 0; jj < OB; ++jj) {
+                if (j0 + jj < NV) {
+                    const int j = (j0 + jj) < NV ? (j0 + jj) : 0;
+                    const int c = 4 * tid + 4096 * j;
+                    uint32_t nib = 0;
+                    if (c < n) {
+                        uint32_t v0 = key[j][0], v1 = key[j][1];
+                        asm volatile("" : "+v"(v0), "+v"(v1));
+                        const uint32_t sb = sbv[jj] >> (4 * (tid & 1));
+#pragma unroll
+                        for (int e = 0; e < 4; ++e) {
+                            const uint32_t kv = ((e < 2 ? v0 : v1) >> (16 * (e & 1))) & 0xffffu;
+                            bool keep = kv > thr;
+                            const bool tie = kv == thr && tie_budget > 0 && c + e < n;
+                            tie_budget -= tie ? 1 : 0;
+                            keep = keep || tie;
+                            if (rnd && !keep) keep = hash_uniform(row, c + e, salt) < p.random_amount;
+                            keep = keep || ((sb >> e) & 1u) != 0;
+                            nib |= (keep ? 1u : 0u) << e;
+                        }
+                    }
+                    kept += __popc(nib);
+                    const uint32_t word = or_over_8_lanes(nib << nib_shift);
+                    if (dwords) {
+                        const int b0 = 4 * (tid >> 3) + 512 * j;
+                        if ((lane & 7) == 0) {
+                            if (b0 + 4 <= nb) *(uint32_t *)(outb + b0) = word;
+                            else
+                                for (int b = 0; b < 3; ++b)
+                                    if (b0 + b < nb) outb[b0 + b] = (uint8_t)(word >> (8 * b));
+                        }
+                    } else {
+                        const int b0 = (tid >> 1) + 512 * j;
+                        if ((lane & 1) == 0 && b0 < nb) outb[b0] = (uint8_t)(word >> (8 * ((lane & 7) >> 1)));
+                    }
+                    asm volatile("" ::: "memory");
+                }
+            }
+            __builtin_amdgcn_sched_barrier(0);
+        }
+        kept = block_count(kept);
+        if (tid == 0) p.kept[row] = kept;
+    } else if constexpr (ALIGNED) {
         constexpr int OB = 5;
 #pragma unroll
         for (int j0 = 0; j0 < NV; j0 += OB) {
@@ -1063,6 +1141,18 @@
     const dim3 grid((unsigned)((rows + 3) / 4));
     if (packed) hipLaunchKernelGGL(mask_row_counts_kernel<true>, grid, dim3(256), 0, (hipStream_t)stream, p);
     else hipLaunchKernelGGL(mask_row_counts_kernel<false>, grid, dim3(256), 0, (hipStream_t)stream, p);
+    CM_LAUNCH_CHECK();
+    return CHIPMUNK_OK;
+}
+
+extern "C" int chipmunk_row_counts_from_kept(const int32_t *kept, int32_t *counts, int64_t *lengths, int64_t rows, int pad_n, int multiple_of,
+                                             void *stream) {
+    CM_CHECK(kept && counts && lengths, "row_counts_from_kept: null pointer");
+    CM_CHECK(rows >= 0 && rows < (1ll << 31) && pad_n > 0 && multiple_of > 0, "row_counts_from_kept: bad sizes rows=%lld pad_n=%d multiple_of=%d",
+             (long long)rows, pad_n, multiple_of);
+    if (rows == 0) return CHIPMUNK_OK;
+    hipLaunchKernelGGL(row_counts_from_kept_kernel, dim3((unsigned)((rows + 255) / 256)), dim3(256), 0, (hipStream_t)stream, kept, counts, lengths,
+                       rows, pad_n, multiple_of);
     CM_LAUNCH_CHECK();
     return CHIPMUNK_OK;
 }
@@ -1200,6 +1290,50 @@
     else hipLaunchKernelGGL((topk_mask_kernel<120, true, true>), dim3(rows), dim3(1024), 0, s, p);
     CM_LAUNCH_CHECK();
     return CHIPMUNK_OK;
+}
+
+static int launch_topk_bits(const uint16_t *cs, int64_t cs_stride, const uint16_t *part, int part_stride, int nrb, int groups_per_bh, int Nq,
+                            const void *static_bits, int64_t static_stride, int static_rows, const void *group_flags, void *packed,
+                            int32_t *kept, int rows, int n, int k, double random_amount, hipStream_t s) {
+    CM_CHECK((cs || part) && packed && kept, "topk_bits: null pointer");
+    CM_CHECK(rows >= 0 && n > 0 && k >= 0, "topk_bits: bad sizes (rows=%d n=%d k=%d)", rows, n, k);
+    CM_CHECK(random_amount >= 0.0 && random_amount <= 1.0, "topk_bits: random_amount must be in [0,1]");
+    CM_CHECK(!static_bits || (static_rows > 0 && static_stride >= n / 8), "topk_bits: bad static mask geometry");
+    if (n % 8 != 0 || n > 1024 * 120) return CHIPMUNK_ERR_UNSUPPORTED;
+    if (cs && ((((uintptr_t)cs) & 7) != 0 || cs_stride < n || (cs_stride & 3) != 0)) return CHIPMUNK_ERR_UNSUPPORTED;
+    CM_CHECK(!part || ((((uintptr_t)part) & 7) == 0 && part_stride >= n && (part_stride & 3) == 0), "topk_bits: bad partial rows");
+    if (rows == 0) return CHIPMUNK_OK;
+    TopkMaskParams p = {cs, (const uint8_t *)static_bits, (const uint8_t *)group_flags, (uint8_t *)packed, cs_stride, static_stride,
+                        rows, n, k, static_bits ? static_rows : 1, (float)random_amount,
+                        random_amount > 0.0 ? chipmunk_next_random_salt() : 0u};
+    p.parts = part, p.pstride = part_stride, p.nrb = nrb, p.ngroups = groups_per_bh, p.nq = Nq, p.kept = kept;
+#define LAUNCH_TB(KPT)                                                                                                   \
+    do {                                                                                                                 \
+        if (part) hipLaunchKernelGGL((topk_mask_kernel<KPT, true, true, true>), dim3(rows), dim3(1024), 0, s, p);        \
+        else hipLaunchKernelGGL((topk_mask_kernel<KPT, true, false, true>), dim3(rows), dim3(1024), 0, s, p);            \
+    } while (0)
+    if (n <= 1024 * 16) LAUNCH_TB(16);
+    else if (n <= 1024 * 48) LAUNCH_TB(48);
+    else LAUNCH_TB(120);
+#undef LAUNCH_TB
+    CM_LAUNCH_CHECK();
+    return CHIPMUNK_OK;
+}
+
+int chipmunk_topk_bits_parts(const uint16_t *part, int part_stride, int nrb, int groups_per_bh, int Nq, const void *static_bits,
+                             int64_t static_stride, int static_rows, const void *group_flags, void *packed, int32_t *kept, int rows, int n,
+                             int k, double random_amount, hipStream_t s) {
+    CM_CHECK(part, "topk_bits: null pointer");
+    return launch_topk_bits(nullptr, 0, part, part_stride, nrb, groups_per_bh, Nq, static_bits, static_stride, static_rows, group_flags, packed,
+                            kept, rows, n, k, random_amount, s);
+}
+
+extern "C" int chipmunk_topk_bits(const void *cs, int64_t cs_stride, const void *static_bits, int64_t static_stride, int static_rows,
+                                  const void *group_flags, void *packed, int32_t *kept, int rows, int n, int k, double random_amount,
+                                  void *stream) {
+    CM_CHECK(cs, "topk_bits: null pointer");
+    return launch_topk_bits((const uint16_t *)cs, cs_stride, nullptr, 0, 0, 1, 0, static_bits, static_stride, static_rows, group_flags, packed,
+                            kept, rows, n, k, random_amount, (hipStream_t)stream);
 }
 
 __global__ __launch_bounds__(256) void qkv_split_norm_kernel(const uint16_t *qkv, int64_t row_stride, const uint16_t *qw,
diff --git a/chipmunk_amd/csrc/torch_registry.cpp b/chipmunk_amd/csrc/torch_registry.cpp
--- a/chipmunk_amd/csrc/torch_registry.cpp
+++ b/chipmunk_amd/csrc/torch_registry.cpp
@@ -765,7 +765,7 @@
 }
 
 std::vector<at::Tensor> mask_to_ragged_indices(at::Tensor mask, at::IntArrayRef shape, int64_t multiple_of, int64_t pad_to_multiple_of,
-                                               bool sorted) {
+                                               bool sorted, const c10::optional<at::Tensor> &kept) {
     CHECK_DEV(mask);
     const bool packed = mask.scalar_type() == at::kByte;
     TORCH_CHECK(packed || mask.scalar_type() == at::kBool, "mask must be bool, or uint8 bit-packed with a shape");
@@ -780,9 +780,18 @@
     c10::DeviceGuard guard(mask.device());
     at::Tensor counts = at::empty({b, h, m}, mask.options().dtype(at::kInt));
     at::Tensor len = at::empty({rows}, mask.options().dtype(at::kLong));
-    check(chipmunk_mask_row_counts(mask.data_ptr(), packed ? 1 : 0, counts.data_ptr<int>(), len.data_ptr<int64_t>(), rows, (int)n,
-                                   (int)pad_n, (int)multiple_of, cur_stream(mask)),
-          "mask_to_ragged_indices");
+    if (kept.has_value() && kept->defined()) {
+        TORCH_CHECK(kept->is_cuda() && kept->get_device() == mask.get_device() && kept->scalar_type() == at::kInt && kept->numel() == rows,
+                    "kept must be an int32 tensor on the mask's device with one entry per mask row");
+        at::Tensor kc = kept->contiguous();
+        check(chipmunk_row_counts_from_kept(kc.data_ptr<int>(), counts.data_ptr<int>(), len.data_ptr<int64_t>(), rows, (int)pad_n,
+                                            (int)multiple_of, cur_stream(mask)),
+              "mask_to_ragged_indices");
+    } else {
+        check(chipmunk_mask_row_counts(mask.data_ptr(), packed ? 1 : 0, counts.data_ptr<int>(), len.data_ptr<int64_t>(), rows, (int)n,
+                                       (int)pad_n, (int)multiple_of, cur_stream(mask)),
+              "mask_to_ragged_indices");
+    }
     at::Tensor offsets = at::zeros({rows + 1}, len.options());
     if (rows) offsets.narrow(0, 1, rows).copy_(len.cumsum(0));
     const int64_t total = rows ? offsets[rows].item<int64_t>() : 0;
@@ -883,6 +892,91 @@
     return mask;
 }
 
+namespace {
+struct SelectionArgs {
+    const void *st = nullptr, *gf = nullptr;
+    int64_t st_stride = 0, st_rows = 1;
+    at::Tensor stc, gfc;
+};
+SelectionArgs selection_args(const c10::optional<at::Tensor> &groups, const c10::optional<at::Tensor> &static_bits, int64_t B, int64_t H,
+                             int64_t G, int64_t N) {
+    SelectionArgs a;
+    if (static_bits.has_value() && static_bits->defined()) {
+        a.stc = *static_bits;
+        CHECK_DEV(a.stc);
+        TORCH_CHECK(N % 8 == 0 && a.stc.scalar_type() == at::kByte && a.stc.dim() == 4 && a.stc.size(3) == N / 8 && a.stc.size(2) == G &&
+                        (a.stc.size(1) == 1 || a.stc.size(1) == H) && (a.stc.size(0) == 1 || a.stc.size(0) == B) &&
+                        (a.stc.size(1) == H || a.stc.size(0) == 1),
+                    "static_bits must be uint8 [1|B, 1|H, G, N / 8] (one plane for all, or one per head)");
+        if (!(a.stc.stride(3) == 1 && (a.stc.size(1) == 1 || a.stc.stride(1) == G * a.stc.stride(2)) &&
+              (a.stc.size(0) == 1 || a.stc.stride(0) == H * a.stc.stride(1))))
+            a.stc = a.stc.contiguous();
+        a.st = a.stc.data_ptr(), a.st_stride = a.stc.stride(2), a.st_rows = a.stc.size(0) * a.stc.size(1) * G;
+    }
+    if (groups.has_value() && groups->defined()) {
+        a.gfc = *groups;
+        CHECK_DEV(a.gfc);
+        TORCH_CHECK(a.gfc.scalar_type() == at::kBool && a.gfc.dim() == 4 && a.gfc.size(3) == 1 && a.gfc.size(2) == G && a.gfc.size(1) == H &&
+                        (a.gfc.size(0) == 1 || a.gfc.size(0) == B),
+                    "groups must be bool [1|B, H, G, 1]");
+        a.gfc = a.gfc.expand({B, H, G, 1}).contiguous();
+        a.gf = a.gfc.data_ptr();
+    }
+    return a;
+}
+}
+
+std::vector<at::Tensor> topk_bits(at::Tensor cs, int64_t k, double random_amount, const c10::optional<at::Tensor> &groups,
+                                  const c10::optional<at::Tensor> &static_bits) {
+    CHECK_DEV(cs); CHECK_BF16(cs);
+    TORCH_CHECK(cs.dim() == 4 && cs.stride(3) == 1, "cs must be [B, H, G, N] with a contiguous last dim");
+    const int64_t B = cs.size(0), H = cs.size(1), G = cs.size(2), N = cs.size(3);
+    if (!(cs.stride(1) == G * cs.stride(2) && (B == 1 || cs.stride(0) == H * cs.stride(1)))) cs = cs.contiguous();
+    const int64_t rows = B * H * G;
+    c10::DeviceGuard guard(cs.device());
+    SelectionArgs a = selection_args(groups, static_bits, B, H, G, N);
+    at::Tensor packed = at::empty({(rows * N + 7) / 8}, cs.options().dtype(at::kByte));
+    at::Tensor kept = at::empty({B, H, G}, cs.options().dtype(at::kInt));
+    const int rc = chipmunk_topk_bits(cs.data_ptr(), cs.stride(2), a.st, a.st_stride, (int)a.st_rows, a.gf, packed.data_ptr(), kept.data_ptr<int>(),
+                                      (int)rows, (int)N, (int)k, random_amount, cur_stream(cs));
+    TORCH_CHECK(rc != CHIPMUNK_ERR_UNSUPPORTED, "topk_bits: rows of ", N, " columns (N % 8 != 0, N > 122880 or unaligned rows) have no packed form; "
+                "use topk_mask and bitpack");
+    check(rc, "topk_bits");
+    return {packed, kept};
+}
+
+std::vector<at::Tensor> dense_colsum_topk_bits(at::Tensor q, at::Tensor k, at::Tensor v, at::Tensor p, int64_t k_top, double random_amount,
+                                               const c10::optional<at::Tensor> &groups, const c10::optional<at::Tensor> &static_bits,
+                                               bool token_major_o) {
+    CHECK_DEV(q); CHECK_DEV(k); CHECK_DEV(v); CHECK_DEV(p);
+    CHECK_BF16(q); CHECK_BF16(k); CHECK_BF16(v);
+    const bool shapes_ok = q.dim() == 4 && k.dim() == 4 && v.dim() == 4 && q.size(3) == 128 && q.stride(3) == 1 && k.stride(3) == 1 &&
+                           v.stride(3) == 1 && p.scalar_type() == at::kFloat && p.is_contiguous();
+    if (shapes_ok && p.numel() == q.size(0) * q.size(1) * q.size(2)) {
+        const int64_t B = q.size(0), H = q.size(1), Nq = q.size(2), Nk = k.size(2), G = (Nq + 191) / 192;
+        c10::DeviceGuard guard(q.device());
+        SelectionArgs a = selection_args(groups, static_bits, B, H, G, Nk);
+        at::Tensor o = alloc_o(q, q, token_major_o);
+        const int64_t os[3] = {o.stride(0), o.stride(1), o.stride(2)};
+        at::Tensor l = at::empty({B, H, Nq, 1}, q.options().dtype(at::kFloat));
+        at::Tensor packed = at::empty({(B * H * G * Nk + 7) / 8}, q.options().dtype(at::kByte));
+        at::Tensor kept = at::empty({B, H, G}, q.options().dtype(at::kInt));
+        const int64_t qs[3] = {q.stride(0), q.stride(1), q.stride(2)}, ks[3] = {k.stride(0), k.stride(1), k.stride(2)},
+                      vs[3] = {v.stride(0), v.stride(1), v.stride(2)};
+        const int rc = chipmunk_dense_colsum_topk_bits(q.data_ptr(), k.data_ptr(), v.data_ptr(), qs, ks, vs, p.data_ptr<float>(), o.data_ptr(), os,
+                                                       l.data_ptr<float>(), (int)B, (int)H, (int)Nq, (int)Nk, a.st, a.st_stride, (int)a.st_rows, a.gf,
+                                                       packed.data_ptr(), kept.data_ptr<int>(), (int)k_top, random_amount, cur_stream(q));
+        if (rc == CHIPMUNK_OK) return {o, packed, kept, l};
+        if (rc != CHIPMUNK_ERR_UNSUPPORTED) check(rc, "dense_colsum_topk_bits");
+    }
+    auto ocl = dense_colsum_attn_layout(q, k, v, p, token_major_o);
+    at::Tensor cs = ocl[1];
+    const int64_t Nk = k.size(2), G = (q.size(2) + 191) / 192;
+    if (cs.size(-1) != Nk || cs.size(-2) != G) cs = cs.slice(-2, 0, G).slice(-1, 0, Nk);
+    auto pk = topk_bits(cs, k_top, random_amount, groups, static_bits);
+    return {ocl[0], pk[0], pk[1], ocl[2]};
+}
+
 at::Tensor bitpack(at::Tensor mask) {
     TORCH_CHECK(mask.scalar_type() == at::kBool, "mask must be bool type");
     CHECK_DEV(mask);
@@ -1033,7 +1127,9 @@
     m.def("dense_attn_layout(Tensor q, Tensor k, Tensor v, bool token_major_o) -> Tensor[]");
     m.def("dense_colsum_attn_layout(Tensor q, Tensor k, Tensor v, Tensor p, bool token_major_o) -> Tensor[]");
     m.def("compact_indices(Tensor indices, Tensor counts) -> Tensor[]");
-    m.def("mask_to_ragged_indices(Tensor mask, int[] shape, int multiple_of, int pad_to_multiple_of, bool sorted) -> Tensor[]");
+    m.def("mask_to_ragged_indices(Tensor mask, int[] shape, int multiple_of, int pad_to_multiple_of, bool sorted, Tensor? kept=None) -> Tensor[]");
+    m.def("topk_bits(Tensor cs, int k, float random_amount, Tensor? groups, Tensor? static_bits) -> Tensor[]");
+    m.def("dense_colsum_topk_bits(Tensor q, Tensor k, Tensor v, Tensor p, int k_top, float random_amount, Tensor? groups, Tensor? static_bits, bool token_major_o=False) -> Tensor[]");
     m.def("csp_attn_out_ragged(Tensor q, Tensor k, Tensor v, Tensor o_in, Tensor indices, Tensor offsets, Tensor indices_counts, int o_scale) -> Tensor");
     m.def("residual_ln_modulate(Tensor x, Tensor? y, Tensor? gate, Tensor shift, Tensor scale, float eps) -> Tensor[]");
     m.def("transpose_last2(Tensor x) -> Tensor");
@@ -1078,6 +1174,8 @@
     m.impl("mask_to_sorted_indices", &mask_to_sorted_indices);
     m.impl("mask_to_ragged_indices", &mask_to_ragged_indices);
     m.impl("topk_mask", &topk_mask);
+    m.impl("topk_bits", &topk_bits);
+    m.impl("dense_colsum_topk_bits", &dense_colsum_topk_bits);
     m.impl("transpose_last2", &transpose_last2);
     m.impl("transpose_last2_pitched", &transpose_last2_pitched);
     m.impl("block_mean", &block_mean);
diff --git a/chipmunk_amd/modules/attn.py b/chipmunk_amd/modules/attn.py
--- a/chipmunk_amd/modules/attn.py
+++ b/chipmunk_amd/modules/attn.py
@@ -15,6 +15,7 @@
 
 singleton_static_mask: Optional[Tensor] = None
 singleton_video_query_groups: Optional[Tensor] = None
+_static_bits_cache: Optional[Tuple[Tensor, Tensor]] = None
 
 
 def _cdiv(a: int, b: int) -> int:
@@ -50,11 +51,25 @@
             for qg in range(n_video // 192):
                 centre = qg * 192 + 96
                 mask[qg, max(0, centre - window // 2):min(n_video, centre + window // 2)] = True
-        mask = mask[None, None, :, :].expand(1, local_heads_num, -1, -1).contiguous()
+        plane = mask[None, None, :, :]
+        mask = plane.expand(1, local_heads_num, -1, -1).contiguous()
         sparse_groups = (mask.sum(dim=-1, keepdim=True) + topk) < (n_video + txt_len)
-        global singleton_static_mask, singleton_video_query_groups
+        global singleton_static_mask, singleton_video_query_groups, _static_bits_cache
         singleton_static_mask = mask
         singleton_video_query_groups = sparse_groups
+        _static_bits_cache = (mask, ops.pack_mask_rows(plane)) if mask.is_cuda and plane.shape[-1] % 8 == 0 else None
+
+    def _static_bits(self, heads: int, qg: int, n: int):
+        global _static_bits_cache
+        if _static_bits_cache is None or _static_bits_cache[0] is not singleton_static_mask:
+            m = singleton_static_mask
+            same = m.shape[1] == 1 or bool((m == m[:, :1]).all())
+            _static_bits_cache = (m, ops.pack_mask_rows(m[:, :1] if same else m))
+        bits = _static_bits_cache[1]
+        g0 = self.query_group_offset
+        groups = self._static(heads, qg, n)[1]
+        h = min(heads, bits.shape[1])
+        return bits[:, :h, g0:g0 + qg, :n // 8], groups
 
     def _static(self, heads: int, qg: int, n: int):
         g0 = self.query_group_offset
@@ -138,10 +153,10 @@
                     and amd_key("attn", "fused_packed_mask_to_indices") and amd_key("attn", "ragged_mask_to_indices"))
 
     @torch.compiler.disable
-    def _ragged_indices(self, packed: Tensor, shape, multiple_of: int, bm: int, mask: Optional[Tensor] = None):
+    def _ragged_indices(self, packed: Tensor, shape, multiple_of: int, bm: int, mask: Optional[Tensor] = None, kept: Optional[Tensor] = None):
         if shape[-1] % 8 != 0:
             packed = mask if mask is not None else ops.bitunpack(packed, shape)
-        return ops.mask_to_ragged_indices(packed, shape, multiple_of, bm, bool(amd_key("attn", "sorted_indices")))
+        return ops.mask_to_ragged_indices(packed, shape, multiple_of, bm, bool(amd_key("attn", "sorted_indices")), kept=kept)
 
     def _stored_indices(self, multiple_of: int, bm: int):
         cfg = GLOBAL_CONFIG["attn"]
@@ -178,11 +193,16 @@
             if inference_step == 1 or cfg["recompute_mask"]:
                 prev_lse = self.storage.get_lse_constants()
                 tk = int(multiple_of * round((cfg["top_keys"] * k.shape[-2]) / multiple_of))
-                mask = bs = None
+                mask = bs = packed = kept = None
                 if (q.is_cuda and cfg["should_compress_indices"] and tk > 0 and amd_key("attn", "fused_colsum_topk")
                         and amd_key("attn", "fused_topk_mask") and k.shape[-2] <= ops.TOPK_MASK_MAX_N):
-                    static, groups = self._static(q.shape[1], _cdiv(q.shape[-2], bm), k.shape[-2])
-                    o, mask, lse = ops.dense_colsum_topk_mask(q, k, v, prev_lse, tk, 0.01, groups, static, tm)
+                    qg, n = _cdiv(q.shape[-2], bm), k.shape[-2]
+                    if use_ragged and amd_key("attn", "packed_selection") and n % 8 == 0 and n <= ops.TOPK_BITS_MAX_N:
+                        bits, groups = self._static_bits(q.shape[1], qg, n)
+                        o, packed, kept, lse = ops.dense_colsum_topk_mask(q, k, v, prev_lse, tk, 0.01, groups, bits, tm, True)
+                    else:
+                        static, groups = self._static(q.shape[1], qg, n)
+                        o, mask, lse = ops.dense_colsum_topk_mask(q, k, v, prev_lse, tk, 0.01, groups, static, tm)
                 elif do_padding:
                     o, bs, lse = ops.dense_colsum_attn(q, k, v, prev_lse, tm)
                 else:
@@ -190,7 +210,13 @@
                                   torch.ops.chipmunk.dense_colsum_attn(q, k, v, prev_lse))
                 lse[..., k.shape[-2]:, :] = 0
                 self.storage.set_lse_constants(lse)
-                if cfg["should_compress_indices"]:
+                if packed is not None:
+                    mask_shape = torch.Size((q.shape[0], q.shape[1], _cdiv(q.shape[-2], bm), k.shape[-2]))
+                    self.mask_shape[self.layer_counter.cur_model_invocation_per_step] = mask_shape
+                    self.storage.set_indices(packed)
+                    ragged = self._ragged_indices(packed, mask_shape, multiple_of, bm, kept=kept)
+                    self._remember_indices(None, ragged[2], ragged[:2])
+                elif cfg["should_compress_indices"]:
                     if mask is not None:
                         pass
                     elif tk > 0:
diff --git a/chipmunk_amd/ops/__init__.py b/chipmunk_amd/ops/__init__.py
--- a/chipmunk_amd/ops/__init__.py
+++ b/chipmunk_amd/ops/__init__.py
@@ -2,8 +2,9 @@
 from .mlp import run_e2e_glu as mlp_glu, run_e2e_glu, mm1_glu
 from .mlp import run_e2e_glu_fp8 as mlp_glu_fp8, run_e2e_glu_fp8, mm1_glu_fp8
 from .indexed_io import (copy_indices, topk_indices, mask_to_indices, scatter_add, packed_mask_to_indices,
-                         mask_to_sorted_indices, mask_to_ragged_indices, topk_mask, manual_seed, TOPK_MASK_MAX_N)
-from .attn import compact_indices, csp_attn, csp_attn_inplace, csp_attn_out, csp_attn_out_ragged, dense_attn, dense_colsum_attn, dense_colsum_topk_mask
+                         mask_to_sorted_indices, mask_to_ragged_indices, topk_mask, manual_seed, TOPK_MASK_MAX_N,
+                         topk_bits, pack_mask_rows, TOPK_BITS_MAX_N)
+from .attn import compact_indices, csp_attn, csp_attn_inplace, csp_attn_out, csp_attn_out_ragged, dense_attn, dense_colsum_attn, dense_colsum_topk_mask, dense_colsum_topk_bits
 from .patch import patchify, unpatchify, patchify_rope
 from .bitpack import bitpack, bitunpack
 from . import voxel
@@ -13,6 +14,6 @@
            "dense_colsum_attn", "patchify", "unpatchify", "patchify_rope", "bitpack", "bitunpack",
            "packed_mask_to_indices", "mask_to_sorted_indices", "csp_attn_inplace", "csp_attn_out", "topk_mask", "TOPK_MASK_MAX_N", "voxel", "manual_seed", "qkv_split_norm", "dense_colsum_topk_mask", "compact_indices", "csp_attn_out_ragged", "residual_ln_modulate",
            "split_heads_rownorm", "wan_rope_table", "mask_to_ragged_indices", "mlp_glu", "run_e2e_glu", "mm1_glu",
-           "mlp_glu_fp8", "run_e2e_glu_fp8", "mm1_glu_fp8"]
+           "mlp_glu_fp8", "run_e2e_glu_fp8", "mm1_glu_fp8", "topk_bits", "pack_mask_rows", "TOPK_BITS_MAX_N", "dense_colsum_topk_bits"]
 
 from . import _fake
diff --git a/chipmunk_amd/ops/_fake.py b/chipmunk_amd/ops/_fake.py
--- a/chipmunk_amd/ops/_fake.py
+++ b/chipmunk_amd/ops/_fake.py
@@ -100,6 +100,18 @@
         return [_o_like(q, token_major_o), q.new_empty((B, H, G, k.shape[2]), dtype=torch.bool),
                 q.new_empty((B, H, Nq, 1), dtype=torch.float32)]
 
+    @lib.register_fake("chipmunk::topk_bits")
+    def _(cs, k, random_amount, groups, static_bits):
+        B, H, G, N = cs.shape
+        return [cs.new_empty(((B * H * G * N + 7) // 8,), dtype=torch.uint8), cs.new_empty((B, H, G), dtype=torch.int32)]
+
+    @lib.register_fake("chipmunk::dense_colsum_topk_bits")
+    def _(q, k, v, p, k_top, random_amount, groups, static_bits, token_major_o=False):
+        B, H, Nq, D = q.shape
+        G = (Nq + 191) // 192
+        return [_o_like(q, token_major_o), q.new_empty(((B * H * G * k.shape[2] + 7) // 8,), dtype=torch.uint8),
+                q.new_empty((B, H, G), dtype=torch.int32), q.new_empty((B, H, Nq, 1), dtype=torch.float32)]
+
     @lib.register_fake("chipmunk::qkv_split_norm")
     def _(qkv, q_weight, k_weight, heads, eps, freqs_cos=None, freqs_sin=None):
         out = qkv.new_empty((3, 1, heads, qkv.shape[0], 128))
diff --git a/chipmunk_amd/ops/attn.py b/chipmunk_amd/ops/attn.py
--- a/chipmunk_amd/ops/attn.py
+++ b/chipmunk_amd/ops/attn.py
@@ -47,7 +47,9 @@
 
 
 def dense_colsum_topk_mask(q: torch.Tensor, k: torch.Tensor, v: torch.Tensor, p: torch.Tensor, k_top: int, random_amount: float,
-                           groups, static_mask, token_major_o: bool = False) -> Tuple[torch.Tensor, torch.Tensor, torch.Tensor]:
+                           groups, static_mask, token_major_o: bool = False, packed: bool = False):
+    if packed:
+        return dense_colsum_topk_bits(q, k, v, p, k_top, random_amount, groups, static_mask, token_major_o)
     n = q.shape[-2]
     padded = _pad_len(n)
     assert p.shape[-2] in (n, padded), "p must be the l vector of the previous full step"
@@ -57,6 +59,19 @@
     if padded != n:
         l = F.pad(l, (0, 0, 0, padded - n))
     return o, mask, l
+
+
+def dense_colsum_topk_bits(q: torch.Tensor, k: torch.Tensor, v: torch.Tensor, p: torch.Tensor, k_top: int, random_amount: float,
+                           groups, static_bits, token_major_o: bool = False):
+    n = q.shape[-2]
+    padded = _pad_len(n)
+    assert p.shape[-2] in (n, padded), "p must be the l vector of the previous full step"
+    o, packed, kept, l = torch.ops.chipmunk.dense_colsum_topk_bits(_last_dim_contiguous(q), _last_dim_contiguous(k), _last_dim_contiguous(v),
+                                                                   p[..., :n, :].contiguous(), k_top, random_amount, groups, static_bits,
+                                                                   token_major_o)
+    if padded != n:
+        l = F.pad(l, (0, 0, 0, padded - n))
+    return o, packed, kept, l
 
 
 def csp_attn(q: torch.Tensor, k: torch.Tensor, v: torch.Tensor, indices: torch.Tensor,
@@ -85,4 +100,4 @@
 
 
 __all__ = ["csp_attn", "csp_attn_inplace", "csp_attn_out", "csp_attn_out_ragged", "compact_indices", "dense_attn", "dense_colsum_attn",
-           "dense_colsum_topk_mask"]
+           "dense_colsum_topk_mask", "dense_colsum_topk_bits"]
diff --git a/chipmunk_amd/ops/indexed_io.py b/chipmunk_amd/ops/indexed_io.py
--- a/chipmunk_amd/ops/indexed_io.py
+++ b/chipmunk_amd/ops/indexed_io.py
@@ -40,9 +40,9 @@
 
 
 def mask_to_ragged_indices(mask: torch.Tensor, shape: Sequence[int], multiple_of: int, pad_to_multiple_of: int,
-                           sorted: bool = True) -> List[torch.Tensor]:
+                           sorted: bool = True, kept: Optional[torch.Tensor] = None) -> List[torch.Tensor]:
     if mask.is_cuda:
-        return torch.ops.chipmunk.mask_to_ragged_indices(mask, list(shape), multiple_of, pad_to_multiple_of, sorted)
+        return torch.ops.chipmunk.mask_to_ragged_indices(mask, list(shape), multiple_of, pad_to_multiple_of, sorted, kept)
     if mask.dtype == torch.uint8:
         from .bitpack import bitunpack
         mask = bitunpack(mask, shape)
@@ -70,6 +70,20 @@
     return torch.ops.chipmunk.topk_mask(cs, k, random_amount, groups, static_mask)
 
 
+TOPK_BITS_MAX_N = 1024 * 120
+
+
+def topk_bits(cs: torch.Tensor, k: int, random_amount: float = 0.0, groups: Optional[torch.Tensor] = None,
+              static_bits: Optional[torch.Tensor] = None) -> List[torch.Tensor]:
+    return torch.ops.chipmunk.topk_bits(cs, k, random_amount, groups, static_bits)
+
+
+def pack_mask_rows(mask: torch.Tensor) -> torch.Tensor:
+    from .bitpack import bitpack
+    assert mask.dtype == torch.bool and mask.shape[-1] % 8 == 0, "pack_mask_rows: bool rows of a multiple of 8 columns"
+    return bitpack(mask.contiguous())[0].view(*mask.shape[:-1], mask.shape[-1] // 8)
+
+
 def manual_seed(seed: int) -> None:
     from .._native import manual_seed as _seed
     _seed(seed)
diff --git a/chipmunk_amd/util/config.py b/chipmunk_amd/util/config.py
--- a/chipmunk_amd/util/config.py
+++ b/chipmunk_amd/util/config.py
@@ -81,6 +81,7 @@
     "attn.keep_unpacked_indices_offloaded": True,
     "attn.kept_indices_offloaded_budget_gb": 8.0,
     "attn.ragged_mask_to_indices": True,
+    "attn.packed_selection": True,
 }
 BASE_CONFIG["offloading"]["keep_resident_if_fits"] = AMD_EXTRA_KEYS["offloading.keep_resident_if_fits"]
 BASE_CONFIG["offloading"]["hbm_budget_gb"] = AMD_EXTRA_KEYS["offloading.hbm_budget_gb"]
@@ -97,6 +98,7 @@
 BASE_CONFIG["attn"]["keep_unpacked_indices_offloaded"] = AMD_EXTRA_KEYS["attn.keep_unpacked_indices_offloaded"]
 BASE_CONFIG["attn"]["kept_indices_offloaded_budget_gb"] = AMD_EXTRA_KEYS["attn.kept_indices_offloaded_budget_gb"]
 BASE_CONFIG["attn"]["ragged_mask_to_indices"] = AMD_EXTRA_KEYS["attn.ragged_mask_to_indices"]
+BASE_CONFIG["attn"]["packed_selection"] = AMD_EXTRA_KEYS["attn.packed_selection"]
 
 GLOBAL_CONFIG: Dict[str, Any] = copy.deepcopy(BASE_CONFIG)
 
diff --git a/include/chipmunk_hip.h b/include/chipmunk_hip.h
--- a/include/chipmunk_hip.h
+++ b/include/chipmunk_hip.h
@@ -157,6 +157,15 @@
                        int static_rows, const void *group_flags, void *mask, int rows, int n, int k,
                        double random_amount, void *stream);
 
+int chipmunk_topk_bits(const void *cs, int64_t cs_stride, const void *static_bits, int64_t static_stride, int static_rows,
+                       const void *group_flags, void *packed, int32_t *kept, int rows, int n, int k, double random_amount,
+                       void *stream);
+int chipmunk_dense_colsum_topk_bits(const void *q, const void *k, const void *v, const int64_t q_strides[3],
+                                    const int64_t k_strides[3], const int64_t v_strides[3], const float *p, void *o,
+                                    const int64_t *o_strides, float *l, int B, int H, int Nq, int Nk, const void *static_bits,
+                                    int64_t static_stride, int static_rows, const void *group_flags, void *packed, int32_t *kept,
+                                    int k_top, double random_amount, void *stream);
+
 int chipmunk_mask_to_indices(const void *mask, int32_t *indices, int32_t *counts, int64_t rows, int n, int pad_n,
                              int multiple_of, void *stream);
 
@@ -170,6 +179,8 @@
                              int multiple_of, void *stream);
 int chipmunk_mask_to_ragged_indices(const void *mask, int packed, int sorted, const int64_t *offsets, int32_t *flat, int64_t rows,
                                     int n, int multiple_of, void *stream);
+int chipmunk_row_counts_from_kept(const int32_t *kept, int32_t *counts, int64_t *lengths, int64_t rows, int pad_n, int multiple_of,
+                                  void *stream);
 
 int chipmunk_copy_indices(const void *src, void *dst, const int32_t *inds, const int32_t *counts, int B, int M, int R,
                           int F, int elem_size, void *stream);
```

After: 0.5541. About the same (-0.0%).
